# thorstone25/qups

Measured on AMD Instinct MI355X. Metric: beamformed Mpixels/sec (1024^2 px, 256x256 Tx/Rx), higher is better.
Workload: dtype f32; 1 GPU; C3: 256-el FSA (256 Tx x 256 Rx), 1024x1024 ScanCartesian lambda/4, T=2816, complex64, lanczos3; pixels=1048576, pairs_per_frame=68719476736, kernel=tiled, reciprocal_mode=True, reciprocity_fold=True, mirror_mode=True, kernel_name=das_tile_kernel<interp=3,f32,sym,fold,mirror,mb=32,W=128> [jit 56fb2bda29f94d0f], jit=True, fallback_tiles=0, aperture_split=1, parallelism=1 GPU, device=AMD Radeon Graphics (gfx950:sramecc+:xnack-), cu=256

## Files before the change

### include/qdas.h

```cpp
#ifndef QDAS_H
#define QDAS_H

#include <stddef.h>
#include <stdint.h>

#ifdef __cplusplus
extern "C" {
#endif

#define QDAS_VERSION 103

#define QDAS_F64 0
#define QDAS_F32 1
#define QDAS_F16 2

#define QDAS_INTERP_NEAREST  0
#define QDAS_INTERP_LINEAR   1
#define QDAS_INTERP_CUBIC    2
#define QDAS_INTERP_LANCZOS3 3
#define QDAS_INTERP_LINEAR4  4
#define QDAS_INTERP_CUBIC_DEV 5
#define QDAS_FLAG_INTERP_MASK 7
#define QDAS_FLAG_KEEP_RX 8
#define QDAS_FLAG_KEEP_TX 16
#define QDAS_FLAG_TPOSE   32

#define QDAS_MEM_HOST   0
#define QDAS_MEM_DEVICE 1

#define QDAS_KERNEL_AUTO    0
#define QDAS_KERNEL_GENERIC 1
#define QDAS_KERNEL_TILED   2

#define QDAS_RXAPOD_NONE             0
#define QDAS_RXAPOD_ACCEPTANCE       1
#define QDAS_RXAPOD_COSINE           2
#define QDAS_RXAPOD_FNUMBER_PLANAR   3
#define QDAS_RXAPOD_FNUMBER_ORIENTED 4

#define QDAS_PLAN_NO_RECIPROCAL 1
#define QDAS_PLAN_JIT           2

#define QDAS_PLAN_COPY_INPUTS   4

#define QDAS_PLAN_NO_MIRROR     8

#define QDAS_PLAN_MIRROR_SLAB   16

#define QDAS_PLAN_NO_FOLD       32

#define QDAS_PLAN_APPROX_SYMMETRY 64

#define QDAS_PLAN_PREFOLDED     128


#define QDAS_OK            0
#define QDAS_EINVAL        1
#define QDAS_EUNSUPPORTED  2
#define QDAS_EHIP          3
#define QDAS_ENOMEM        4
#define QDAS_ENOCONV       5
#define QDAS_ENOTLDS       6

typedef struct qdas_sizes {
    uint64_t T;
    uint64_t N, M;
    uint64_t I1, I2, I3;
    uint64_t S;
    int32_t  flag;
    int32_t  VS;
    int32_t  DV;
    int32_t  dtype;
} qdas_sizes;

typedef struct qdas_desc {
    qdas_sizes sz;
    double fs, fmod;
    const void *Pi;
    const void *Pr;
    const void *Pv;
    const void *Nv;
    const void *apod;
    const void *cinv;
    const uint64_t *acstride;
    int32_t mem;
    int32_t apod_real;
    int32_t kernel;
    int32_t device;
    uint64_t i_begin;
    uint64_t i_count;
    uint64_t y_ld;
    int32_t  rx_apod_kind;
    int32_t  plan_flags;
    double   rx_apod_p[2];
    const void *rx_normals;
} qdas_desc;

typedef struct qdas_plan qdas_plan;

int  qdas_plan_create(qdas_plan **plan, const qdas_desc *desc);
int  qdas_plan_execute(qdas_plan *plan, const void *x, void *y, void *stream);
int  qdas_plan_execute_frames(qdas_plan *plan, const void *x, void *y, uint64_t F,
                              uint64_t x_stride, uint64_t y_stride, void *stream);
int  qdas_plan_prepare_frames(qdas_plan *plan, uint64_t F);
int  qdas_plan_delays(qdas_plan *plan, void *tau, void *stream);
void qdas_plan_destroy(qdas_plan *plan);
int  qdas_plan_kernel(const qdas_plan *plan);
int  qdas_plan_fallback_tiles(const qdas_plan *plan, uint64_t *ntiles);
int  qdas_plan_tile_shape(const qdas_plan *plan, int *tile_z, int *tile_cols, int *wave_z, int *ksplit);
int  qdas_plan_reciprocal(const qdas_plan *plan);
int  qdas_plan_folded(const qdas_plan *plan);
typedef struct qdas_fold_desc {
    uint64_t T, N;
    uint64_t strN, strM;
    int32_t  dtype;
    int32_t  device;
    const void *wtab;
} qdas_fold_desc;
int  qdas_fold(const qdas_fold_desc *d, const void *x, void *xs, void *stream);
int  qdas_plan_symmetry_bound(const qdas_plan *plan, double *mirror_samples, double *reciprocal_samples);
int  qdas_plan_mirror(const qdas_plan *plan);
int  qdas_plan_kernel_name(const qdas_plan *plan, char *buf, size_t len);
int  qdas_plan_set_timing(qdas_plan *plan, int enable);
int  qdas_plan_last_kernel_ms(const qdas_plan *plan, float *ms);

typedef struct qdas_sharded_plan qdas_sharded_plan;
int  qdas_plan_create_sharded(qdas_sharded_plan **plan, const qdas_desc *desc, int ndev, const int *devices);
int  qdas_plan_execute_sharded(qdas_sharded_plan *plan, const void *x, void *y, void *stream);
int  qdas_plan_sharded_info(const qdas_sharded_plan *plan, int shard, int *device, uint64_t *i_begin, uint64_t *i_count, int *kernel);
int  qdas_plan_sharded_mirror(const qdas_sharded_plan *plan);
void qdas_plan_destroy_sharded(qdas_sharded_plan *plan);

int qdas_DAS (const qdas_sizes *sz, void *y, const double *Pi, const double *Pr, const double *Pv,
              const double *Nv, const void *a, const double *cinv, const uint64_t *acstride_host,
              const void *x, const double tvars[2], void *stream);
int qdas_DASf(const qdas_sizes *sz, void *y, const float *Pi, const float *Pr, const float *Pv,
// ... 217 lines not shown
```

### qups_amd/_lib.py

```python
from __future__ import annotations

import ctypes as C
import os

_HERE = os.path.dirname(os.path.abspath(__file__))
LIB_PATH = os.environ.get("QDAS_LIB") or os.path.join(_HERE, "libqdas.so")

QDAS_F64, QDAS_F32, QDAS_F16 = 0, 1, 2
INTERP_FLAGS = {"nearest": 0, "linear": 1, "cubic": 2, "lanczos3": 3, "cubic_dev": 5}
FLAG_KEEP_RX, FLAG_KEEP_TX, FLAG_TPOSE = 8, 16, 32
MEM_HOST, MEM_DEVICE = 0, 1
KERNEL_AUTO, KERNEL_GENERIC, KERNEL_TILED = 0, 1, 2
KERNEL_NAMES = {KERNEL_GENERIC: "generic", KERNEL_TILED: "tiled"}
MAX_APOD = 6
QDAS_PRE_F32, QDAS_PRE_I16 = 0, 1
QDAS_CONV_FULL, QDAS_CONV_SAME, QDAS_CONV_VALID, QDAS_CONV_CAUSAL = 0, 1, 2, 3
QDAS_CONV_X_ONE_COLUMN, QDAS_CONV_X_ONE_SLICE, QDAS_CONV_Y_ONE_COLUMN, QDAS_CONV_Y_ONE_SLICE = 1, 2, 4, 8
PLAN_NO_RECIPROCAL, PLAN_JIT, PLAN_COPY_INPUTS, PLAN_NO_MIRROR, PLAN_MIRROR_SLAB, PLAN_NO_FOLD, PLAN_APPROX_SYMMETRY, PLAN_PREFOLDED = 1, 2, 4, 8, 16, 32, 64, 128
COH_SLSC_AVERAGE, COH_SLSC_ENSEMBLE, COH_DMAS, COH_COHFAC, COH_PCF = 1, 2, 3, 4, 5
QDAS_ENOCONV = 5
QDAS_ENOTLDS = 6
RXAPOD_NONE, RXAPOD_ACCEPTANCE, RXAPOD_COSINE, RXAPOD_FNUMBER_PLANAR, RXAPOD_FNUMBER_ORIENTED = 0, 1, 2, 3, 4

SYMBOLS = (
    "qdas_plan_create", "qdas_plan_execute", "qdas_plan_execute_frames", "qdas_plan_prepare_frames", "qdas_plan_delays",
    "qdas_plan_destroy", "qdas_plan_kernel", "qdas_plan_fallback_tiles", "qdas_plan_tile_shape", "qdas_plan_reciprocal", "qdas_plan_folded", "qdas_fold", "qdas_plan_symmetry_bound", "qdas_plan_mirror", "qdas_plan_kernel_name", "qdas_plan_set_timing",
    "qdas_plan_last_kernel_ms", "qdas_plan_create_sharded", "qdas_plan_execute_sharded", "qdas_plan_sharded_info", "qdas_plan_sharded_mirror",
    "qdas_plan_destroy_sharded", "qdas_DAS", "qdas_DASf", "qdas_DASh", "qdas_delays", "qdas_delaysf",
    "qdas_das_lut", "qdas_das_lut_last_kernel", "qdas_wsinterpd", "qdas_shift_sum", "qdas_greens", "qdas_convd", "qdas_convd_len", "qdas_permute3", "qdas_pre_plan_create", "qdas_pre_execute", "qdas_pre_plan_destroy", "qdas_pre_plan_one_pass", "qdas_last_error", "qdas_version", "qdas_device_malloc", "qdas_device_free", "qdas_device_trim", "qdas_device_copy", "qdas_iir", "qdas_device_info", "qdas_kernel_variant_build", "qdas_kernel_variant_prebuilt",
    "qdas_coherence", "qdas_eikonal", "qdas_eikonal_tables", "qdas_eikonal_last_passes", "qdas_eikonal_pass_cap", "qdas_adjoint", "qdas_migration",
)


class Sizes(C.Structure):
    _fields_ = [("T", C.c_uint64), ("N", C.c_uint64), ("M", C.c_uint64),
                ("I1", C.c_uint64), ("I2", C.c_uint64), ("I3", C.c_uint64), ("S", C.c_uint64),
                ("flag", C.c_int32), ("VS", C.c_int32), ("DV", C.c_int32), ("dtype", C.c_int32)]


class Desc(C.Structure):
    _fields_ = [("sz", Sizes), ("fs", C.c_double), ("fmod", C.c_double),
                ("Pi", C.c_void_p), ("Pr", C.c_void_p), ("Pv", C.c_void_p), ("Nv", C.c_void_p),
                ("apod", C.c_void_p), ("cinv", C.c_void_p), ("acstride", C.POINTER(C.c_uint64)),
                ("mem", C.c_int32), ("apod_real", C.c_int32), ("kernel", C.c_int32), ("device", C.c_int32),
                ("i_begin", C.c_uint64), ("i_count", C.c_uint64), ("y_ld", C.c_uint64),
                ("rx_apod_kind", C.c_int32), ("plan_flags", C.c_int32), ("rx_apod_p", C.c_double * 2),
                ("rx_normals", C.c_void_p)]


class LutDesc(C.Structure):
    _fields_ = [("T", C.c_uint64), ("N", C.c_uint64), ("M", C.c_uint64), ("I", C.c_uint64),
                ("flag", C.c_int32), ("dtype", C.c_int32), ("omega", C.c_double),
                ("tau_rx", C.c_void_p), ("tau_tx", C.c_void_p), ("w", C.c_void_p),
                ("wstride", C.c_uint64 * 3), ("w_real", C.c_int32), ("reserved", C.c_int32), ("I1", C.c_uint64)]


class WsDesc(C.Structure):
    _fields_ = [("T", C.c_uint64), ("x_tstride", C.c_uint64), ("ndim", C.c_int32), ("flag", C.c_int32), ("dtype", C.c_int32),
                ("w_real", C.c_int32), ("size", C.c_uint64 * 8), ("tstride", C.c_int64 * 8), ("xstride", C.c_int64 * 8),
                ("wstride", C.c_int64 * 8), ("sum", C.c_uint8 * 8), ("omega", C.c_double), ("extrap", C.c_double),
                ("t", C.c_void_p), ("w", C.c_void_p), ("x", C.c_void_p), ("ystride", C.c_int64 * 8), ("lane_dim", C.c_int32), ("reserved", C.c_int32)]


class FoldDesc(C.Structure):
    _fields_ = [("T", C.c_uint64), ("N", C.c_uint64), ("strN", C.c_uint64), ("strM", C.c_uint64), ("dtype", C.c_int32), ("device", C.c_int32), ("wtab", C.c_void_p)]


class IirDesc(C.Structure):
    _fields_ = [("T", C.c_uint64), ("K", C.c_uint64), ("nsec", C.c_int32), ("dtype", C.c_int32), ("cplx", C.c_int32), ("device", C.c_int32),
                ("gain", C.c_double), ("sos", C.POINTER(C.c_double))]


class GreensDesc(C.Structure):
    _fields_ = [("S", C.c_uint64), ("T", C.c_uint64), ("N", C.c_uint64), ("M", C.c_uint64), ("I", C.c_uint64),
                ("En", C.c_int32), ("Em", C.c_int32), ("interp", C.c_int32), ("dtype", C.c_int32),
                ("s0", C.c_double), ("t0", C.c_double), ("fs", C.c_double), ("fsr", C.c_double), ("cinv", C.c_double),
                ("R0", C.c_double), ("Ps", C.c_void_p), ("a", C.c_void_p), ("Pr", C.c_void_p), ("Pv", C.c_void_p),
                ("x", C.c_void_p), ("device", C.c_int32), ("reserved", C.c_int32)]


class PreDesc(C.Structure):
    _fields_ = [("T", C.c_uint64), ("K", C.c_uint64), ("Nfft", C.c_uint64), ("in_type", C.c_int32), ("device", C.c_int32),
                ("fs", C.c_double), ("t0", C.c_double), ("fdown", C.c_double)]


class ShiftDesc(C.Structure):
    _fields_ = [("T", C.c_uint64), ("To", C.c_uint64), ("N", C.c_uint64), ("M", C.c_uint64), ("Mo", C.c_uint64), ("F", C.c_uint64),
                ("flag", C.c_int32), ("dtype", C.c_int32), ("cplx", C.c_int32), ("w_real", C.c_int32), ("device", C.c_int32), ("tpad", C.c_int32),
                ("shift", C.c_void_p), ("w", C.c_void_p)]


class ConvdDesc(C.Structure):
    _fields_ = [("C", C.c_uint64), ("M", C.c_uint64), ("N", C.c_uint64), ("S", C.c_uint64), ("dtype", C.c_int32), ("cplx", C.c_int32),
                ("shape", C.c_int32), ("bcast", C.c_int32), ("device", C.c_int32), ("y_real", C.c_int32)]


class CoherenceDesc(C.Structure):
    _fields_ = [("method", C.c_int32), ("dtype", C.c_int32), ("cplx", C.c_int32), ("device", C.c_int32),
                ("N", C.c_uint64), ("K", C.c_uint64), ("strideN", C.c_int64), ("strideK", C.c_int64),
                ("size", C.c_uint64 * 3), ("stride", C.c_int64 * 3), ("lag_lo", C.c_uint64), ("lag_hi", C.c_uint64),
                ("lags", C.POINTER(C.c_int64)), ("nlags", C.c_uint64), ("gamma", C.c_double)]
# ... 122 lines not shown
```

### qups_amd/csrc/das_tile_impl.h

```cpp
#pragma once
#include "tile_params.h"
#ifndef QDAS_DBG_SYNC
#define QDAS_DBG_SYNC 0
#endif
#ifndef QDAS_ONEACC_PLAIN
#define QDAS_ONEACC_PLAIN 0
#endif
#ifndef QDAS_F16_PIPE
#define QDAS_F16_PIPE 0
#endif
#include "tile_util.h"
#include "tile_taps.h"
#include "tile_hooks.h"
#include "das_tile_cfg.h"

namespace qdas {

typedef __attribute__((address_space(3))) void lds_void;

template <int INTERP_, typename ST_, bool FMOD_, bool WTAB_, bool SYM_, bool FB2_, bool FB4_, int WAVES_, int MB_, int W_, int NBUF_, bool BIG_, bool LUT_, bool BF_ = false, bool MIRQ_ = false, bool FOLD_ = false>
struct TileCfg {
    static constexpr int INTERP = INTERP_, WAVES = WAVES_, MB = MB_, W = W_, NBUF = NBUF_;
    using ST = ST_;
    static constexpr bool FMOD = FMOD_, WTAB = WTAB_, SYM = SYM_, FB2 = FB2_, FB4 = FB4_, BIG = BIG_, LUT = LUT_;
    static constexpr bool BF = BF_;
    static constexpr bool FBX = FB2 || FB4;
    static constexpr bool MIRQ = MIRQ_;
    static constexpr bool FOLD = FOLD_;
    static constexpr bool FOLDQ = FOLD_ && MIRQ_;
    static constexpr bool QUAD = FB4 || (MIRQ && !FOLD) || (FOLDQ && FB2);
    static constexpr bool TWO = (SYM && !FOLD) || FBX || FOLDQ;
    static constexpr bool ONEACC = (FB2 && !SYM && sizeof(ST_) == 8 && MB_ >= 32) || (!TWO && sizeof(ST_) == 8 && FMOD_ && WTAB_ && INTERP_ == 3 && !BF_ && !LUT_ && !BIG_);
    static constexpr int NHP = QUAD ? 2 : 1;
    static constexpr int NFR = FB4 ? 4 : (FB2 ? 2 : 1);
    static constexpr int NW = QUAD ? 4 * MB : (TWO ? 2 * MB : MB);
    static constexpr int K = tapinfo<INTERP>::K;
    static constexpr int THREADS = WAVES * 64;
    static constexpr int WPW = FB4 ? 1 : MB / WAVES;
    static constexpr int SB = (int)sizeof(ST);
    static constexpr bool F32 = (SB == 8);
    static constexpr bool F64 = (SB == 16);
#ifdef QDAS_JIT
    static constexpr bool JITB = true;
#else
    static constexpr bool JITB = false;
#endif
#ifdef QDAS_NO_ACT
    static constexpr bool ACT = false;
#else
    static constexpr bool ACT = !F64 && !SYM && !BIG && !BF_ && !(FB2 && F32 && !JITB) && !FB4;
    static constexpr bool WMIR = ACT && FB2;
    static constexpr bool W64 = F64 && !FMOD_;
#endif
    static constexpr bool WST = WTAB_ && !F64 && !BF_ && !FB4;
    static constexpr int WSTB = WST ? NBUF_ * (2 * MB_ * 8 + 16) : 0;
    static constexpr bool BPIX = F32 && !SYM_ && !FB2_ && !FB4_ && !BF_ && !LUT_ && !BIG_ && !WTAB_ && !FMOD_ && MB_ == 16 && W_ == 384;
    using GT = std::conditional_t<F64, double, float>;
    static constexpr int WB = W * SB;
    static constexpr int PB = 1024;
    static constexpr int PCS = (WB + PB - 1) / PB;
    static constexpr int NDMA = WPW * PCS * (QUAD ? (FB4 ? 2 : 4) : TWO ? 2 : 1);
    static_assert(!(SYM && FBX && !FOLD_) && !(FB2 && FB4) && !(FOLD_ && FB4), "reciprocal mode runs one frame per launch (folded data: one or two)");
    static_assert(!MIRQ || FOLD || (SYM && MB_ == WAVES_ && 4 * MB_ * W_ * (int)sizeof(ST_) <= 65536), "reciprocal + lateral-mirror mode: one window per wave and set, immediate LDS offsets");
    static_assert(!FOLD || (SYM && !WTAB_ && !BIG && !LUT && !BF_ && sizeof(ST_) == 8), "folded data: reciprocal plans, fp32, weights folded into the data");
    static_assert(!FOLDQ || (MB_ % WAVES_ == 0 && (FB2 ? 4 : 2) * MB_ * W_ * (int)sizeof(ST_) <= 65536), "folded data + lateral-mirror mode: two (two frames: four) window sets within the immediate LDS offsets");
    static_assert(!BIG || (!SYM && !FBX), "the re-basing general kernel runs one frame per launch");
    static_assert(!(FOLDQ && FB2) || MB_ == WAVES_, "folded data + mirror mode, two frames: one window per wave and set");
    static_assert(!LUT || (!SYM && !FB4 && !BIG && (!FB2 || JITB)), "table-driven delays: general mode, one frame per launch (hiprtc builds: the lateral-mirror mode's two window sets)");
    static_assert(!BF || (!SYM && !FBX && !BIG && !LUT && sizeof(ST_) == 8), "'BF': general mode, fp32 data, one frame per launch");
    static_assert(!F64 || (!SYM && !FBX && !BIG && !LUT && !BF), "fp64 data: the 'DAS' sum (optionally remodulated / with a weight table), one frame per launch");
    static_assert(FB4 ? (2 * MB == WAVES) : (MB % WAVES == 0 && MB % 2 == 0), "staging split");
    static_assert(WB % 16 == 0, "window must be a whole number of 16-byte lanes");
};

template <class C> struct Tile {
    using ST = typename C::ST;
    const TileParams &P;
    hooks::Timer timer;
    int tid, lane, wave;
    uint32_t M, N;
    int T;
    uint64_t strN, strM;
    int kindB, kindS;
    using GT = typename C::GT;
    struct rec64 { double x, y, z; int b, pad; };
    int *Abase; float *Aext, *Bext; float4 *nrec; rec64 *nrec64; GT *PvL, *NvL; ST *win; float *part; uint32_t win_off;
    unsigned char *wst; uint32_t wst_off;
    uint2 *act;
    uint32_t split, S, tile_id;
    uint32_t Sm, sm;
    double fs, symC; int symCi;
    bool tile_interior;
    int need_b;
    static constexpr uint32_t NOT_MINE = 0xffffffffu;
    uint32_t pofs;
    __device__ __forceinline__ bool in_shard() const { return pofs != NOT_MINE; }
    static __device__ __forceinline__ uint32_t lane_now() {
        uint32_t l;
        asm volatile("v_mbcnt_lo_u32_b32 %0, -1, 0\n\tv_mbcnt_hi_u32_b32 %0, -1, %0" : "=v"(l));
        return l;
    }
    uint64_t ipx;
    uint64_t ipx2;
    GT px, py, pz;
    double cf;
    uint32_t n_lo, n_hi, nstage;
    uint32_t nact; bool use_act;
    v2f acc, acc1, acc2, acc3;
    v2f ra[C::MB / 2];
    v2f bw[C::BPIX ? C::MB / 2 : 1]; bool bp;
    double rad[C::F64 ? C::MB : 1];
    double dacc[4];
    v2f tot[C::NFR];
    double dtot[2], w64[2];
    bool wpix, syn;
    int wb[C::WPW], wb2[C::WPW];
    int qo[C::MIRQ ? (C::FOLD ? 2 * C::WPW : 4) : 1];
    uint32_t soff, soff2;
    __amdgpu_buffer_rsrc_t rsD, rsM;
    uint64_t offD, offM, xbytes;
    int fa, fb;

    __device__ __forceinline__ Tile(const TileParams &p) : P(p) {}

    __device__ __forceinline__ void setup(unsigned char *smem);
    __device__ __forceinline__ uint32_t locate(uint32_t &i1, uint32_t &col, bool first, bool image = false);
    template <bool PROBE> __device__ __forceinline__ bool prologue();
    __device__ __forceinline__ void plan_stages();
    template <bool CHECK> __device__ __forceinline__ void run();
    __device__ __forceinline__ void epilogue();

    __device__ __forceinline__ uint32_t blk(uint32_t r) const {
        if constexpr (C::SYM) return (r * S + ((r & 1u) ? S - 1u - split : split)) * C::MB;
        else if constexpr (C::ACT) return (r * Sm + sm) * C::MB;
        else return r * C::MB;
    }
    __device__ __forceinline__ uint32_t nlim(uint32_t m0) const { return C::SYM ? (m0 + C::MB < N ? m0 + C::MB : N) : n_hi; }

    static __device__ __forceinline__ double dsqrt(double d2) {
        const float s0 = __builtin_amdgcn_sqrtf((float)d2);
        const double sd = (double)s0;
        const double r = __builtin_fma(-sd, sd, d2);
        return __builtin_fma(r, (double)(0.5f * __builtin_amdgcn_rcpf(fmaxf(s0, 1.0e-30f))), sd);
    }
    __device__ __forceinline__ double a_of(uint32_t m, const GT *gPv, const GT *gNv) const;
    __device__ __forceinline__ double b_at(GT ex, GT ey, GT ez) const;
    __device__ __forceinline__ double s_at(uint32_t n, GT ex, GT ey, GT ez) const;
    __device__ __forceinline__ bool on_side(uint32_t n, GT ex, GT ey, GT ez) const;
    __device__ __forceinline__ const GT *geo_Pi() const { return (const GT *)P.Pi; }
    __device__ __forceinline__ const GT *geo_Pr() const { return (const GT *)P.Pr; }
    __device__ __forceinline__ const GT *geo_Pv() const { return (const GT *)P.Pv; }
    __device__ __forceinline__ const GT *geo_Nv() const { return (const GT *)P.Nv; }
    struct wraw { uint32_t a, b; };
    __device__ __forceinline__ wraw wload_raw(uint32_t n, bool image = false) const;
    __device__ __forceinline__ v2f wconv(wraw r) const;
    __device__ __forceinline__ v2f wload(uint32_t n) const { return wconv(wload_raw(n)); }

    __device__ __forceinline__ __amdgpu_buffer_rsrc_t make_rs(uint64_t o, uint64_t extra) const;
    __device__ __forceinline__ int wjr(int r) const;
    __device__ __forceinline__ void dma_block(uint32_t m0);
    __device__ __forceinline__ void stage_dma(int bn, int buf);

    template <bool CHECK, bool TAILV, bool WZ = true> __device__ __forceinline__ void pairs_plain(uint32_t n, uint32_t m0, int bn, float rb, uint32_t cbase, float phB, uint32_t wbase, uint64_t wmask, uint64_t xmask);
    __device__ __forceinline__ void pairs_pipelined(float rb, uint32_t cbase);
    template <bool CHECK, bool TAILV> __device__ __forceinline__ void pairs_f64(uint32_t n, uint32_t m0, int bn, double rb, uint32_t cbase);
    __device__ __forceinline__ void frame_sums(v2f (&Sf)[4]) const {
        if constexpr (C::FOLDQ && C::FB2) { Sf[0] = acc; Sf[1] = acc1; Sf[2] = acc2; Sf[3] = acc3; }
        else if constexpr (C::MIRQ) { Sf[0] = acc + acc1; Sf[1] = acc2 + acc3; }
        else if constexpr (C::FB4) { Sf[0] = acc; Sf[1] = acc1; Sf[2] = acc2; Sf[3] = acc3; }
        else if constexpr (C::FB2) { Sf[0] = acc + acc1; Sf[1] = acc2 + acc3; }
        else Sf[0] = (acc + acc1) + (acc2 + acc3);
    }
};

}

#include "tile_prologue.h"
#include "tile_staging.h"
#include "tile_pairs.h"

namespace qdas {

template <class C> __device__ __forceinline__ uint32_t Tile<C>::locate(uint32_t &i1, uint32_t &col, bool first, bool image) {
    const uint32_t nb = gridDim.x;
    uint32_t bid = blockIdx.x;
    {
        const uint32_t q = nb / 8, r = nb % 8, xcd = bid % 8, k = bid / 8;
        bid = (xcd < r ? xcd * (q + 1) : r * (q + 1) + (xcd - r) * q) + k;
    }
    const uint32_t ntile = P.tiles_x * P.tiles_z;
    const uint32_t sp = bid / ntile;
    bid -= sp * ntile;
#ifdef QDAS_SHALLOW_FIRST
    const uint32_t tz = bid / P.tiles_x, txi = P.tile_x0 + bid % P.tiles_x;
#else
    const uint32_t tz = P.tiles_z - 1u - bid / P.tiles_x, txi = P.tile_x0 + bid % P.tiles_x;
#endif
    if (first) { S = QSPEC(KSPLIT, P.ksplit); split = sp; tile_id = tz + P.tiles_z * txi; }

    const uint64_t I1 = QSPEC(I1, P.I1);
    uint64_t ncols = P.I2 * P.I3;
    asm volatile("" : "+s"(ncols));
    const uint64_t i_end = P.i_begin + P.i_count;
    const int tzl = QSPEC(TZL, P.tz_log2), wzl = QSPEC(WZL, P.wz_log2);
    const uint32_t wave_z = (uint32_t)wave & ((1u << (tzl - wzl)) - 1u), wave_c = (uint32_t)wave >> (tzl - wzl);
    if (first) {
        i1 = (tz << tzl) + (wave_z << wzl) + (uint32_t)(lane & ((1 << wzl) - 1));
        col = txi * ((uint32_t)(C::WAVES * 64) >> tzl) + (wave_c << (6 - wzl)) + (uint32_t)(lane >> wzl);
    } else {
        uint32_t ln = (uint32_t)lane;
        asm volatile("" : "+v"(ln));
        i1 = (tz << tzl) + (wave_z << wzl) + (ln & ((1u << wzl) - 1u));
        col = txi * ((uint32_t)(C::WAVES * 64) >> tzl) + (wave_c << (6 - wzl)) + (ln >> wzl);
    }
    const bool mirror = C::MIRQ || (C::FB2 && QSPEC(MIR, P.mir));
    const uint64_t ncols_mine = mirror ? (ncols + 1) / 2 : ncols;
    uint64_t ig = (uint64_t)i1 + I1 * (uint64_t)col;
    bool inside = ((uint64_t)i1 < I1) && ((uint64_t)col < ncols_mine) && (ig >= P.i_begin) && (ig < i_end);
    if constexpr (C::MIRQ || C::FB2) {
        if (image) {
            const uint64_t col2 = ncols - 1 - (uint64_t)col;
            inside = inside && mirror && col2 != (uint64_t)col;
            ig = (uint64_t)i1 + I1 * col2;
            if (QSPEC(MIR, P.mir) == 2) ig = ig - (I1 * ncols - i_end) + i_end;
        }
    }
    uint32_t po = inside ? (uint32_t)(ig - P.i_begin) : NOT_MINE;
    asm volatile("" : "+v"(po));
    return po;
}

template <class C> __device__ __forceinline__ void Tile<C>::setup(unsigned char *smem) {
    tid = threadIdx.x; lane = tid & 63;
    wave = __builtin_amdgcn_readfirstlane(tid >> 6);
    M = QSPEC(M, (uint32_t)P.M); N = QSPEC(N, (uint32_t)P.N);
    T = QSPEC(T, (int)P.T);
    strN = QSPEC(STRN, P.strN); strM = QSPEC(STRM, P.strM);
    kindB = QSPEC(KINDB, P.kindB); kindS = QSPEC(KINDS, P.kindS);
    fs = P.fs;
    Abase = (int *)smem;
    Aext  = (float *)(Abase + M);
    Bext  = Aext + M;
    nrec = (float4 *)(smem + (((2 * M + N) * 4 + 15) & ~15u));
    nrec64 = (rec64 *)nrec;
    constexpr uint32_t RECB = C::F64 ? 32u : 16u, GB = (uint32_t)sizeof(GT);
    PvL   = (GT *)((unsigned char *)nrec + RECB * N);
    NvL   = PvL + 4 * M;
// ... 354 lines not shown
            if (skip64) {}
            else if (m0 + C::MB <= M) pairs_f64<CHECK, false>(n, m0, bn, rbd, cbase);
            else                      pairs_f64<CHECK, true>(n, m0, bn, rbd, cbase);
        } else if (!skip) {
            const int bn = rec_b;
            const float rb = C::LUT ? tbc - (float)bn : hooks::fake_rx_delay ? (float)(lane * 2 + 3) + 0.37f * (float)(n & 7)
                                                                            : (float)(s_at(n, rec_x, rec_y, rec_z) - (double)bn);
            const uint32_t cbase = win_off + (uint32_t)buf * (C::NW * C::WB) - (MAGIC_BITS * (uint32_t)C::SB);
            if (C::SYM ? (n < m0 && (!C::FOLD || m0 + C::MB <= M)) : (m0 + C::MB <= M)) {
                if constexpr (C::TWO && (C::F32 || C::SYM || QDAS_F16_PIPE) && C::K == 4 && !(CHECK || C::FMOD || C::WTAB) && !hooks::no_pipeline && !((QDAS_ONEACC_PLAIN || C::INTERP == 3) && C::ONEACC))
                    pairs_pipelined(rb, cbase);
                else
                {
                    constexpr uint64_t FULL = C::MB >= 64 ? ~0ull : ((1ull << (C::MB & 63)) - 1ull);
                    bool done = false;
                    if constexpr (C::WST) {
                        if (wmask == FULL && (!C::SYM || xmask == FULL)) {
                            pairs_plain<CHECK, false, false>(n, m0, bn, rb, cbase, phB, wst_off + (uint32_t)buf * WBUF, wmask, xmask);
                            done = true;
                        }
                    }
                    if (!done) pairs_plain<CHECK, false>(n, m0, bn, rb, cbase, phB, wst_off + (uint32_t)buf * WBUF, wmask, xmask);
                }
            } else {
                pairs_plain<CHECK, true>(n, m0, bn, rb, cbase, phB, wst_off + (uint32_t)buf * WBUF, wmask, xmask);
            }
        }
        if constexpr ((QDAS_DBG_SYNC & 8) != 0) __syncthreads();
        if constexpr (!hooks::no_fair_prio) __builtin_amdgcn_s_setprio(3);
        if (!hooks::no_stage_dma && more && dma_late) dma_next((buf + NBUF - 1) % NBUF);
        if (st + 1 < nstage) wst_store((buf + 1) % NBUF);
        timer.mark(3);
        if (!hooks::no_stage_barrier) {
            if (more) asm volatile("s_waitcnt vmcnt(%0) lgkmcnt(0)\n\ts_barrier" ::"n"((NBUF - 2) * NDMA) : "memory");
            else asm volatile("s_waitcnt vmcnt(0) lgkmcnt(0)\n\ts_barrier" ::: "memory");
        }
        timer.mark(4);
        timer.stage_done();
        buf = (buf + 1 == NBUF) ? 0 : buf + 1;
        if (syn) {
            v2f Sf[4];
            frame_sums(Sf);
#pragma unroll
            for (int f = 0; f < C::NFR; ++f) {
                if (wpix) Sf[f] = (v2f){wcur.x * Sf[f].x - wcur.y * Sf[f].y, wcur.x * Sf[f].y + wcur.y * Sf[f].x};
                if (in_shard()) {
                    float2 *plane = (float2 *)P.y + (size_t)f * P.y_fstride + (size_t)n * P.y_ld;
                    asm volatile("" : "+s"(plane));
                    uint32_t po = pofs;
                    asm volatile("" : "+v"(po));
                    float *q = (float *)(plane + po);
                    unsafeAtomicAdd(q, Sf[f].x); unsafeAtomicAdd(q + 1, Sf[f].y);
                }
            }
            if (wpix) { if constexpr (!C::F32) asm volatile("" : "+v"(wnext_r.a)); wcur = wconv(wnext_r); }
            acc = acc1 = acc2 = acc3 = (v2f){0.f, 0.f};
        } else if (C::W64 && wpix) {
            if constexpr (C::W64) {
                const double sr = dacc[0] + dacc[2], si = dacc[1] + dacc[3];
                dtot[0] += w64[0] * sr - w64[1] * si; dtot[1] += w64[0] * si + w64[1] * sr;
                dacc[0] = dacc[1] = dacc[2] = dacc[3] = 0.0;
                w64[0] = w64n[0]; w64[1] = w64n[1];
            }
        } else if (wpix) {
            v2f Sf[4];
            frame_sums(Sf);
#pragma unroll
            for (int f = 0; f < C::NFR; ++f) {
                const v2f wf = (C::WMIR && f == 1) ? wcur2 : wcur;
                tot[f] += (v2f){wf.x * Sf[f].x - wf.y * Sf[f].y, wf.x * Sf[f].y + wf.y * Sf[f].x};
            }
            acc = acc1 = acc2 = acc3 = (v2f){0.f, 0.f};
            if constexpr (!C::F32) asm volatile("" : "+v"(wnext_r.a));
            wcur = wconv(wnext_r);
            wcur2 = wcur;
            if constexpr (C::WMIR) { if (wmir) { asm volatile("" : "+v"(wnext_r2.a)); wcur2 = wconv(wnext_r2); } }
        }
        if constexpr (C::LUT) tbc = tbn;
        if (++k == klim(m0)) { k = 0; m0 = blk(++cr); }
        n = n_next;
    }
}

template <class C> __device__ __forceinline__ void Tile<C>::epilogue() {
    if (syn || C::BF) return;
    if constexpr (C::F64) {
        if (pofs != NOT_MINE) {
            uint32_t po = pofs;
            asm volatile("" : "+v"(po));
            ST *base = S > 1 ? (ST *)P.part + (size_t)split * P.i_count : (ST *)P.y;
            asm volatile("" : "+s"(base));
            if (C::W64 && wpix) st(base, (size_t)po, cplx<double>{dtot[0], dtot[1]});
            else st(base, (size_t)po, cplx<double>{dacc[0] + dacc[2], dacc[1] + dacc[3]});
        }
    } else {
        v2f res[4];
        frame_sums(res);
        uint32_t po = pofs;
        if constexpr (C::SYM) { uint32_t i1, col; po = locate(i1, col, false); }
        if constexpr (C::FOLDQ && C::FB2) {
            uint32_t i1, col;
            const uint32_t po2 = locate(i1, col, false, true);
            const uint32_t pos[2] = {po, po2};
#pragma unroll
            for (int f = 0; f < 2; ++f) {
#pragma unroll
                for (int h = 0; h < 2; ++h) {
                    uint32_t q = pos[h];
                    if (q == NOT_MINE) continue;
                    asm volatile("" : "+v"(q));
                    const v2f r = res[2 * f + h];
                    if (S > 1) { float2 *base = P.part + ((size_t)split * 2 + f) * (P.i_count << (QSPEC(MIR, P.mir) == 2 ? 1 : 0)); asm volatile("" : "+s"(base)); base[q] = make_float2(r.x, r.y); }
                    else { ST *base = (ST *)P.y + (size_t)f * P.y_fstride; asm volatile("" : "+s"(base)); st(base, (size_t)q, cplx<float>{r.x, r.y}); }
                }
            }
            return;
        }
        if constexpr (C::FB2 || C::MIRQ) {
            if (C::MIRQ || QSPEC(MIR, P.mir)) {
                uint32_t i1, col;
                const uint32_t po2 = locate(i1, col, false, true);
                const uint32_t pos[2] = {po, po2};
#pragma unroll
                for (int f = 0; f < 2; ++f) {
                    uint32_t q = pos[f];
                    if (q == NOT_MINE) continue;
                    asm volatile("" : "+v"(q));
                    v2f r = res[f];
                    if constexpr (!C::MIRQ) { if (wpix) r = tot[f]; }
                    if (S > 1) { float2 *base = P.part + (size_t)split * (P.i_count << (QSPEC(MIR, P.mir) == 2 ? 1 : 0)); asm volatile("" : "+s"(base)); base[q] = make_float2(r.x, r.y); }
                    else { ST *base = (ST *)P.y; asm volatile("" : "+s"(base)); st(base, (size_t)q, cplx<float>{r.x, r.y}); }
                }
                return;
            }
        }
        if (po != NOT_MINE) {
            asm volatile("" : "+v"(po));
#pragma unroll
            for (int f = 0; f < C::NFR; ++f) {
                const v2f r = wpix ? tot[f] : res[f];
                if (S > 1) { float2 *base = P.part + ((size_t)split * C::NFR + f) * P.i_count; asm volatile("" : "+s"(base)); base[po] = make_float2(r.x, r.y); }
                else { ST *base = (ST *)P.y + (size_t)f * P.y_fstride; asm volatile("" : "+s"(base)); st(base, (size_t)po, cplx<float>{r.x, r.y}); }
            }
        }
    }
}

template <class C, bool PROBE> __device__ __forceinline__ void das_tile_body(const TileParams &P, unsigned char *smem) {
    Tile<C> t(P);
    t.timer.begin();
    t.setup(smem);
    if (!t.template prologue<PROBE>()) return;
    if constexpr (!PROBE) {
        t.timer.prologue_done();
        t.plan_stages();
        if (P.pro_mask == 2) return;
        if (t.tile_interior) t.template run<false>(); else t.template run<true>();
        t.timer.finish(t.lane, t.wave, C::WAVES);
        t.epilogue();
    }
}

template <int INTERP, typename ST, bool FMOD, bool WTAB, bool SYM, bool FB2, bool FB4, int WAVES, int MB, int W, int NBUF, int PSZ, int BPC, bool PROBE, bool BIG = false, bool LUT = false, bool BFM = false, bool MIRQ = false, bool FOLD = false>
__global__ void __launch_bounds__(WAVES * 64, WAVES * BPC / 4)
das_tile_kernel(const TileParams P) {
    static_assert(PSZ == 16, "16-byte DMA pieces");
    extern __shared__ __attribute__((aligned(16))) unsigned char smem[];
    das_tile_body<TileCfg<INTERP, ST, FMOD, WTAB, SYM, FB2, FB4, WAVES, MB, W, NBUF, BIG, LUT, BFM, MIRQ, FOLD>, PROBE>(P, smem);
}

#ifndef __HIPCC_RTC__
}
#include "jit.h"
namespace qdas {
void tile_census(int ci, int interp, int sample_bytes, bool fm, bool wt, bool probe);
bool tile_prepare_only();
template <int INTERP, typename ST, int CI>
static hipError_t launch_tile_i(const TileParams &P, unsigned ntiles, size_t lds, hipStream_t s) {
    constexpr Cfg G = CFGS[CI];
    constexpr bool FOLD = (CI >= 17 && CI <= 21);
    constexpr bool MIRQ = (CI == 15 || CI == 16 || CI == 17 || CI == 18 || CI == 20);
    constexpr bool SYM = (CI == 1 || CI == 7 || CI == 8 || MIRQ || FOLD), FB2 = (CI == 3 || CI == 4 || CI == 20 || CI == 21), FB4 = (CI == 5 || CI == 6), BIG = (CI == 9), LUT = (CI == 10 || CI == 11), BFM = (CI == 12);
    const bool fm = P.fmod != 0.0, wt = P.wtab != nullptr;
    const dim3 g(ntiles * (P.probe ? 1u : P.ksplit)), b(G.waves * 64);
    tile_census(CI, INTERP, (int)sizeof(ST), fm, wt, P.probe != 0);
#define QDAS_LAUNCH(FM, WT) QDAS_LAUNCH_P(FM, WT, false)
#define QDAS_LAUNCH_P(FM, WT, PR)                                                                        \
    do {                                                                                                 \
        if constexpr (tile_prebuilt(CI, INTERP, FM, WT, PR)) {                                           \
            if (tile_prepare_only()) return hipSuccess;                                                  \
            auto kfn = das_tile_kernel<INTERP, ST, FM, WT, SYM, FB2, FB4, G.waves, G.mb, G.w, G.nbuf, G.psz, G.bpc, PR, BIG && !PR, LUT, BFM && !PR, MIRQ && !PR, FOLD && !PR>; \
            hipError_t e = hipFuncSetAttribute((const void *)kfn, hipFuncAttributeMaxDynamicSharedMemorySize, (int)lds); \
            if (e != hipSuccess) return e;                                                               \
            kfn<<<g, b, lds, s>>>(P);                                                                    \
        } else {                                                                                         \
            return lazy_tile_launch(LazySpec{INTERP, (int)sizeof(ST), FM, WT, CI, PR}, P, g.x, b.x, lds, s, tile_prepare_only()); \
        }                                                                                                \
    } while (0)
    if (P.probe) {
        if constexpr (FB2 || FB4) return hipErrorInvalidValue;
        else { QDAS_LAUNCH_P(false, false, true); return hipGetLastError(); }
    }
    if constexpr (sizeof(ST) == 16) {
        if ((P.apix && fm) || P.gen_kind || P.syn) return hipErrorInvalidValue;
        if (fm && wt) QDAS_LAUNCH(true, true);
        else if (fm)  QDAS_LAUNCH(true, false);
        else if (wt)  QDAS_LAUNCH(false, true);
        else          QDAS_LAUNCH(false, false);
    } else if constexpr (FOLD) {
        if (wt) return hipErrorInvalidValue;
        if (fm) QDAS_LAUNCH(true, false);
        else    QDAS_LAUNCH(false, false);
    } else if constexpr (MIRQ) {
        if (fm && wt) QDAS_LAUNCH(true, true);
        else if (fm)  QDAS_LAUNCH(true, false);
        else if (wt)  QDAS_LAUNCH(false, true);
        else          QDAS_LAUNCH(false, false);
    } else if constexpr (SYM) {
        if (fm && wt) QDAS_LAUNCH(true, true);
        else if (fm)  QDAS_LAUNCH(true, false);
        else if (wt)  QDAS_LAUNCH(false, true);
        else          QDAS_LAUNCH(false, false);
    } else if constexpr (FB4 && sizeof(ST) == 8) {
        if (fm || wt || P.apix || P.gen_kind) return hipErrorInvalidValue;
        QDAS_LAUNCH(false, false);
    } else if constexpr (FB2 && sizeof(ST) == 8) {
        if (P.apix || P.gen_kind) return hipErrorInvalidValue;
        if (fm && wt) QDAS_LAUNCH(true, true);
        else if (fm)  QDAS_LAUNCH(true, false);
        else if (wt)  QDAS_LAUNCH(false, true);
        else          QDAS_LAUNCH(false, false);
    } else {
        if (fm && wt) QDAS_LAUNCH(true, true);
        else if (fm)  QDAS_LAUNCH(true, false);
        else if (wt)  QDAS_LAUNCH(false, true);
        else          QDAS_LAUNCH(false, false);
    }
#undef QDAS_LAUNCH
#undef QDAS_LAUNCH_P
    return hipGetLastError();
// ... 5 lines not shown
```

### qups_amd/csrc/jit.h

```cpp
#pragma once
#include <hip/hip_runtime.h>
#include <stdint.h>
#include <string>
#include <vector>
#include "tile_params.h"
#include "das_tile_cfg.h"

namespace qdas {

struct JitSpec {
    int interp, dtype, fmod, wtab, sym, big;
    int waves, mb, w, nbuf;
    uint64_t N, M, T, I1, strN, strM;
    int kindB, kindS, tzl, wzl;
    unsigned ksplit;
    int gen_kind, has_apix, apix_real, syn, has_st, has_cinv_pix;
    int mir;
    int mirq;
    int mslab;
    int wreal;
    int fold;
    int lut;
    int plain;
};

struct LazySpec { int interp, sample_bytes, fm, wt, ci, probe; };
std::string lazy_tile_source(const LazySpec &k);
hipError_t lazy_tile_launch(const LazySpec &k, const TileParams &P, unsigned grid, unsigned block, size_t lds, hipStream_t s, bool prepare_only);
void lazy_tile_reset();
const std::string &lazy_tile_last();
std::string jit_compile_source(const std::string &src, std::vector<char> *code, std::string *key_out, bool use_disk);

std::string jit_source(const JitSpec &k);
std::string jit_spec_string(const JitSpec &k);
std::string jit_compile(const JitSpec &k, std::vector<char> *code, std::string *key_out, bool use_disk = true);
struct JitKernel { hipFunction_t fn; std::string key, err; };
JitKernel jit_kernel(JitSpec &k, int device);
hipError_t jit_launch(hipFunction_t fn, const TileParams &P, unsigned grid, unsigned block, size_t lds, hipStream_t s);
size_t jit_tile_lds(const JitSpec &k, uint64_t tN, uint64_t tM, uint32_t act_bytes, bool wtab);

}
```

### qups_amd/csrc/jit.hip

```cpp
#include <hip/hip_runtime.h>
#include <hip/hiprtc.h>

#include <dlfcn.h>
#include <fcntl.h>
#include <sys/file.h>
#include <sys/stat.h>
#include <unistd.h>

#include <algorithm>
#include <cstdio>
#include <cstdlib>
#include <cstring>
#include <map>
#include <memory>
#include <mutex>
#include <string>
#include <vector>

#include "../../include/qdas.h"
#include "api_util.h"
#include "jit.h"

namespace qdas {

namespace {
struct Header { const char *name; const char *text; };
#include "jit_sources.inc"

struct Rtc {
    void *h = nullptr;
    decltype(&hiprtcCreateProgram) create = nullptr;
    decltype(&hiprtcCompileProgram) compile = nullptr;
    decltype(&hiprtcGetProgramLogSize) logsize = nullptr;
    decltype(&hiprtcGetProgramLog) log = nullptr;
    decltype(&hiprtcGetCodeSize) codesize = nullptr;
    decltype(&hiprtcGetCode) code = nullptr;
    decltype(&hiprtcDestroyProgram) destroy = nullptr;
    decltype(&hiprtcVersion) version = nullptr;
    bool ok = false;
    std::string why;
};

Rtc &rtc() {
    static Rtc r;
    static std::once_flag once;
    std::call_once(once, [] {
        for (const char *n : {"libhiprtc.so", "libhiprtc.so.7", "/opt/rocm/lib/libhiprtc.so"}) {
            r.h = dlopen(n, RTLD_NOW | RTLD_LOCAL);
            if (r.h) break;
        }
        if (!r.h) {
            const char *e = dlerror();
            r.why = std::string("hiprtc not available: ") + (e ? e : "libhiprtc.so not found");
            return;
        }
#define QDAS_SYM(field, name) r.field = (decltype(r.field))dlsym(r.h, name); if (!r.field) { r.why = "hiprtc: missing symbol " name; return; }
        QDAS_SYM(create, "hiprtcCreateProgram") QDAS_SYM(compile, "hiprtcCompileProgram") QDAS_SYM(logsize, "hiprtcGetProgramLogSize")
        QDAS_SYM(log, "hiprtcGetProgramLog") QDAS_SYM(codesize, "hiprtcGetCodeSize") QDAS_SYM(code, "hiprtcGetCode")
        QDAS_SYM(destroy, "hiprtcDestroyProgram") QDAS_SYM(version, "hiprtcVersion")
#undef QDAS_SYM
        r.ok = true;
    });
    return r;
}

uint64_t fnv1a(const std::string &s, uint64_t h = 1469598103934665603ull) {
    for (unsigned char c : s) { h ^= c; h *= 1099511628211ull; }
    return h;
}

static thread_local bool g_variant_build = false;
std::string cache_dir() {
    if (g_variant_build) { if (const char *v = getenv("QDAS_VARIANT_CACHE_DIR")) if (*v) return std::string(v); }
    if (const char *e = getenv("QDAS_CACHE_DIR")) return *e ? std::string(e) : std::string();
    const char *home = getenv("HOME");
    if (!home || !*home) return std::string();
    return std::string(home) + "/.cache/qdas";
}

void mkdirs(const std::string &p) {
    for (size_t i = 1; i <= p.size(); ++i)
        if (i == p.size() || p[i] == '/') (void)mkdir(p.substr(0, i).c_str(), 0700);
}

bool dir_is_private(const std::string &p) {
    struct stat st;
    if (stat(p.c_str(), &st) != 0 || !S_ISDIR(st.st_mode)) return false;
    return st.st_uid == geteuid() && (st.st_mode & (S_IWGRP | S_IWOTH)) == 0;
}

constexpr char CACHE_MAGIC[8] = {'Q', 'D', 'A', 'S', 'H', 'S', 'A', '1'};

uint64_t fnv_bytes(const char *p, size_t n) {
    uint64_t h = 1469598103934665603ull;
    for (size_t i = 0; i < n; ++i) { h ^= (unsigned char)p[i]; h *= 1099511628211ull; }
    return h;
}

bool read_cache_file(const std::string &p, std::vector<char> *out) {
    FILE *f = fopen(p.c_str(), "rb");
    if (!f) return false;
    fseek(f, 0, SEEK_END);
    const long n = ftell(f);
    fseek(f, 0, SEEK_SET);
    bool ok = n > 28 && n < (1l << 30);
    if (ok) { out->resize((size_t)n); ok = fread(out->data(), 1, (size_t)n, f) == (size_t)n; }
    fclose(f);
    if (ok) {
        const size_t len = (size_t)n - 24;
        uint64_t flen = 0, sum = 0;
        memcpy(&flen, out->data() + len + 8, 8);
        memcpy(&sum, out->data() + len + 16, 8);
        ok = memcmp(out->data() + len, CACHE_MAGIC, 8) == 0 && flen == len && sum == fnv_bytes(out->data(), len) && memcmp(out->data(), "\x7f" "ELF", 4) == 0;
        if (ok) out->resize(len);
    }
    if (!ok) out->clear();
    return ok;
}

void write_cache_file_atomic(const std::string &p, const std::vector<char> &d) {
    const std::string tmp = p + "." + std::to_string((long)getpid()) + ".tmp";
    const int fd = open(tmp.c_str(), O_WRONLY | O_CREAT | O_TRUNC | O_NOFOLLOW, 0600);
    if (fd < 0) return;
    FILE *f = fdopen(fd, "wb");
    if (!f) { close(fd); return; }
    const uint64_t len = d.size(), h = fnv_bytes(d.data(), d.size());
    const bool ok = fwrite(d.data(), 1, d.size(), f) == d.size() && fwrite(CACHE_MAGIC, 1, 8, f) == 8 && fwrite(&len, 8, 1, f) == 1 && fwrite(&h, 8, 1, f) == 1;
    const bool closed = fclose(f) == 0;
    if (ok && closed) (void)rename(tmp.c_str(), p.c_str()); else (void)remove(tmp.c_str());
}

struct BuildLock {
    int fd = -1;
    explicit BuildLock(const std::string &path) {
        fd = open(path.c_str(), O_RDWR | O_CREAT | O_NOFOLLOW, 0600);
        if (fd >= 0 && flock(fd, LOCK_EX) != 0) { close(fd); fd = -1; }
    }
    ~BuildLock() { if (fd >= 0) { (void)flock(fd, LOCK_UN); close(fd); } }
};

std::mutex g_mu;
std::map<std::string, std::vector<char>> g_code;
std::map<std::pair<std::string, int>, hipFunction_t> g_fn;
}

std::string jit_source(const JitSpec &k) {
    char b[4096];
    const char *st = k.dtype == QDAS_F16 ? "uint32_t" : k.dtype == QDAS_F64 ? "double2" : "float2";
    static const char *INTERP_NAMES[8] = {"nearest", "linear", "cubic", "lanczos3", "linear", "cubicdev", "i6", "i7"};
    const std::string sym_name = std::string("qdas_jit_tile__") + INTERP_NAMES[k.interp & 7] + (k.dtype == QDAS_F16 ? "_f16" : k.dtype == QDAS_F64 ? "_f64" : "_f32")
                                 + (k.lut ? "_lut" : "") + (k.fmod ? "_fmod" : "") + (k.wtab ? "_wtab" : "") + (k.sym ? "_sym" : "") + (k.fold ? "_fold" : "") + (k.mirq ? "_mirq" : k.mir ? "_mirror" : "")
                                 + (k.big ? "_big" : "") + "_mb" + std::to_string(k.mb) + "_w" + std::to_string(k.w) + "_n" + std::to_string((unsigned long long)k.N)
                                 + "_m" + std::to_string((unsigned long long)k.M) + "_t" + std::to_string((unsigned long long)k.T);
    snprintf(b, sizeof b,
             "#define QDAS_JIT 1\n%s"
             "#define QDAS_SPEC_M ((uint32_t)%lluu)\n#define QDAS_SPEC_N ((uint32_t)%lluu)\n#define QDAS_SPEC_T ((int)%llu)\n"
             "#define QDAS_SPEC_I1 ((uint64_t)%lluull)\n#define QDAS_SPEC_STRN ((uint64_t)%lluull)\n#define QDAS_SPEC_STRM ((uint64_t)%lluull)\n"
             "#define QDAS_SPEC_KINDB %d\n#define QDAS_SPEC_KINDS %d\n#define QDAS_SPEC_TZL %d\n#define QDAS_SPEC_WZL %d\n#define QDAS_SPEC_KSPLIT ((uint32_t)%uu)\n"
             "#define QDAS_SPEC_GEN_KIND %d\n#define QDAS_SPEC_HAS_APIX %s\n#define QDAS_SPEC_APIX_REAL %d\n#define QDAS_SPEC_SYN %d\n"
             "#define QDAS_SPEC_HAS_ST %s\n#define QDAS_SPEC_HAS_CINV_PIX %s\n#define QDAS_SPEC_MIR %d\n#define QDAS_SPEC_WREAL %d\n"
             "#include \"das_tile_impl.h\"\n"
             "extern \"C\" __global__ void __launch_bounds__(%d, %d) %s(const qdas::TileParams P) {\n"
             "    extern __shared__ __attribute__((aligned(16))) unsigned char smem[];\n"
             "    qdas::das_tile_body<qdas::TileCfg<%d, %s, %s, %s, %s, %s, false, %d, %d, %d, %d, %s, %s, false, %s, %s>, false>(P, smem);\n"
             "}\n",
             k.plain ? "#define QDAS_ONEACC_PLAIN 1\n" : "",
             (unsigned long long)k.M, (unsigned long long)k.N, (unsigned long long)k.T, (unsigned long long)k.I1,
             (unsigned long long)k.strN, (unsigned long long)k.strM, k.kindB, k.kindS, k.tzl, k.wzl, k.ksplit, k.gen_kind,
             k.has_apix ? "true" : "false", k.apix_real, k.syn, k.has_st ? "true" : "false", k.has_cinv_pix ? "true" : "false", k.mslab ? 2 : ((k.mir || k.mirq) ? 1 : 0), k.wreal ? 1 : 0,
             k.waves * 64, k.waves / 4, sym_name.c_str(),
             k.interp, st, k.fmod ? "true" : "false", k.wtab ? "true" : "false", k.sym ? "true" : "false", k.mir ? "true" : "false", k.waves, k.mb, k.w, k.nbuf,
             k.big ? "true" : "false", k.lut ? "true" : "false", k.mirq ? "true" : "false", k.fold ? "true" : "false");
    std::string src = b;
    if (const char *e = getenv("QDAS_JIT_DEFINES")) {
        std::string defs, item;
        for (const char *c = e;; ++c) {
            if (*c == ';' || *c == 0) {
                if (!item.empty()) {
                    const size_t eq = item.find('=');
                    defs += "#define " + (eq == std::string::npos ? item + " 1" : item.substr(0, eq) + " " + item.substr(eq + 1)) + "\n";
                }
                item.clear();
                if (!*c) break;
            } else item += *c;
        }
        src = defs + src;
    }
    return src;
}

static std::string key_of(const std::string &src, int *rtc_major = nullptr) {
    uint64_t h = fnv1a(src);
    if (const char *e = getenv("QDAS_JIT_FLAGS")) h = fnv1a(std::string("flags:") + e, h);
    for (const Header &hd : JIT_HEADERS) h = fnv1a(hd.text, h);
    int maj = 0, min = 0;
    if (rtc().ok) (void)rtc().version(&maj, &min);
    if (rtc_major) *rtc_major = maj;
    h = fnv1a("gfx950;v" + std::to_string(QDAS_VERSION) + ";rtc" + std::to_string(maj) + "." + std::to_string(min), h);
    char hex[32];
    snprintf(hex, sizeof hex, "%016llx", (unsigned long long)h);
    return hex;
}

std::string jit_compile(const JitSpec &k, std::vector<char> *code, std::string *key_out, bool use_disk) {
    return jit_compile_source(jit_source(k), code, key_out, use_disk);
}

std::string jit_compile_source(const std::string &src, std::vector<char> *code, std::string *key_out, bool use_disk) {
    Rtc &R = rtc();
    const std::string key = key_of(src);
    if (key_out) *key_out = key;
    {
        std::lock_guard<std::mutex> lk(g_mu);
        auto it = g_code.find(key);
        if (it != g_code.end()) { *code = it->second; return ""; }
    }
    std::string dir = (use_disk && !getenv("QDAS_JIT_NO_DISK_CACHE")) ? cache_dir() : std::string();
    if (!dir.empty()) { mkdirs(dir); if (!dir_is_private(dir)) dir.clear(); }
    const std::string path = dir + "/" + key + ".hsaco";
    auto from_disk = [&]() {
        if (dir.empty() || !read_cache_file(path, code)) return false;
        std::lock_guard<std::mutex> lk(g_mu);
        g_code[key] = *code;
        return true;
    };
    if (from_disk()) return "";
    if (const char *wd = (use_disk && !getenv("QDAS_JIT_NO_DISK_CACHE")) ? getenv("QDAS_JIT_WARM_DIR") : nullptr) {
        if (*wd && dir_is_private(wd) && read_cache_file(std::string(wd) + "/" + key + ".hsaco", code)) {
            if (!dir.empty()) write_cache_file_atomic(path, *code);
            std::lock_guard<std::mutex> lk(g_mu);
            g_code[key] = *code;
            return "";
        }
    }
    if (!R.ok) return R.why;
    std::unique_ptr<BuildLock> lock;
    if (!dir.empty()) {
        lock.reset(new BuildLock(path + ".lock"));
        if (from_disk()) return "";
    }
    std::vector<const char *> names, texts;
    for (const Header &hd : JIT_HEADERS) { names.push_back(hd.name); texts.push_back(hd.text); }
    hiprtcProgram prog = nullptr;
    if (R.create(&prog, src.c_str(), "qdas_jit_tile.hip", (int)names.size(), texts.data(), names.data()) != HIPRTC_SUCCESS)
        return "hiprtcCreateProgram failed";
    std::vector<std::string> optv = {"--offload-arch=gfx950", "-std=c++17", "-O3", "-ffp-contract=fast"};
    if (const char *e = getenv("QDAS_JIT_FLAGS")) {
        std::string item;
        for (const char *c = e;; ++c) {
            if (*c == ' ' || *c == 0) { if (!item.empty()) optv.push_back(item); item.clear(); if (!*c) break; }
            else item += *c;
        }
    }
    std::vector<const char *> opts;
    for (const std::string &o : optv) opts.push_back(o.c_str());
// ... 21 lines not shown
    if (a == std::string::npos) return "qdas_jit_tile";
    size_t b = a;
    while (b < src.size() && (isalnum((unsigned char)src[b]) || src[b] == '_')) ++b;
    return src.substr(a, b - a);
}

namespace {
struct Entry {
    JitSpec spec{};
    hipFunction_t fn = nullptr;
    std::string key, err;
    int scratch = 0;
    bool transient = false, logged = false;
};
std::mutex g_reg_mu;
std::map<std::string, Entry> g_reg;

std::string scratch_refusal(int scratch, bool variant) {
    if (scratch <= (variant ? 32 : 0) || getenv("QDAS_JIT_ALLOW_SCRATCH")) return "";
    return "hiprtc build uses " + std::to_string(scratch) + " bytes of scratch memory per lane (spilled registers): not used";
}

Entry build(const std::string &src, int device, bool variant) {
    Entry e;
    std::vector<char> code;
    g_variant_build = variant;
    e.err = jit_compile_source(src, &code, &e.key, true);
    g_variant_build = false;
    if (!e.err.empty()) return e;
    {
        std::lock_guard<std::mutex> lk(g_mu);
        auto it = g_fn.find({e.key, device});
        hipModule_t mod = nullptr;
        hipError_t r = hipSuccess;
        if (it != g_fn.end()) e.fn = it->second;
        else if ((r = hipModuleLoadData(&mod, code.data())) != hipSuccess) e.err = std::string("hipModuleLoadData: ") + hipGetErrorString(r);
        else if ((r = hipModuleGetFunction(&e.fn, mod, jit_entry_name(src).c_str())) != hipSuccess) e.err = std::string("hipModuleGetFunction: ") + hipGetErrorString(r);
        else g_fn[{e.key, device}] = e.fn;
        if (r != hipSuccess) { e.fn = nullptr; e.transient = true; return e; }
    }
    if (hipFuncGetAttribute(&e.scratch, HIP_FUNC_ATTRIBUTE_LOCAL_SIZE_BYTES, e.fn) != hipSuccess) { (void)hipGetLastError(); e.scratch = 0; }
    return e;
}

template <class Spec> std::string memo_key(char kind, const Spec &k, int device) {
    std::string m(1, kind);
    m.append((const char *)&k, sizeof k).append((const char *)&device, sizeof device);
    for (const char *v : {"QDAS_JIT_DEFINES", "QDAS_JIT_FLAGS"}) { const char *e = getenv(v); m += e ? std::string("=") + e : std::string(); m += '\0'; }
    return m;
}

template <class Make> Entry resolve(const std::string &mk, bool variant, bool may_build, Make make) {
    std::unique_lock<std::mutex> lk(g_reg_mu);
    auto it = g_reg.find(mk);
    if (it == g_reg.end()) {
        if (!may_build) return Entry{};
        lk.unlock();
        const Entry b = make();
        if (b.transient) return b;
        lk.lock();
        it = g_reg.emplace(mk, b).first;
    }
    Entry &m = it->second;
    const std::string why = m.err.empty() ? scratch_refusal(m.scratch, variant) : m.err;
    if (!why.empty()) { Entry r = m; r.fn = nullptr; r.err = why; return r; }
    if (const char *lf = variant || m.logged ? nullptr : getenv("QDAS_JIT_SPEC_LOG")) {
        if (FILE *f = fopen(lf, "a")) { fprintf(f, "%s\n", jit_spec_string(m.spec).c_str()); fclose(f); }
        m.logged = true;
    }
    return m;
}
}

JitKernel jit_kernel(JitSpec &k, int device) {
    const Entry e = resolve(memo_key('J', k, device), false, true, [&] {
        JitSpec s = k;
        const bool tight = s.mir && !s.sym && s.dtype == QDAS_F32 && s.mb >= 32;
        if (tight && s.has_st) s.plain = 1;
        Entry b = build(jit_source(s), device, false);
        if (b.err.empty() && tight && !s.plain && b.scratch > 0) {
            s.plain = 1;
            Entry b2 = build(jit_source(s), device, false);
            if (b2.err.empty() || b2.transient) b = b2; else s.plain = 0;
        }
        b.spec = s;
        return b;
    });
    k = e.spec;
    return JitKernel{e.fn, e.key, e.err};
}

std::string lazy_tile_source(const LazySpec &k) {
    const Cfg &G = CFGS[k.ci];
    const int CI = k.ci;
    const bool FOLD = (CI >= 17 && CI <= 21), MIRQ = (CI == 15 || CI == 16 || CI == 17 || CI == 18 || CI == 20);
    const bool SYM = (CI == 1 || CI == 7 || CI == 8 || MIRQ || FOLD), FB2 = (CI == 3 || CI == 4 || CI == 20 || CI == 21), FB4 = (CI == 5 || CI == 6), BIG = (CI == 9), LUT = (CI == 10 || CI == 11), BFM = (CI == 12);
    const bool PR = k.probe != 0;
    const char *st = k.sample_bytes == 4 ? "uint32_t" : k.sample_bytes == 16 ? "double2" : "float2";
    auto B = [](bool v) { return v ? "true" : "false"; };
    char b[2048];
    snprintf(b, sizeof b,
             "#include \"das_tile_impl.h\"\n"
             "extern \"C\" __global__ void __launch_bounds__(%d, %d) qdas_jit_tile__cfg%d_i%d_b%d%s%s%s(const qdas::TileParams P) {\n"
             "    extern __shared__ __attribute__((aligned(16))) unsigned char smem[];\n"
             "    qdas::das_tile_body<qdas::TileCfg<%d, %s, %s, %s, %s, %s, %s, %d, %d, %d, %d, %s, %s, %s, %s, %s>, %s>(P, smem);\n"
             "}\n",
             G.waves * 64, G.waves * G.bpc / 4, CI, k.interp, k.sample_bytes, k.fm ? "_fmod" : "", k.wt ? "_wtab" : "", PR ? "_probe" : "",
             k.interp, st, B(k.fm), B(k.wt), B(SYM), B(FB2), B(FB4), G.waves, G.mb, G.w, G.nbuf, B(BIG && !PR), B(LUT), B(BFM && !PR), B(MIRQ && !PR), B(FOLD && !PR), B(PR));
    return b;
}

static thread_local std::string g_lazy_key;
void lazy_tile_reset() { g_lazy_key.clear(); }
const std::string &lazy_tile_last() { return g_lazy_key; }

hipError_t lazy_tile_launch(const LazySpec &k, const TileParams &P, unsigned grid, unsigned block, size_t lds, hipStream_t s, bool prepare_only) {
    int dev = 0;
    if (hipGetDevice(&dev) != hipSuccess) return hipErrorInvalidDevice;
    const bool no_lazy = getenv("QDAS_NO_LAZY") != nullptr;
    const Entry e = no_lazy && prepare_only ? Entry{} : resolve(memo_key('L', k, dev), true, !no_lazy, [&] { return build(lazy_tile_source(k), dev, true); });
    if (!e.fn) {
        ::qdas_internal_set_error(no_lazy ? "this variant of the fused kernel is built on demand (hiprtc), and QDAS_NO_LAZY is set"
                                          : ("this variant of the fused kernel is built on demand: " + e.err).c_str());
        return hipErrorSharedObjectInitFailed;
    }
    g_lazy_key = e.key;
    if (prepare_only) return hipSuccess;
    return jit_launch(e.fn, P, grid, block, lds, s);
}

hipError_t jit_launch(hipFunction_t fn, const TileParams &P, unsigned grid, unsigned block, size_t lds, hipStream_t s) {
    TileParams p = P;
    void *args[] = {&p};
    return hipModuleLaunchKernel(fn, grid, 1, 1, block, 1, 1, (unsigned)lds, s, args, nullptr);
}

size_t jit_tile_lds(const JitSpec &k, uint64_t tN, uint64_t tM, uint32_t act_bytes, bool wtab) {
    const size_t MX = std::min<size_t>(tM > tN ? tM : tN, QDAS_PROLOGUE_CHUNK);
    const size_t off_act = (((((2 * tM + tN) * 4 + 15) & ~(size_t)15) + 16 * tN + 7 * tM * 4) + 15) & ~(size_t)15;
    const size_t off_wst = off_act + (((size_t)act_bytes + 15) & ~(size_t)15);
    const size_t hdr = (off_wst + (wtab ? (size_t)k.nbuf * (2 * (size_t)k.mb * 8 + 16) : 0) + 15) & ~(size_t)15;
    size_t body = (size_t)k.nbuf * k.mb * (k.fold ? (k.mirq ? 2 : 1) : k.mirq ? 4 : (k.sym || k.mir) ? 2 : 1) * k.w * (k.dtype == QDAS_F16 ? 4 : 8);
    const size_t scratch = 2 * (size_t)k.waves * MX * 4 + 1024;
    if (body < scratch) body = scratch;
    return hdr + body;
}

}

namespace qdas {
#define QDAS_JITSPEC_FIELDS(X) X(interp) X(dtype) X(fmod) X(wtab) X(sym) X(big) X(waves) X(mb) X(w) X(nbuf) X(N) X(M) X(T) X(I1) X(strN) X(strM) X(kindB) X(kindS) X(tzl) X(wzl) \
    X(ksplit) X(gen_kind) X(has_apix) X(apix_real) X(syn) X(has_st) X(has_cinv_pix) X(mir) X(mirq) X(mslab) X(wreal) X(fold) X(lut) X(plain)
std::string jit_spec_string(const JitSpec &k) {
    std::string o = "raw:";
#define X(f) o += std::string(#f "=") + std::to_string((unsigned long long)k.f) + ",";
    QDAS_JITSPEC_FIELDS(X)
#undef X
    o.pop_back();
    return o;
}
static bool jit_spec_parse(const char *str, JitSpec *k) {
    if (strncmp(str, "raw:", 4) != 0) return false;
    std::string s(str + 4);
    size_t pos = 0;
    *k = JitSpec{};
    while (pos < s.size()) {
        size_t end = s.find(',', pos);
        if (end == std::string::npos) end = s.size();
        const std::string item = s.substr(pos, end - pos);
        const size_t eq = item.find('=');
        if (eq == std::string::npos) return false;
        const std::string nm = item.substr(0, eq);
        const unsigned long long v = strtoull(item.c_str() + eq + 1, nullptr, 10);
        bool known = false;
#define X(f) if (nm == #f) { k->f = (decltype(k->f))v; known = true; }
        QDAS_JITSPEC_FIELDS(X)
#undef X
        if (!known) return false;
        pos = end + 1;
    }
    return k->waves > 0 && k->mb > 0 && k->w > 0 && k->nbuf >= 2;
}
}

extern "C" int qdas_debug_jit_compile(int interp, int dtype, int sym, int fmod, unsigned long long N, unsigned long long M, unsigned long long T,
                                      char *msg, size_t msg_len, unsigned long long *code_bytes) {
    qdas::JitSpec k{};
    k.interp = interp; k.dtype = dtype; k.sym = sym; k.fmod = fmod;
    const qdas::Cfg &g = qdas::CFGS[qdas::cfg_index(dtype, sym, 1, getenv("QDAS_JIT_NARROW") ? 1 : 0)];
    k.waves = g.waves; k.mb = g.mb; k.w = g.w; k.nbuf = g.nbuf;
    if (const char *e = getenv("QDAS_JIT_MB")) { const int mb = atoi(e); if (mb >= 2 && mb % k.waves == 0) k.mb = mb; }
    k.N = N; k.M = M; k.T = T; k.I1 = 512; k.strN = T; k.strM = T * N; k.kindB = 0; k.kindS = 0; k.tzl = 5; k.wzl = 3; k.ksplit = 1;
    const char *raw = getenv("QDAS_JIT_DEBUG_SPEC");
    if (raw && !strncmp(raw, "raw:", 4)) {
        if (!qdas::jit_spec_parse(raw, &k)) { if (msg && msg_len) snprintf(msg, msg_len, "bad raw spec"); return 1; }
    } else
    if (const char *e = getenv("QDAS_JIT_DEBUG_SPEC")) {
        std::string str(e);
        size_t pos = 0;
        while (pos < str.size()) {
            size_t end = str.find(',', pos);
            if (end == std::string::npos) end = str.size();
            const std::string item = str.substr(pos, end - pos);
            const size_t eq = item.find('=');
            if (eq != std::string::npos) {
                const std::string nm = item.substr(0, eq);
                const long long v = atoll(item.c_str() + eq + 1);
                if (nm == "has_apix") k.has_apix = v != 0; else if (nm == "apix_real") k.apix_real = (int)v; else if (nm == "gen_kind") k.gen_kind = (int)v;
                else if (nm == "syn") k.syn = (int)v; else if (nm == "wtab") k.wtab = v != 0; else if (nm == "kindB") k.kindB = (int)v; else if (nm == "kindS") k.kindS = (int)v;
                else if (nm == "tzl") k.tzl = (int)v; else if (nm == "wzl") k.wzl = (int)v; else if (nm == "ksplit") k.ksplit = (unsigned)v; else if (nm == "I1") k.I1 = (uint64_t)v;
                else if (nm == "has_cinv_pix") k.has_cinv_pix = v != 0; else if (nm == "has_st") k.has_st = v != 0;
                else if (nm == "wreal") k.wreal = v != 0;
                else if (nm == "mb") k.mb = (int)v; else if (nm == "w") k.w = (int)v;
                else if (nm == "fold") { k.fold = v != 0; if (k.fold) { k.sym = 1; const qdas::Cfg &g2 = qdas::CFGS[qdas::cfg_index(dtype, 1, 1, v == 1, k.mirq, 1)]; k.waves = g2.waves; k.mb = g2.mb; k.w = g2.w; k.nbuf = g2.nbuf; } }
                else if (nm == "mirq") { k.mirq = v != 0; if (k.mirq) { const qdas::Cfg &g2 = qdas::CFGS[qdas::cfg_index(dtype, 1, 1, 1, 1)]; k.waves = g2.waves; k.mb = g2.mb; k.w = g2.w; k.nbuf = g2.nbuf; k.sym = 1; } }
                else if (nm == "mir") { k.mir = v != 0; if (k.mir) { const qdas::Cfg &g2 = qdas::CFGS[qdas::cfg_index(dtype, 0, 2, 0)]; k.waves = g2.waves; k.mb = g2.mb; k.w = g2.w; k.nbuf = g2.nbuf; } }
            }
            pos = end + 1;
        }
    }
    std::vector<char> code;
    std::string key;
    const std::string err = qdas::jit_compile(k, &code, &key, getenv("QDAS_CACHE_DIR") != nullptr);
    if (msg && msg_len) snprintf(msg, msg_len, "%s", err.empty() ? key.c_str() : err.c_str());
    if (code_bytes) *code_bytes = code.size();
    return err.empty() ? 0 : 1;
}

extern "C" int qdas_debug_lazy_compile(int ci, int interp, int sample_bytes, int fm, int wt, int probe, char *msg, size_t msg_len, unsigned long long *code_bytes) {
    if (ci < 0 || ci > 21 || interp < 0 || interp > 5 || interp == 4 || (sample_bytes != 4 && sample_bytes != 8 && sample_bytes != 16)) { if (msg && msg_len) snprintf(msg, msg_len, "bad spec"); return 1; }
    const qdas::LazySpec k{interp, sample_bytes, fm, wt, ci, probe};
    std::vector<char> code;
    std::string key;
    const std::string err = qdas::jit_compile_source(qdas::lazy_tile_source(k), &code, &key, getenv("QDAS_CACHE_DIR") != nullptr);
    if (msg && msg_len) snprintf(msg, msg_len, "%s", err.empty() ? key.c_str() : err.c_str());
    if (code_bytes) *code_bytes = code.size();
    return err.empty() ? 0 : 1;
}
extern "C" int qdas_debug_tile_prebuilt(int ci, int interp, int fm, int wt, int probe) { return qdas::tile_prebuilt(ci, interp, fm != 0, wt != 0, probe != 0) ? 1 : 0; }

extern "C" int qdas_kernel_variant_prebuilt(int cfg, int interp, int fmod, int wtab) {
    const bool fm = fmod != 0, wt = wtab != 0;
    const bool known = cfg == 0 || (cfg >= 2 && cfg <= 6) || (cfg >= 8 && cfg <= 14) || (cfg >= 16 && cfg <= 21);
    if (!known || interp < 0 || interp > 5 || interp == 4) return -1;
    if ((cfg >= 17 && wt) || (cfg == 5 && (fm || wt))) return -1;
    return qdas::tile_prebuilt(cfg, interp, fm, wt, false) ? 1 : 0;
}

extern "C" int qdas_kernel_variant_build(int cfg, int interp, int fmod, int wtab) {
    const bool fm = fmod != 0, wt = wtab != 0;
    const int pb = qdas_kernel_variant_prebuilt(cfg, interp, fmod, wtab);
    if (pb < 0) { qdas_internal_set_error("no such variant of the fused kernel"); return 3; }
    if (pb) return 2;
    const int sb = (cfg == 2 || cfg == 4 || cfg == 6 || cfg == 8 || cfg == 11 || cfg == 16) ? 4 : cfg == 13 ? 16 : 8;
    const qdas::LazySpec k{interp, sb, fm, wt, cfg, 0};
    std::vector<char> code;
    std::string key;
    qdas::g_variant_build = true;
    const std::string err = qdas::jit_compile_source(qdas::lazy_tile_source(k), &code, &key, true);
    qdas::g_variant_build = false;
    if (!err.empty()) { qdas_internal_set_error(err.c_str()); return 1; }
    return 0;
}
```

### qups_amd/csrc/plan_modes.h

```cpp
#pragma once
#include <stddef.h>
#include <stdint.h>
#include <algorithm>
#include "../../include/qdas.h"
#include "das_tile_cfg.h"

#ifndef QDAS_MAX_APOD
#define QDAS_MAX_APOD 6
#endif

namespace qdas {

struct TileConfig { int waves; int mb; int window; size_t lds_bytes; int threads; };

inline TileConfig tile_config(int dtype, int sym, int narrow = 0, int fb = 1, int mirq = 0, int fold = 0) {
    const Cfg &g = CFGS[cfg_index(dtype, sym, fb, narrow, mirq, fold)];
    TileConfig c;
    c.waves = g.waves;
    c.mb = g.mb;
    c.window = g.w;
    c.threads = g.waves * 64;
    const int sets = (fold && sym && dtype == 1) ? (mirq ? 2 : 1) * (fb == 2 ? 2 : 1) : (mirq && sym) ? 4 : (sym || fb == 2) ? 2 : 1;
    c.lds_bytes = (size_t)g.nbuf * g.mb * sets * g.w * (dtype == 2 ? 4 : dtype == 0 ? 16 : 8);
    return c;
}

inline size_t tile_lds_bytes(int dtype, int sym, uint64_t N, uint64_t M, int narrow = 0, int pixw = 0, int wtab = 0, int mirq = 0, int fold = 0, int fb = 1) {
    const Cfg &g = CFGS[cfg_index(dtype, sym, fold ? fb : 1, narrow, mirq, fold)];
    const TileConfig c = tile_config(dtype, sym, narrow, fold ? fb : 1, mirq, fold);
    const size_t MX = std::min<size_t>(M > N ? M : N, QDAS_PROLOGUE_CHUNK);
    const size_t off_act = (((((2 * M + N) * 4 + 15) & ~(size_t)15) + (dtype == 0 ? 32 : 16) * N + 7 * M * (dtype == 0 ? 8 : 4)) + 15) & ~(size_t)15;
    const size_t off_wst = off_act + (((pixw ? 8 * (N + 1) : 0) + 15) & ~(size_t)15);
    const size_t hdr = (off_wst + ((wtab && dtype != 0) ? (size_t)g.nbuf * (2 * (size_t)g.mb * 8 + 16) : 0) + 15) & ~(size_t)15;
    size_t body = c.lds_bytes;
    const size_t scratch = 2 * (size_t)g.waves * MX * 4 + 1024;
    if (body < scratch) body = scratch;
    return hdr + body;
}
inline size_t tile_lds_limit(int sym) { return (size_t)(160 * 1024) / CFGS[sym ? 1 : 0].bpc; }

namespace modes {

inline size_t data_size(int dtype) { return dtype == QDAS_F64 ? 16 : (dtype == QDAS_F32 ? 8 : 4); }

struct Switches {
    bool no_sym = false, no_fold = false, no_jit = false, no_mirror = false, no_mirq = false, no_narrow = false, no_role_swap = false, no_bpix = false,
         no_w64 = false, no_mirror_wpix = false, no_mirror_wpix32 = false, no_side_split = false, no_wide = false, no_fb2 = false, no_fb4 = false, no_fold16 = false;
    double sym_tol = -1.0;
    int ksplit = 0;
    int ksplit_m = 0;
};

struct Request {
    bool eligible = true;
    const char *why = "";
    bool mul = false, syn = false, bfm = false, cmap = false;
    int pix_arr = -1;
    bool pix_is_tx = false, pix_only = false, pix_fold = false, bpix_mode = false;
    bool is_pix[QDAS_MAX_APOD] = {};
    uint64_t npix = 0;
    bool dep_rx = false, dep_tx = false;
};

inline Request analyze_request(const qdas_desc &d, const Switches &sw) {
    Request r;
    const qdas_sizes &z = d.sz;
    const int dt = z.dtype;
    const uint64_t *cst = d.acstride, *ast = d.acstride + 6;
    r.mul = (z.flag & QDAS_FLAG_KEEP_TX) && !(z.flag & QDAS_FLAG_KEEP_RX);
    r.syn = ((z.flag & QDAS_FLAG_KEEP_RX) && !(z.flag & QDAS_FLAG_KEEP_TX)) || r.mul;
    r.bfm = (z.flag & QDAS_FLAG_KEEP_TX) && (z.flag & QDAS_FLAG_KEEP_RX);
    r.eligible = (!r.syn && !r.bfm) || dt == QDAS_F32;
    r.why = "tiled kernel needs the 'DAS' mode (or fp32 data and 'SYN' / 'MUL' / 'BF')";
    auto no = [&](const char *w) { r.eligible = false; r.why = w; };
    if (r.eligible && dt == QDAS_F64 && d.rx_apod_kind) no("tiled kernel, fp64 data: a generated receive apodization needs the generic kernel");
    if (r.eligible && (cst[0] || cst[1] || cst[2] || cst[3] || cst[4])) {
        r.cmap = !cst[3] && !cst[4] && (cst[0] == 1 || z.I1 == 1) && (cst[1] == z.I1 || z.I2 == 1) && (cst[2] == z.I1 * z.I2 || z.I3 == 1);
        if (!r.cmap) no("tiled kernel needs a scalar sound speed or a full per-pixel map without aperture dependence");
        else if (dt == QDAS_F64) no("tiled kernel, fp64 data: a sound-speed map needs the generic kernel");
    }
    const uint64_t I = z.I1 * z.I2 * z.I3;
    bool direct = true;
    for (uint64_t s = 0; s < z.S && r.eligible; ++s) {
        const uint64_t *a = &ast[6 * s];
        if (!a[0] && !a[1] && !a[2]) continue;
        const bool dn = a[3] && z.N > 1, dm = a[4] && z.M > 1;
        if (dn && dm) { no("tiled kernel: an apodization array over pixels x receivers x transmits needs the generic kernel"); break; }
        const bool pixstr = (a[0] == 1 || z.I1 == 1) && (a[1] == z.I1 || z.I2 == 1) && (a[2] == z.I1 * z.I2 || z.I3 == 1);
        if (!pixstr || (dn && a[3] != I) || (dm && a[4] != I)) direct = false;
        r.is_pix[s] = true; ++r.npix; r.dep_rx |= dn; r.dep_tx |= dm;
        if (r.pix_arr < 0) r.pix_arr = (int)s;
    }
    if (r.eligible && r.npix) {
        if (r.dep_rx && r.dep_tx) {
            bool ok = dt == QDAS_F32 && d.apod_real && !r.syn && !r.bfm && d.fmod == 0.0 && I < (1ull << 30) && !sw.no_bpix;
            for (uint64_t s = 0; s < z.S && ok; ++s) {
                const uint64_t *a = &ast[6 * s];
                if (!r.is_pix[s] && a[3] && z.N > 1 && a[4] && z.M > 1) ok = false;
            }
            if (ok) { r.bpix_mode = true; r.pix_is_tx = true; for (uint64_t s = 0; s < z.S; ++s) r.is_pix[s] = true; r.npix = z.S; }
            else no("tiled kernel: pixel x receiver and pixel x transmit apodization arrays together run fused for fp32 data, real weights, 'DAS', no remodulation, no N x M array only");
        }
        else if (dt == QDAS_F64 && !(r.npix == 1 && direct && !r.dep_tx && d.fmod == 0.0 && !r.syn && !r.bfm && !r.mul && !sw.no_w64)) {
            no("tiled kernel, fp64 data: only a single pixel x receiver / pixel-only apodization array without remodulation runs fused");
        }
        else if (r.dep_tx) {
            if ((!r.syn || r.mul) && !r.bfm) r.pix_is_tx = true;
            else no("tiled kernel: a pixel x transmit apodization array with 'SYN' / 'BF' needs the generic kernel");
        } else if (!r.dep_rx && z.N > 1) {
            if (!r.bfm && !r.mul) r.pix_only = true;
            else no("tiled kernel: a pixel-only apodization array needs the generic kernel");
        }
        r.pix_fold = r.eligible && (r.npix > 1 || !direct || r.bpix_mode);
    }
    if (r.eligible && d.rx_apod_kind && r.pix_arr >= 0) no("tiled kernel: a generated receive apodization and a pixel-dependent array need the generic kernel");
    if (r.eligible && r.bfm && (r.pix_arr >= 0 || d.rx_apod_kind)) no("tiled kernel: 'BF' with a pixel x receiver apodization needs the generic kernel");
    if (r.eligible && r.mul && ((r.pix_arr >= 0 && !r.pix_is_tx) || d.rx_apod_kind)) no("tiled kernel: 'MUL' with a pixel x receiver apodization needs the generic kernel");
    return r;
}

struct Facts {
    bool recip_known = false, recip_one_t0 = false, recip_exact = false, recip_finite = true;
    double recip_dev = 0.0;
    double cinv0 = 0.0;
    bool fold_buf_known = false, fold_buf_ok = false;
    bool mirror_known = false, mirror_yes = false;
    double mirror_bound = 0.0;
};
enum { NEED_NOTHING = 0, NEED_RECIP = 1, NEED_FOLD_BUF = 2, NEED_MIRROR = 3 };

// ... 119 lines not shown
        if (!t.mir) { t.narrow = 0; t.set_tc(1, 0, 1, 0, 1); fit = run(); if (*err) return false; }
        return fit;
    }
    t.narrow = (t.sym && dt == QDAS_F32 && !sw.no_narrow) ? 1 : 0;
    if (t.sym && t.mir && dt == QDAS_F32 && !t.narrow) t.mir = 0;
    if (t.narrow) t.set_tc(1, 1, 1, t.mir ? 1 : 0);
    else if (t.sym && t.mir) t.set_tc(1, 0, 1, 1);
    if (t.bpix) { t.narrow = 2; t.set_tc(0, 2); }
    fit = run(); if (*err) return false;
    if (t.mir && !fit) {
        t.mir = 0;
        if (t.narrow == 1) t.set_tc(1, 1); else t.set_tc(t.sym);
        fit = run(); if (*err) return false;
    }
    if (t.narrow == 1 && !fit) { t.narrow = 0; t.set_tc(1, 0); fit = run(); if (*err) return false; }
    return fit;
}

inline bool side_split_applicable(const qdas_desc &d, const Request &rq, const Symmetry &s, bool no_fallback, int txkind, bool has_wtab_in_kernel, const Switches &sw) {
    const qdas_sizes &z = d.sz;
    const int dt = z.dtype;
    return !no_fallback && txkind == 1 && !rq.syn && !rq.bfm && !s.sym && !s.big && (rq.pix_arr < 0 || ((rq.pix_is_tx || rq.pix_only) && !(d.fmod != 0.0 && has_wtab_in_kernel)))
           && !d.rx_apod_kind && (dt == QDAS_F32 || dt == QDAS_F16) && z.M < (1u << 15) && tile_lds_bytes(dt, 0, 2 * z.M, z.N, 0, 1, has_wtab_in_kernel ? 1 : 0) <= tile_lds_limit(0) && !sw.no_side_split;
}

inline bool wide_applicable(int dtype, bool no_fallback, bool bfm, int big, int narrow, bool prefolded, uint64_t tN, uint64_t tM, uint64_t strN, uint64_t strM,
                            bool stage_list, bool table_in_kernel, const Switches &sw) {
    return !no_fallback && dtype == QDAS_F32 && !bfm && !big && narrow != 2 && !sw.no_wide && !prefolded
           && tile_lds_bytes(dtype, 0, tN, tM, 2, stage_list ? 1 : 0, table_in_kernel ? 1 : 0) <= tile_lds_limit(0)
           && (tN * strN + (uint64_t)tile_config(dtype, 0, 2).mb * strM) * data_size(dtype) + 65536 < (1ull << 31);
}

inline unsigned choose_ksplit(unsigned ntiles, unsigned cus, uint64_t M, int mb, bool sym, uint64_t kN_eff, bool stage_list, bool syn, const Switches &sw) {
    const uint64_t nmb = (M + (uint64_t)mb - 1) / (uint64_t)mb;
    const unsigned cap = (unsigned)std::min<uint64_t>(8, sym ? nmb : kN_eff);
    unsigned ks = 1;
    while (ks * 2 <= cap && (uint64_t)ntiles * ks < (uint64_t)cus) ks *= 2;
    if (stage_list && !syn)
        while (ks * 2 <= cap && (uint64_t)ntiles * ks < 8ull * cus && kN_eff / (ks * 2) >= 16) ks *= 2;
    if (sw.ksplit >= 1 && sw.ksplit <= 8 && (unsigned)sw.ksplit <= cap) ks = (unsigned)sw.ksplit;
    return ks;
}

inline unsigned choose_ksplit_m(uint32_t *ksplit, uint64_t tM, int mb, bool sym, bool stage_list, bool syn, int dtype, const Switches &sw) {
    if (!stage_list || syn || sym || dtype == QDAS_F64 || *ksplit <= 1) return 1;
    const unsigned nblk = (unsigned)((tM + (uint64_t)mb - 1) / (uint64_t)mb);
    if (sw.ksplit_m >= 1) {
        const unsigned f = (unsigned)sw.ksplit_m;
        return (f <= nblk && *ksplit % f == 0) ? f : 1;
    }
    if (sw.ksplit >= 1 || nblk < 2) return 1;
    const unsigned sm = nblk < 8u ? nblk : 8u;
    unsigned sn = *ksplit / sm;
    if (sn < 1) sn = 1;
    *ksplit = sm * sn;
    return sm;
}

struct StreamModes { bool fb2_ok, fold2_ok, fb4_off; };
struct PlanShape {
    int dtype = QDAS_F32;
    bool tiled = false;
    int sym = 0, fold = 0, mir = 0, narrow = 0, big = 0, bf = 0, syn = 0, stage_shift = 0;
    bool has_apix = false, has_wtab = false, has_bpix = false;
    int gen_kind = 0;
    double fmod = 0.0;
    uint64_t N = 0, M = 0;
    bool mem_device = true;
};
inline StreamModes stream_modes(const PlanShape &p, uint64_t zN, uint64_t zM, const Switches &sw) {
    StreamModes m;
    const int dt = p.dtype;
    m.fb2_ok = p.tiled && dt != QDAS_F64 && !p.mir && !p.stage_shift && p.narrow != 2 && !(dt == QDAS_F32 && (p.has_apix || p.gen_kind)) && !p.bf && !p.sym && !p.big && p.mem_device && !sw.no_fb2;
    m.fold2_ok = p.tiled && p.fold && (!p.mir || p.narrow) && !p.syn && p.mem_device && !sw.no_fb2
                 && tile_lds_bytes(dt, 1, zN, zM, p.narrow, 0, 0, p.mir ? 1 : 0, 1, 2) <= tile_lds_limit(1);
    m.fb4_off = sw.no_fb4 || (dt == QDAS_F32 && p.tiled && (p.fmod != 0.0 || p.has_wtab || p.has_apix || p.gen_kind));
    return m;
}

struct LaunchShape {
    int dtype = QDAS_F32;
    int sym = 0, fold = 0, mir = 0, narrow_raw = 0, big = 0, bf = 0, syn = 0, stage_shift = 0, probe = 0, nfr = 1;
    bool lut = false, has_wtab = false, has_apix = false, has_bpix = false, has_part = false, jit = false;
    int gen_kind = 0;
    double fmod = 0.0;
    uint32_t act_bytes = 0, ksplit = 1;
    uint64_t N = 0, M = 0;
};
struct LaunchChoice { int narrow = 0, fold = 0, mirq = 0, nf = 1, nfr = 1; bool probe_f32sym = false; size_t lds = 0; int cfg = 0; };

inline const char *launch_legal(const LaunchShape &P, LaunchChoice *c) {
    const int dtype = P.dtype, sym = P.sym ? 1 : 0;
    LaunchChoice ch;
    if (sym && dtype != 1 && dtype != 2) return "reciprocal mode: fp32 / fp16 data only";
    if (dtype == 0) {
        if (P.lut || P.bf || P.syn || P.big || P.nfr > 1 || (P.jit && P.probe) || (!P.probe && (P.ksplit < 1 || (P.ksplit > 1 && !P.has_part)))) return "fp64 data: plain 'DAS', one frame per launch";
        ch.lds = tile_lds_bytes(0, 0, P.N, P.M, 0);
        if (ch.lds > tile_lds_limit(0)) return "fp64 data: LDS image too large";
        ch.cfg = 13;
        if (c) *c = ch;
        return nullptr;
    }
    const int narrow = (sym && dtype == 1 && P.narrow_raw) ? 1 : (!sym && dtype == 1 && P.narrow_raw == 2) ? 2 : 0;
    if (narrow == 2 && (P.lut || P.bf || P.big || (!P.probe && P.nfr > 1))) return "384-sample windows: one frame, no table-driven delays / 'BF' / re-basing";
    if (P.has_bpix && (narrow != 2 || P.has_wtab || P.fmod != 0.0 || P.syn || sym)) return "per-pair pixel weights: the 384-sample configuration without table / remodulation only";
    if (P.act_bytes != 0 && P.act_bytes != 8 * (P.N + 1)) return "stage list: 8 (N + 1) bytes";
    const int fold = (sym && P.fold && dtype == 1) ? 1 : 0;
    if (P.fold && (!fold || P.has_wtab)) return "folded data: reciprocal fp32 plans, the table belongs to the fold pass";
    const bool probe_f32sym = P.probe && sym && dtype == 1;
    if (sym && dtype == 1 && !fold && !P.jit && !P.probe) return "unfolded fp32 reciprocal mode: hiprtc builds only";
    const int mirq = (sym && P.mir && !P.probe) ? 1 : 0;
    const size_t lds = probe_f32sym ? tile_lds_bytes(dtype, 1, P.N, P.M, narrow, 0, 0, narrow ? 1 : 0, 1)
                                    : tile_lds_bytes(dtype, sym, P.N, P.M, narrow, P.act_bytes ? 1 : 0, P.has_wtab ? 1 : 0, mirq, fold, (fold && P.nfr == 2) ? 2 : 1);
    if (lds > tile_lds_limit(sym)) return "LDS image too large";
    if (!P.probe && (P.ksplit < 1 || (P.ksplit > 1 && !P.has_part && !P.bf))) return "split aperture without partial images";
    const int nfr = P.probe ? 1 : (P.nfr > 1 ? P.nfr : 1);
    if (P.mir && !P.probe && ((nfr != 1 && !(fold && nfr == 2)) || P.big || P.bf || (P.lut && !P.jit) || P.syn || ((P.has_apix || P.gen_kind) && ((dtype != 2 && !P.jit) || sym || P.stage_shift || P.has_bpix))
                              || (!sym && narrow) || (sym && dtype == 1 && !narrow && !fold)))
        return "lateral-mirror mode: one frame (folded data: two), no re-basing / 'BF' / 'SYN' / tables of delays, pixel weights for fp16 data or hiprtc builds, narrow windows when reciprocal";
    const int nf = (P.mir && !P.probe && !sym) ? 2 : nfr;
    if ((nf != 1 && nf != 2 && nf != 4) || (nf > 1 && ((sym && !(fold && nf == 2)) || P.big))) return "frames per launch: 1, 2 or 4; reciprocal plans one (folded: two); no re-basing";
    if (P.lut && (sym || (nf != 1 && !(P.mir && P.jit && nf == 2 && dtype == 1 && !P.syn)) || (dtype != 1 && dtype != 2) || (P.syn && dtype != 1))) return "table-driven delays: general mode, one frame";
    if (P.jit && (P.probe || nfr != 1 || (P.lut && !P.mir) || P.bf)) return "hiprtc builds: one frame, no probe / 'BF'; table-driven delays in lateral-mirror mode only";
    if (P.bf && (sym || nf != 1 || dtype != 1 || P.lut || P.big || P.has_apix || P.gen_kind)) return "'BF': fp32 general mode without pixel weights";
    ch.narrow = narrow; ch.fold = fold; ch.mirq = mirq; ch.nf = nf; ch.nfr = nfr; ch.probe_f32sym = probe_f32sym; ch.lds = lds;
    ch.cfg = cfg_index(dtype, sym, 1, narrow, mirq, fold);
    if (c) *c = ch;
    return nullptr;
}

struct BuildOutcome {
    int mir = 0, narrow = 0;
    bool side_split = false, wide = false;
    unsigned ksplit = 1;
};
inline LaunchShape derive_launch_shape(const qdas_desc &d, const Request &rq, const Symmetry &sy, const BuildOutcome &o) {
    LaunchShape L;
    const qdas_sizes &z = d.sz;
    const int dt = z.dtype;
    L.dtype = dt; L.sym = sy.sym; L.fold = sy.rfold; L.big = sy.big; L.mir = o.mir; L.narrow_raw = o.narrow;
    L.bf = rq.bfm ? 1 : 0; L.syn = rq.syn ? 1 : 0;
    uint64_t tN = sy.swap ? z.M : z.N, tM = sy.swap ? z.N : z.M;
    const bool apix = rq.bpix_mode || rq.pix_fold || rq.pix_arr >= 0;
    const bool table = z.S > rq.npix;
    L.has_apix = apix; L.has_bpix = rq.bpix_mode; L.gen_kind = d.rx_apod_kind;
    L.has_wtab = table && !L.fold;
    if (o.side_split) { tN = 2 * z.M; tM = z.N; L.stage_shift = 1; L.gen_kind = apix ? 6 : 5; }
    L.act_bytes = ((apix || L.gen_kind) && dt != QDAS_F64) ? (uint32_t)(8 * (tN + 1)) : 0u;
    if (o.wide) { L.narrow_raw = 2; L.sym = 0; if (L.fold) { L.fold = 0; L.has_wtab = table; } }
    L.N = tN; L.M = tM; L.ksplit = o.ksplit; L.has_part = o.ksplit > 1 && !L.bf;
    L.fmod = dt == QDAS_F64 ? d.fmod : (double)(float)d.fmod;
    return L;
}
inline const char *shape_mismatch(const LaunchShape &a, const LaunchShape &b) {
#define QDAS_CMP(f) if (a.f != b.f) return #f;
    QDAS_CMP(dtype) QDAS_CMP(sym) QDAS_CMP(fold) QDAS_CMP(mir) QDAS_CMP(narrow_raw) QDAS_CMP(big) QDAS_CMP(bf) QDAS_CMP(syn) QDAS_CMP(stage_shift) QDAS_CMP(lut)
    QDAS_CMP(has_wtab) QDAS_CMP(has_apix) QDAS_CMP(has_bpix) QDAS_CMP(has_part) QDAS_CMP(gen_kind) QDAS_CMP(fmod) QDAS_CMP(act_bytes) QDAS_CMP(ksplit) QDAS_CMP(N) QDAS_CMP(M)
#undef QDAS_CMP
    return nullptr;
}

}
}
```

### qups_amd/csrc/qdas_api.hip

```cpp
#include <hip/hip_runtime.h>
#include <hip/hip_fp16.h>

#include <algorithm>
#include <cmath>
#include <cstdarg>
#include <cstdio>
#include <cstdlib>
#include <cstring>
#include <string>
#include <vector>

#include "../../include/qdas.h"
#include "api_util.h"
#include "qdas_kernels.h"
#include "jit.h"

using namespace qdas;

static thread_local std::string g_err;

int qdas::fail(int code, const char *fmt, ...) {
    char buf[512];
    va_list ap;
    va_start(ap, fmt);
// ... 291 lines not shown
}
static int mirror_symmetric_map(const float *dmap, uint64_t I1, uint64_t I2, bool *yes) {
    *yes = false;
    uint32_t *flag = nullptr, res = 1;
    HIPCHK(hipMalloc((void **)&flag, sizeof(uint32_t)));
    hipError_t e = hipMemset(flag, 0, sizeof(uint32_t));
    if (e == hipSuccess) {
        const uint64_t n = I1 * (I2 / 2);
        mirror_map_check_kernel<<<(unsigned)std::min<uint64_t>((n + 255) / 256 + 1, 4096), 256, 0, 0>>>((const uint32_t *)dmap, I1, I2, flag);
        e = hipGetLastError();
        if (e == hipSuccess) e = hipMemcpy(&res, flag, sizeof(uint32_t), hipMemcpyDeviceToHost);
    }
    (void)hipFree(flag);
    HIPCHK(e);
    *yes = res == 0;
    return QDAS_OK;
}
static int mirror_symmetric(const qdas_desc *desc, const float *dPi, bool *yes, double tol = -1.0, double cinv_fs = 0.0, double *bound = nullptr) {
    const qdas_sizes &z = desc->sz;
    *yes = false;
    if (bound) *bound = 0.0;
    std::vector<float> hr(3 * z.N), hv(4 * z.M), hn(3 * z.M);
    int rc;
    if ((rc = fetch_host(desc->Pr, hr.size() * 4, desc->mem, hr.data()))) return rc;
    if ((rc = fetch_host(desc->Pv, hv.size() * 4, desc->mem, hv.data()))) return rc;
    if ((rc = fetch_host(desc->Nv, hn.size() * 4, desc->mem, hn.data()))) return rc;
    double dr = 0.0, dv = 0.0;
    auto dist3 = [](const float *a, const float *b) { const double dx = (double)a[0] + (double)b[0], dy = (double)a[1] - (double)b[1], dz = (double)a[2] - (double)b[2]; return sqrt(dx * dx + dy * dy + dz * dz); };
    for (uint64_t n = 0; n < z.N; ++n) {
        const float *a = &hr[3 * n], *b = &hr[3 * (z.N - 1 - n)];
        if (!(a[0] == -b[0] && a[1] == b[1] && a[2] == b[2])) {
            if (tol < 0) return QDAS_OK;
            const double d = dist3(a, b);
            if (!(d == d)) return QDAS_OK;
            dr = std::max(dr, d);
        }
    }
    for (uint64_t m = 0; m < z.M; ++m) {
        const float *a = &hv[4 * m], *b = &hv[4 * (z.M - 1 - m)], *c = &hn[3 * m], *d = &hn[3 * (z.M - 1 - m)];
        if (!(a[3] == b[3] && c[0] == -d[0] && c[1] == d[1] && c[2] == d[2])) return QDAS_OK;
        if (!(a[0] == -b[0] && a[1] == b[1] && a[2] == b[2])) {
            if (tol < 0) return QDAS_OK;
            const double e = dist3(a, b);
            if (!(e == e)) return QDAS_OK;
            dv = std::max(dv, e);
        }
    }
    if (desc->rx_apod_kind && desc->rx_normals) {
        std::vector<float> hx(3 * z.N);
        if ((rc = fetch_host(desc->rx_normals, hx.size() * 4, desc->mem, hx.data()))) return rc;
        for (uint64_t n = 0; n < z.N; ++n) {
            const float *a = &hx[3 * n], *b = &hx[3 * (z.N - 1 - n)];
            if (!(a[0] == -b[0] && a[1] == b[1] && a[2] == b[2])) return QDAS_OK;
        }
    }
    uint32_t *flag = nullptr;
    HIPCHK(hipMalloc(&flag, 2 * sizeof(uint32_t)));
    hipError_t e = hipMemset(flag, 0, 2 * sizeof(uint32_t));
    uint32_t res[2] = {1u, 0x7f800000u};
    if (e == hipSuccess) {
        const uint64_t n = z.I1 * ((z.I2 + 1) / 2);
        mirror_check_kernel<<<(unsigned)std::min<uint64_t>((n + 255) / 256, 4096), 256, 0, 0>>>(dPi, z.I1, z.I2, flag, flag + 1);
        e = hipGetLastError();
        if (e == hipSuccess) e = hipMemcpy(res, flag, 2 * sizeof(uint32_t), hipMemcpyDeviceToHost);
    }
    (void)hipFree(flag);
    HIPCHK(e);
    float dpf;
    memcpy(&dpf, &res[1], 4);
    const double dp = res[0] ? (double)dpf : 0.0;
    if (tol < 0) { *yes = res[0] == 0; return QDAS_OK; }
    const double b = cinv_fs * (2.0 * dp + dr + dv);
    if (bound) *bound = b;
    *yes = b == b && b <= tol;
    return QDAS_OK;
}

static modes::Switches read_switches() {
    modes::Switches sw;
    auto on = [](const char *n) { return getenv(n) != nullptr; };
    sw.no_sym = on("QDAS_NO_SYM"); sw.no_fold = on("QDAS_NO_FOLD"); sw.no_jit = on("QDAS_NO_JIT"); sw.no_mirror = on("QDAS_NO_MIRROR"); sw.no_mirq = on("QDAS_NO_MIRQ");
    sw.no_narrow = on("QDAS_NO_NARROW"); sw.no_role_swap = on("QDAS_NO_ROLE_SWAP"); sw.no_bpix = on("QDAS_NO_BPIX"); sw.no_w64 = on("QDAS_NO_W64");
    sw.no_mirror_wpix = on("QDAS_NO_MIRROR_WPIX"); sw.no_mirror_wpix32 = on("QDAS_NO_MIRROR_WPIX32"); sw.no_side_split = on("QDAS_NO_SIDE_SPLIT"); sw.no_wide = on("QDAS_NO_WIDE");
    sw.no_fb2 = on("QDAS_NO_FB2"); sw.no_fb4 = on("QDAS_NO_FB4"); sw.no_fold16 = on("QDAS_NO_FOLD16");
    if (const char *e = getenv("QDAS_SYM_TOL")) { const double v = atof(e); if (v >= 0.0 && v <= 0.5) sw.sym_tol = v; }
    if (const char *e = getenv("QDAS_KSPLIT")) { const int v = atoi(e); if (v >= 1 && v <= 8) sw.ksplit = v; }
    if (const char *e = getenv("QDAS_KSPLIT_M")) { const int v = atoi(e); if (v >= 1 && v <= 8) sw.ksplit_m = v; }
    return sw;
}

struct PlanBuild {
    const qdas_desc *desc = nullptr;
    modes::Switches sw;
    modes::Request rq;
    modes::Symmetry sy;
    size_t ael = 0;
    int txkind = 0;
    std::vector<float> host_tab;
    uint64_t kN_eff = 0;
    modes::BuildOutcome outcome;
};

static int plan_init(qdas_plan *pl, const qdas_desc *desc) {
    pl->d = *desc;
    const qdas_sizes &z = pl->d.sz;
    pl->I = z.I1 * z.I2 * z.I3;
    pl->i_count = desc->i_count ? desc->i_count : pl->I - desc->i_begin;
    pl->y_ld = desc->y_ld ? desc->y_ld : pl->i_count;
    pl->oN = (z.flag & QDAS_FLAG_KEEP_RX) ? z.N : 1;
    pl->oM = (z.flag & QDAS_FLAG_KEEP_TX) ? z.M : 1;
    if (pl->y_ld < pl->i_count) return fail(QDAS_EINVAL, "y_ld smaller than the pixel count");
    if (desc->plan_flags & QDAS_PLAN_MIRROR_SLAB) {
        const bool ok = z.I3 == 1 && z.I2 % 2 == 0 && z.I1 && desc->i_begin % z.I1 == 0 && pl->i_count % z.I1 == 0 && pl->i_count
                        && desc->i_begin + pl->i_count <= pl->I / 2 && !(z.flag & (QDAS_FLAG_KEEP_RX | QDAS_FLAG_KEEP_TX)) && desc->kernel != QDAS_KERNEL_GENERIC;
        if (!ok) return fail(QDAS_EINVAL, "QDAS_PLAN_MIRROR_SLAB: the slab must be whole columns of the first half of an even number of columns (I3 == 1, 'DAS')");
        if (!desc->y_ld) pl->y_ld = 2 * pl->i_count;
        else if (desc->y_ld < 2 * pl->i_count) return fail(QDAS_EINVAL, "QDAS_PLAN_MIRROR_SLAB: y_ld smaller than 2 * i_count (y holds slab A and its mirror image)");
    }
    return QDAS_OK;
}

static int plan_import_inputs(qdas_plan *pl, const qdas_desc *desc, PlanBuild &b) {
    const qdas_sizes &z = pl->d.sz;
    const int dt = z.dtype;
    GenericParams &g = pl->gp;
    int rc;
    memcpy(g.cst, desc->acstride, sizeof g.cst);
    memset(g.ast, 0, sizeof g.ast);
    memcpy(g.ast, desc->acstride + 6, sizeof(uint64_t) * 6 * z.S);
    const size_t rs = real_size(dt);
    uint64_t apod_elems = 0;
    for (uint64_t s = 0; s < z.S; ++s) {
        const uint64_t end = g.ast[6 * s + 5] + bcast_numel(&g.ast[6 * s], z);
        if (end > apod_elems) apod_elems = end;
    }
    b.ael = desc->apod_real ? apod_real_size(dt) : data_size(dt);
    const uint64_t cinv_elems = bcast_numel(g.cst, z);
    if ((rc = import_array(pl, desc->Pi, 3 * pl->I * rs, desc->mem, &g.Pi))) return rc;
    if ((rc = import_array(pl, desc->Pr, 3 * z.N * rs, desc->mem, &g.Pr))) return rc;
    if ((rc = import_array(pl, desc->Pv, 4 * z.M * rs, desc->mem, &g.Pv))) return rc;
    if ((rc = import_array(pl, desc->Nv, 3 * z.M * rs, desc->mem, &g.Nv))) return rc;
    if ((rc = import_array(pl, desc->cinv, cinv_elems * rs, desc->mem, &g.cinv))) return rc;
    if ((rc = import_array(pl, desc->apod, apod_elems * b.ael, desc->mem, &g.apod))) return rc;
    g.T = z.T; g.N = z.N; g.M = z.M; g.I1 = z.I1; g.I2 = z.I2; g.I3 = z.I3;
    g.i_begin = desc->i_begin; g.i_count = pl->i_count; g.y_ld = pl->y_ld;
    g.fs = dt == QDAS_F64 ? desc->fs : (double)(float)desc->fs;
    g.fmod = dt == QDAS_F64 ? desc->fmod : (double)(float)desc->fmod;
    g.S = (int32_t)z.S; g.flag = z.flag; g.VS = z.VS; g.DV = z.DV; g.apod_real = desc->apod_real;
    g.gen_kind = desc->rx_apod_kind; g.gen_p0 = desc->rx_apod_p[0]; g.gen_p1 = desc->rx_apod_p[1]; g.rxn = nullptr;
    if (g.gen_kind && desc->rx_normals && (rc = import_array(pl, desc->rx_normals, 3 * z.N * rs, desc->mem, &g.rxn))) return rc;
    g.tile_list = nullptr; g.blocks_per_tile = 0; g.tile_cols = 0; g.tiles_z = 0;
    if (dt == QDAS_F64) { if ((rc = fetch_host(desc->cinv, sizeof(double), desc->mem, &pl->cinv0))) return rc; }
    else { float c32; if ((rc = fetch_host(desc->cinv, sizeof(float), desc->mem, &c32))) return rc; pl->cinv0 = (double)c32; }
    return QDAS_OK;
}

static int gather_recip_facts(const qdas_desc *desc, modes::Facts *f) {
    const qdas_sizes &z = desc->sz;
    std::vector<float> hr(3 * z.N), hv(4 * z.M);
    int rc;
    if ((rc = fetch_host(desc->Pr, hr.size() * 4, desc->mem, hr.data()))) return rc;
    if ((rc = fetch_host(desc->Pv, hv.size() * 4, desc->mem, hv.data()))) return rc;
    f->recip_known = true; f->recip_one_t0 = true; f->recip_exact = true; f->recip_finite = true; f->recip_dev = 0.0;
    for (uint64_t m = 0; m < z.M; ++m) {
        if (memcmp(&hv[4 * m + 3], &hv[3], 4) != 0) { f->recip_one_t0 = false; break; }
        if (memcmp(&hv[4 * m], &hr[3 * m], 12) != 0) {
            f->recip_exact = false;
// ... 311 lines not shown
        pl->misfit_frac = keep_frac; pl->no_fallback = keep_frac == 0.0; pl->ntiles = keep_ntiles; pl->tile_cols = keep_cols;
        HIPCHK(hipMemset(pl->fallback, 0, sizeof(uint32_t)));
    }
    return QDAS_OK;
}

static int plan_wide_windows(qdas_plan *pl, const qdas_desc *desc, PlanBuild &b) {
    const qdas_sizes &z = pl->d.sz;
    TileParams &t = pl->tp;
    if (!modes::wide_applicable(z.dtype, pl->no_fallback, b.rq.bfm, t.big, t.narrow, pl->prefolded, t.N, t.M, t.strN, t.strM, t.act_bytes != 0,
                                t.wtab || (t.fold && pl->fold_wtab), b.sw)) return QDAS_OK;
    int rc;
    const TileParams keep = t;
    const TileConfig keep_tc = pl->tc;
    const double keep_frac = pl->misfit_frac;
    const unsigned keep_ntiles = pl->ntiles, keep_cols = pl->tile_cols;
    t.narrow = 2; t.sym = 0;
    if (t.fold) { t.fold = 0; t.wtab = pl->fold_wtab; }
    pl->tc = tile_config(z.dtype, 0, 2);
    auto set_grid = [&](int tzl) { plan_set_grid(pl, tzl); };
    if ((rc = choose_tile_shape(pl, desc, set_grid))) return rc;
    b.outcome.wide = pl->misfit_frac < keep_frac;
    if (!b.outcome.wide) {
        t = keep; pl->tc = keep_tc;
        pl->misfit_frac = keep_frac; pl->no_fallback = keep_frac == 0.0; pl->ntiles = keep_ntiles; pl->tile_cols = keep_cols;
        HIPCHK(hipMemset(pl->fallback, 0, sizeof(uint32_t)));
    }
    return QDAS_OK;
}

static int plan_stage_shape(qdas_plan *pl, const qdas_desc *desc, PlanBuild &b) {
    const qdas_sizes &z = pl->d.sz;
    TileParams &t = pl->tp;
    const bool jit_on = (desc->plan_flags & QDAS_PLAN_JIT) && !b.sw.no_jit;
    const bool f16 = z.dtype == QDAS_F16;
    if (!(jit_on && (z.dtype == QDAS_F32 || f16) && !t.big && !t.bf && !t.syn && !t.bpix && t.narrow == 0 && !t.stage_shift && !t.cinv_pix
          && !(f16 && (t.sym || !t.mir)) && pl->no_fallback && !getenv("QDAS_NO_STAGE_SHAPE") && !getenv("QDAS_JIT_MB") && !getenv("QDAS_JIT_W"))) return QDAS_OK;
    int mb = 0, sets = 1;
    if (t.mir && !t.sym) { mb = 32; sets = 2; }
    else if (!t.mir && (!t.sym || t.fold)) { mb = 64; sets = 1; }
    if (!mb || t.M < (uint64_t)mb) return QDAS_OK;
    const int w1k = f16 ? 256 : 128;
    const int pixw = t.act_bytes ? 1 : 0;
    const size_t hdr = tile_lds_bytes(z.dtype, t.sym, t.N, t.M, 0, pixw, t.wtab ? 1 : 0, 0, t.fold) - tile_config(z.dtype, t.sym, 0, t.mir ? 2 : 1, 0, t.fold).lds_bytes;
    if (hdr + (t.wtab ? (size_t)2 * 2 * (size_t)mb * 8 : 0) + (size_t)2 * sets * mb * 1024 > (size_t)158 * 1024) return QDAS_OK;
    int rc;
    const TileParams keep = t;
    const double keep_frac = pl->misfit_frac;
    const unsigned keep_ntiles = pl->ntiles, keep_cols = pl->tile_cols;
    const bool keep_nf = pl->no_fallback;
    t.probe_w = w1k;
    auto set_grid = [&](int tzl) { plan_set_grid(pl, tzl); };
    if ((rc = choose_tile_shape(pl, desc, set_grid))) return rc;
    const bool fits = pl->no_fallback;
    t.probe_w = 0;
    if (fits) { pl->hint_mb = mb; pl->hint_w = w1k; }
    else {
        t = keep;
        pl->misfit_frac = keep_frac; pl->no_fallback = keep_nf; pl->ntiles = keep_ntiles; pl->tile_cols = keep_cols;
        HIPCHK(hipMemset(pl->fallback, 0, sizeof(uint32_t)));
    }
    return QDAS_OK;
}

static int plan_split_aperture(qdas_plan *pl, PlanBuild &b) {
    const qdas_sizes &z = pl->d.sz;
    TileParams &t = pl->tp;
    int ncu = 0, rc;
    HIPCHK(hipDeviceGetAttribute(&ncu, hipDeviceAttributeMultiprocessorCount, pl->device));
    const unsigned cus = ncu > 0 ? (unsigned)ncu : 256u;
    int mb_eff = pl->hint_mb ? pl->hint_mb : pl->tc.mb;
    int mb_grp = pl->hint_mb ? pl->hint_mb : pl->tc.mb;
    if (const char *e = getenv("QDAS_JIT_MB")) { const int mb = atoi(e); if (mb >= 2 && mb % pl->tc.waves == 0 && (b.desc->plan_flags & QDAS_PLAN_JIT) && !b.sw.no_jit) { mb_eff = mb; mb_grp = mb; } }
    t.ksplit = modes::choose_ksplit(pl->ntiles, cus, z.M, mb_eff, t.sym != 0, b.kN_eff, t.act_bytes != 0, t.syn != 0, b.sw);
    t.ksplit_m = modes::choose_ksplit_m(&t.ksplit, t.M, mb_grp, t.sym != 0, t.act_bytes != 0, t.syn != 0, z.dtype, b.sw);
    if (t.ksplit > 1 && !t.bf) {
        void *pb;
        if ((rc = dev_alloc(pl, &pb, sizeof(float) * 2 * (size_t)t.ksplit * 4 * pl->i_count * (t.mir == 2 ? 2 : 1)))) return rc;
        t.part = (float2 *)pb;
    }
    return QDAS_OK;
}

static int plan_jit(qdas_plan *pl, const qdas_desc *desc, int *remake) {
    const qdas_sizes &z = pl->d.sz;
    const int dt = z.dtype;
    *remake = 0;
    g_err.clear();
    if (!((desc->plan_flags & QDAS_PLAN_JIT) && pl->kernel == QDAS_KERNEL_TILED && !pl->tp.bf && !getenv("QDAS_NO_JIT"))) return QDAS_OK;
    const TileParams &t = pl->tp;
    JitSpec k{};
    k.interp = (z.flag & 7) == 4 ? 1 : (z.flag & 7); k.dtype = dt; k.fmod = t.fmod != 0.0; k.wtab = t.wtab != nullptr; k.sym = t.sym; k.big = t.big;
    const int narrow = (t.sym && dt == QDAS_F32 && t.narrow) ? 1 : (!t.sym && dt == QDAS_F32 && t.narrow == 2) ? 2 : 0;
    const int mirq = (t.sym && t.mir) ? 1 : 0;
    const Cfg &cg = CFGS[cfg_index(dt, t.sym, t.fold ? 1 : (t.mir ? 2 : 1), narrow, mirq, t.fold)];
    k.mir = t.sym ? 0 : t.mir; k.mirq = mirq; k.mslab = t.mir == 2; k.fold = t.fold;
    k.waves = cg.waves; k.mb = cg.mb; k.w = cg.w; k.nbuf = cg.nbuf;
    k.N = t.N; k.M = t.M; k.T = t.T; k.I1 = t.I1; k.strN = t.strN; k.strM = t.strM;
    k.kindB = t.kindB; k.kindS = t.kindS; k.tzl = t.tz_log2; k.wzl = t.wz_log2; k.ksplit = t.ksplit;
    k.gen_kind = t.gen_kind; k.has_apix = t.apix != nullptr; k.apix_real = t.apix_real; k.syn = t.syn;
    k.has_st = t.St != nullptr; k.has_cinv_pix = t.cinv_pix != nullptr;
    k.wreal = (t.wtab && pl->wtab_real && !getenv("QDAS_NO_WREAL")) ? 1 : 0;
    if (t.sym && !mirq && !t.fold && z.M % 32 == 0 && 2 * 32 * k.w * (dt == QDAS_F16 ? 4 : 8) <= 65536 && !getenv("QDAS_JIT_NO_MB32")) k.mb = 32;
    if (pl->hint_mb && pl->hint_w) { k.mb = pl->hint_mb; k.w = pl->hint_w; }
    if (const char *e = getenv("QDAS_JIT_MB")) {
        const int mb = atoi(e);
        if (mb >= 2 && mb % k.waves == 0 && (!t.sym || t.fold || z.M % (uint64_t)mb == 0) && (!mirq || t.fold)) k.mb = mb;
    }
    if (const char *e = getenv("QDAS_JIT_NBUF")) { const int nb = atoi(e); if (nb >= 2 && nb <= 4) k.nbuf = nb; }
    if (const char *e = getenv("QDAS_JIT_W")) { const int wv = atoi(e); if (wv >= 64 && wv <= 1024 && wv % 64 == 0) k.w = wv; }
    pl->jit_lds = dt == QDAS_F64 ? 0 : jit_tile_lds(k, t.N, t.M, t.act_bytes, t.wtab != nullptr);
    const JitKernel jk = pl->jit_lds > (size_t)160 * 1024 ? JitKernel{nullptr, "", "LDS image too large for the requested configuration"} : jit_kernel(k, pl->device);
    pl->jit_fn = jk.fn;
    if (jk.fn) { pl->jit_tag = "jit " + jk.key; pl->jit_mb = k.mb; pl->jit_w = k.w; return QDAS_OK; }
    g_err = "QDAS_PLAN_JIT: " + jk.err + " -- using the prebuilt kernel";
    const bool unfolded = dt == QDAS_F32 && t.sym && !t.fold;
    if ((dt == QDAS_F32 && t.mir && !t.sym && (t.apix || t.gen_kind)) || unfolded)
        *remake = unfolded ? QDAS_PLAN_NO_RECIPROCAL : QDAS_PLAN_NO_MIRROR;
    return QDAS_OK;
}

static void plan_f16_child(qdas_plan *pl, const qdas_desc *desc) {
    const qdas_sizes &z = pl->d.sz;
    if (!(pl->kernel == QDAS_KERNEL_TILED && z.dtype == QDAS_F16 && pl->tp.sym && !pl->tp.syn && !pl->tp.bf && !(desc->plan_flags & QDAS_PLAN_NO_FOLD) && !getenv("QDAS_NO_FOLD")
          && !getenv("QDAS_NO_FOLD16") && z.N >= 2 && z.N <= 65535)) return;
    qdas_desc d = *desc;
    const GenericParams &gg = pl->gp;
    uint64_t acs[6] = {gg.cst[0], gg.cst[1], gg.cst[2], gg.cst[3], gg.cst[4], gg.cst[5]};
    d.sz.dtype = QDAS_F32; d.sz.S = 0;
    d.Pi = gg.Pi; d.Pr = gg.Pr; d.Pv = gg.Pv; d.Nv = gg.Nv; d.cinv = gg.cinv; d.apod = nullptr; d.rx_normals = nullptr; d.rx_apod_kind = 0; d.acstride = acs;
    d.mem = QDAS_MEM_DEVICE; d.device = pl->device; d.y_ld = 0;
    d.plan_flags = (d.plan_flags | QDAS_PLAN_PREFOLDED) & ~(QDAS_PLAN_COPY_INPUTS | QDAS_PLAN_NO_FOLD);
    const std::string keep = g_err;
    qdas_plan *child = nullptr;
    void *fb = nullptr, *yb = nullptr;
    if (qdas_plan_create(&child, &d) == QDAS_OK && child && child->kernel == QDAS_KERNEL_TILED && child->prefolded
        && hipMalloc(&fb, (size_t)z.T * z.N * z.M * 8) == hipSuccess && hipMalloc(&yb, (size_t)child->y_ld * 8 + 16) == hipSuccess
        && hipMemset(fb, 0, (size_t)z.T * z.N * z.M * 8) == hipSuccess) {
        pl->owned.push_back(fb); pl->owned.push_back(yb);
        pl->fold_buf = fb; pl->y32 = yb; pl->f16_child = child;
        pl->fold_wtab = pl->tp.wtab;
    } else {
        (void)hipGetLastError();
        if (fb) (void)hipFree(fb);
        if (yb) (void)hipFree(yb);
        if (child) qdas_plan_destroy(child);
    }
    g_err = keep;
}

static void plan_resolve_kernel(qdas_plan *pl, bool *no_compiler) {
    *no_compiler = false;
    if (!(pl->kernel == QDAS_KERNEL_TILED && !pl->jit_fn && !pl->f16_child)) return;
    std::string built;
    TileParams t1 = pl->tp;
    t1.nfr = 1;
    const hipError_t pe = prepare_tile(t1, pl->d.sz.dtype, pl->ntiles, &built);
    if (pe == hipErrorSharedObjectInitFailed) { *no_compiler = true; return; }
    if (pe != hipSuccess) (void)hipGetLastError();
    if (!built.empty()) pl->jit_tag = "built on demand " + built;
}

static int plan_finish(qdas_plan *pl, const qdas_desc *desc, const PlanBuild &b) {
    const qdas_sizes &z = pl->d.sz;
    const int dt = z.dtype;
    int rc;
    modes::PlanShape ps;
    ps.dtype = dt; ps.tiled = pl->kernel == QDAS_KERNEL_TILED; ps.sym = pl->tp.sym; ps.fold = pl->tp.fold; ps.mir = pl->tp.mir; ps.narrow = pl->tp.narrow; ps.big = pl->tp.big;
    ps.bf = pl->tp.bf; ps.syn = pl->tp.syn; ps.stage_shift = pl->tp.stage_shift; ps.has_apix = pl->tp.apix != nullptr; ps.has_wtab = pl->tp.wtab != nullptr;
    ps.has_bpix = pl->tp.bpix != nullptr; ps.gen_kind = pl->tp.gen_kind; ps.fmod = pl->tp.fmod; ps.N = pl->tp.N; ps.M = pl->tp.M; ps.mem_device = desc->mem == QDAS_MEM_DEVICE;
    const modes::StreamModes sm = modes::stream_modes(ps, z.N, z.M, b.sw);
    pl->fb2_ok = sm.fb2_ok; pl->fold2_ok = sm.fold2_ok; pl->fb4_off = sm.fb4_off;
    if (desc->mem == QDAS_MEM_HOST) {
        pl->x_bytes = (size_t)z.T * z.N * z.M * data_size(dt);
        pl->y_bytes = (size_t)pl->y_ld * pl->oN * pl->oM * data_size(dt);
        if ((rc = dev_alloc(pl, &pl->dx, pl->x_bytes))) return rc;
        if ((rc = dev_alloc(pl, &pl->dy, pl->y_bytes))) return rc;
    }
    pl->mirror_bound = b.sy.mirror_bound; pl->recip_bound = b.sy.recip_bound;
    if (pl->fold_buf && !pl->f16_child && !(pl->kernel == QDAS_KERNEL_TILED && pl->tp.fold)) {
        for (size_t k = 0; k < pl->owned.size(); ++k) if (pl->owned[k] == pl->fold_buf) { pl->owned.erase(pl->owned.begin() + (long)k); break; }
        (void)hipFree(pl->fold_buf);
        pl->fold_buf = nullptr;
    }
    pl->d.Pi = pl->d.Pr = pl->d.Pv = pl->d.Nv = pl->d.apod = pl->d.cinv = pl->d.rx_normals = nullptr;
    pl->d.acstride = nullptr;
    return QDAS_OK;
}

namespace qdas { modes::LaunchShape launch_shape(const TileParams &P, int dtype, bool jit); }

static int plan_cache_prologue(qdas_plan *pl) {
    TileParams &t = pl->tp;
    t.pro_tab = nullptr; t.pro_out = nullptr;
    if (getenv("QDAS_NO_PRO_TAB") || !pl->ntiles) return QDAS_OK;
    t.pro_mask = 0;
    const bool with_mask = t.act_bytes != 0 && !getenv("QDAS_NO_PRO_MASK");
// ... 501 lines not shown
```

### qups_amd/csrc/tile_pairs.h

```cpp
#pragma once

#ifndef QDAS_PAIR_PRIO
#define QDAS_PAIR_PRIO(q) (q)
#endif

namespace qdas {

template <class C> template <bool CHECK, bool TAILV, bool WZ>
__device__ __forceinline__ void Tile<C>::pairs_plain(uint32_t n, uint32_t m0, int bn, float rb, uint32_t cbase, float phB, uint32_t wbase, uint64_t wmask, uint64_t xmask) {
    constexpr int K = C::K, MB = C::MB, WB = C::WB, INTERP = C::INTERP, NHP = C::NHP;
    constexpr bool SYM = C::SYM, FB4 = C::QUAD, FBX = C::FBX, TWO = C::TWO, F32 = C::F32, FMOD = C::FMOD, WTAB = C::WTAB, BF = C::BF;
    constexpr bool TAIL = (!SYM || C::FOLD) && TAILV, DIAG = SYM && TAILV;
    const bool wmixed = C::WST && WZ && ((((wmask ^ (wmask >> 1)) & 0x5555555555555555ull) != 0ull) || (SYM && C::WTAB && (((xmask ^ (xmask >> 1)) & 0x5555555555555555ull) != 0ull)));
    unroll<MB / 2>([&](auto pc) {
        constexpr int p = decltype(pc)::value;
        if constexpr (!hooks::no_fair_prio && (p * 4) % (MB / 2) == 0) __builtin_amdgcn_s_setprio(QDAS_PAIR_PRIO(3 - (p * 4) / (MB / 2)));
        const uint32_t m = m0 + 2 * p;
        if constexpr (TAIL) { if (m >= M) return; }
        if constexpr (DIAG) { if (m + 1 < n) return; }
        const bool upper = !TAIL || (m + 1 < M);
        float wr0 = 1.f, wi0 = 0.f, wr1 = 1.f, wi1 = 0.f;
        float xr0 = 1.f, xi0 = 0.f, xr1 = 1.f, xi1 = 0.f;
        constexpr bool SW = SYM && WTAB;
        constexpr bool SEP = FBX || SW || C::FOLDQ;
        constexpr bool RECIP = SYM && !SW && !C::FOLD;
        v4f wv = {1.f, 0.f, 1.f, 0.f}, xv = {1.f, 0.f, 1.f, 0.f};
        if constexpr (C::WST) {
            if constexpr (WZ) { if (((wmask >> (2 * p)) & 3ull) == 0ull && (!SW || ((xmask >> (2 * p)) & 3ull) == 0ull)) return; }
            asm volatile("ds_read_b128 %0, %1 offset:%2" : "=&v"(wv) : "v"(wbase), "n"(2 * p * 8));
            if constexpr (SW) asm volatile("ds_read_b128 %0, %1 offset:%2" : "=&v"(xv) : "v"(wbase), "n"(MB * 8 + 2 * p * 8));
        } else if constexpr (WTAB) {
            const float2 wa = ((const float2 *)P.wtab)[n + (size_t)N * m];
            const float2 wb_ = upper ? ((const float2 *)P.wtab)[n + (size_t)N * (m + 1)] : make_float2(0.f, 0.f);
            wr0 = wa.x; wi0 = wa.y; wr1 = wb_.x; wi1 = wb_.y;
            if constexpr (!BF) { if (wr0 == 0.f && wi0 == 0.f && wr1 == 0.f && wi1 == 0.f) return; }
        }
        const v2f t = ra[p] + rb;
        const v2f tm = t + MAGIC;
        const v2f s = t - (tm - MAGIC);
        const uint32_t ad0 = (hooks::linear_taps ? (MAGIC_BITS + (uint32_t)lane + (__float_as_uint(tm.x) & 1u)) : __float_as_uint(tm.x)) * (uint32_t)C::SB + cbase;
        const uint32_t ad1 = (hooks::linear_taps ? (MAGIC_BITS + (uint32_t)lane + (__float_as_uint(tm.y) & 1u)) : __float_as_uint(tm.y)) * (uint32_t)C::SB + cbase;
        constexpr bool SPLIT = CHECK || FMOD || WTAB || BF || C::BPIX;
        v2f w[4] = {{0.f, 0.f}, {0.f, 0.f}, {0.f, 0.f}, {0.f, 0.f}};
        unroll<NHP>([&](auto hpc) {
            constexpr int hp = decltype(hpc)::value;
            constexpr int GSET = FB4 ? 2 * hp : 0, HSET = FB4 ? 2 * hp + 1 : 1;
            v2f &A0 = *(FB4 ? (hp ? &acc2 : &acc) : &acc), &A1 = *(FB4 ? (hp ? &acc2 : &acc) : ((C::FOLDQ || C::ONEACC) ? &acc : &acc1));
            v2f &B0 = *((C::MIRQ && !C::FOLD) ? (hp ? &acc2 : &acc) : FB4 ? (hp ? &acc3 : &acc1) : &acc2), &B1 = *((C::MIRQ && !C::FOLD) ? (hp ? &acc2 : &acc) : FB4 ? (hp ? &acc3 : &acc1) : ((SYM || C::ONEACC) ? &acc2 : &acc3));
            v2f v0 = {0.f, 0.f}, v1 = {0.f, 0.f};
            v2f u0 = {0.f, 0.f}, u1 = {0.f, 0.f};
            if constexpr (F32) {
                taps_f32 g0, g1, h0, h1;
                if constexpr (hooks::no_tap_reads) { for (int k = 0; k < 4; ++k) { g0.s[k] = h0.s[k] = (v2f){s.x, t.x}; g1.s[k] = h1.s[k] = (v2f){t.y, s.y}; } }
                else {
                    lds_issue<K, (GSET * MB + 2 * p) * WB>(g0, ad0); lds_issue<K, (GSET * MB + 2 * p + 1) * WB>(g1, ad1);
                    if constexpr (TWO) { lds_issue<K, (HSET * MB + 2 * p) * WB>(h0, ad0); lds_issue<K, (HSET * MB + 2 * p + 1) * WB>(h1, ad1); }
                }
                if constexpr (hp == 0) {
                    if constexpr (hooks::trivial_weights) { w[0] = s; w[1] = t; w[2] = tm; w[3] = s + t; }
                    else if constexpr (K > 1) weights2<INTERP>(s, w);
                }
                if constexpr (TWO) lds_fence2<K>(g0, g1, h0, h1, w); else lds_fence<K>(g0, g1, w);
                if constexpr (DIAG) {
                    const v2f z = {0.f, 0.f};
                    if (m < n)      { for (int k = 0; k < K; ++k) g0.s[k] = z; }
                    if constexpr (C::FOLD) {
                        if constexpr (TWO) { if (m < n) { for (int k = 0; k < K; ++k) h0.s[k] = z; } }
                    } else {
                        if (m <= n)     { for (int k = 0; k < K; ++k) h0.s[k] = z; }
                        if (m + 1 <= n) { for (int k = 0; k < K; ++k) h1.s[k] = z; }
                    }
                }
                if constexpr (TAIL) {
                    if (!upper) {
#pragma unroll
                        for (int k = 0; k < K; ++k) { g1.s[k] = (v2f){0.f, 0.f}; if constexpr (FBX || C::FOLDQ) h1.s[k] = (v2f){0.f, 0.f}; }
                    }
                }
                if constexpr (K == 1) { v0 = g0.s[0]; v1 = g1.s[0]; if constexpr (SEP) { u0 = h0.s[0]; u1 = h1.s[0]; } }
                else if constexpr (SPLIT) {
#pragma unroll
                    for (int k = 0; k < K; ++k) { v0 = w[k].x * g0.s[k] + v0; v1 = w[k].y * g1.s[k] + v1; }
                    if constexpr (RECIP) {
#pragma unroll
                        for (int k = 0; k < K; ++k) { v0 = w[k].x * h0.s[k] + v0; v1 = w[k].y * h1.s[k] + v1; }
                    }
                    if constexpr (SEP) {
#pragma unroll
                        for (int k = 0; k < K; ++k) { u0 = w[k].x * h0.s[k] + u0; u1 = w[k].y * h1.s[k] + u1; }
                    }
                } else {
#pragma unroll
                    for (int k = 0; k < K; ++k) { A0 = w[k].x * g0.s[k] + A0; A1 = w[k].y * g1.s[k] + A1; }
                    if constexpr (TWO) {
#pragma unroll
                        for (int k = 0; k < K; ++k) { B0 = w[k].x * h0.s[k] + B0; B1 = w[k].y * h1.s[k] + B1; }
                    }
                }
                if constexpr (RECIP && K == 1) { v0 += h0.s[0]; v1 += h1.s[0]; }
            } else {
                taps_f16 g0, g1, h0, h1;
                lds_issue<K, (GSET * MB + 2 * p) * WB>(g0, ad0); lds_issue<K, (GSET * MB + 2 * p + 1) * WB>(g1, ad1);
                if constexpr (TWO) { lds_issue<K, (HSET * MB + 2 * p) * WB>(h0, ad0); lds_issue<K, (HSET * MB + 2 * p + 1) * WB>(h1, ad1); }
                if constexpr (hp == 0 && K > 1) weights2<INTERP>(s, w);
                if constexpr (TWO) lds_fence2<K>(g0, g1, h0, h1, w); else lds_fence<K>(g0, g1, w);
                if constexpr (DIAG) {
                    if (m < n)      { for (int k = 0; k < K; ++k) g0.r[k] = 0u; }
                    if constexpr (C::FOLD) {
                        if constexpr (TWO) { if (m < n) { for (int k = 0; k < K; ++k) h0.r[k] = 0u; } }
                    } else {
                        if (m <= n)     { for (int k = 0; k < K; ++k) h0.r[k] = 0u; }
                        if (m + 1 <= n) { for (int k = 0; k < K; ++k) h1.r[k] = 0u; }
                    }
                }
                if constexpr (TAIL) {
                    if (!upper) {
#pragma unroll
                        for (int k = 0; k < K; ++k) { g1.r[k] = 0u; if constexpr (FBX || C::FOLDQ) h1.r[k] = 0u; }
                    }
                }
                if constexpr (K == 1) {
                    v0 = half2_to_v2f(g0.r[0]); v1 = half2_to_v2f(g1.r[0]);
                    if constexpr (SEP) { u0 = half2_to_v2f(h0.r[0]); u1 = half2_to_v2f(h1.r[0]); }
                    if constexpr (RECIP) { v0 += half2_to_v2f(h0.r[0]); v1 += half2_to_v2f(h1.r[0]); }
                } else if constexpr (SPLIT) {
#pragma unroll
                    for (int k = 0; k < K; ++k) { mix_mac(v0, g0.r[k], w[k].x); mix_mac(v1, g1.r[k], w[k].y); }
                    if constexpr (RECIP) {
#pragma unroll
                        for (int k = 0; k < K; ++k) { mix_mac(v0, h0.r[k], w[k].x); mix_mac(v1, h1.r[k], w[k].y); }
                    }
                    if constexpr (SEP) {
#pragma unroll
                        for (int k = 0; k < K; ++k) { mix_mac(u0, h0.r[k], w[k].x); mix_mac(u1, h1.r[k], w[k].y); }
                    }
                } else {
#pragma unroll
                    for (int k = 0; k < K; ++k) { mix_mac(A0, g0.r[k], w[k].x); mix_mac(A1, g1.r[k], w[k].y); }
                    if constexpr (TWO) {
#pragma unroll
                        for (int k = 0; k < K; ++k) { mix_mac(B0, h0.r[k], w[k].x); mix_mac(B1, h1.r[k], w[k].y); }
                    }
                }
            }
            if constexpr (C::WST && hp == 0) {
                asm volatile("" : "+v"(wv), "+v"(xv));
                wr0 = wv.x; wi0 = wv.y; wr1 = wv.z; wi1 = wv.w;
                xr0 = xv.x; xi0 = xv.y; xr1 = xv.z; xi1 = xv.w;
            }
            if constexpr (CHECK) {
                const uint32_t mb = upper ? m + 1 : m;
                const int ws0 = Abase[m] + bn, ws1 = Abase[mb] + bn;
                const float lo0 = tapinfo<INTERP>::LO - 0.5f - (float)ws0, hi0 = (float)(T - K + 1 - ws0) - 0.5f;
                const float lo1 = tapinfo<INTERP>::LO - 0.5f - (float)ws1, hi1 = (float)(T - K + 1 - ws1) - 0.5f;
                const bool k0 = (t.x >= lo0) && (t.x < hi0), k1 = (t.y >= lo1) && (t.y < hi1) && upper;
                v0 = k0 ? v0 : (v2f){0.f, 0.f}; v1 = k1 ? v1 : (v2f){0.f, 0.f};
                if constexpr (SEP) { u0 = k0 ? u0 : (v2f){0.f, 0.f}; u1 = k1 ? u1 : (v2f){0.f, 0.f}; }
            }
            if constexpr (C::BPIX) {
                {
                    const v2f b2 = bw[p];
                    v0 = b2.x != 0.f ? v0 * b2.x : (v2f){0.f, 0.f};
                    v1 = b2.y != 0.f ? v1 * b2.y : (v2f){0.f, 0.f};
                }
            }
            if constexpr (FMOD) {
                const uint32_t mb = upper ? m + 1 : m;
                const float f = (float)(P.fmod / fs);
                const v2f ph = t * f + ((v2f){Aext[m], Aext[mb]} + phB);
                const float c0 = __builtin_amdgcn_cosf(ph.x), s0 = __builtin_amdgcn_sinf(ph.x);
                const float c1 = __builtin_amdgcn_cosf(ph.y), s1 = __builtin_amdgcn_sinf(ph.y);
                if constexpr (!BF && !WTAB) {
                    rot_acc(A0, v0, c0, s0); rot_acc(A1, v1, c1, s1);
                    if constexpr (FBX || C::FOLDQ) { rot_acc(B0, u0, c0, s0); rot_acc(B1, u1, c1, s1); }
                } else {
                    v0 = (v2f){v0.x * c0 - v0.y * s0, v0.x * s0 + v0.y * c0};
                    v1 = (v2f){v1.x * c1 - v1.y * s1, v1.x * s1 + v1.y * c1};
                    if constexpr (SEP) {
                        u0 = (v2f){u0.x * c0 - u0.y * s0, u0.x * s0 + u0.y * c0};
                        u1 = (v2f){u1.x * c1 - u1.y * s1, u1.x * s1 + u1.y * c1};
                    }
                }
            }
            if constexpr (BF) {
                if constexpr (WTAB) {
                    v0 = (v2f){wr0 * v0.x - wi0 * v0.y, wr0 * v0.y + wi0 * v0.x};
// ... 3 lines not shown
                    float2 *pl0 = (float2 *)P.y + ((size_t)n * P.bf_pn + (size_t)m * P.bf_pm) * P.y_ld;
                    asm volatile("" : "+s"(pl0));
                    uint32_t po = pofs;
                    asm volatile("" : "+v"(po));
                    pl0[po] = make_float2(v0.x, v0.y);
                    if (upper) { float2 *pl1 = pl0 + P.bf_pm * P.y_ld; asm volatile("" : "+s"(pl1)); pl1[po] = make_float2(v1.x, v1.y); }
                }
            } else if constexpr (WTAB) {
                if constexpr (C::WST && WZ) {
                  if (wmixed) {
                    const v2f z = {0.f, 0.f};
                    if (!((wmask >> (2 * p)) & 1ull)) { v0 = z; if constexpr (FBX) u0 = z; }
                    if (!((wmask >> (2 * p + 1)) & 1ull)) { v1 = z; if constexpr (FBX) u1 = z; }
                    if constexpr (SW) { if (!((xmask >> (2 * p)) & 1ull)) { u0 = z; } if (!((xmask >> (2 * p + 1)) & 1ull)) { u1 = z; } }
                  }
                }
                wgt_acc(A0, v0, wr0, wi0); wgt_acc(A1, v1, wr1, wi1);
                if constexpr (FBX) { wgt_acc(B0, u0, wr0, wi0); wgt_acc(B1, u1, wr1, wi1); }
                if constexpr (SW) { wgt_acc(B0, u0, xr0, xi0); wgt_acc(B1, u1, xr1, xi1); }
            } else if constexpr (FMOD) {
            } else if constexpr (SPLIT || K == 1) { A0 += v0; A0 += v1; if constexpr (FBX || C::FOLDQ) { B0 += u0; B0 += u1; } }
        });
    });
}

template <class C> template <bool CHECK, bool TAILV>
__device__ __forceinline__ void Tile<C>::pairs_f64(uint32_t n, uint32_t m0, int bn, double rb, uint32_t cbase) {
    constexpr int K = C::K, MB = C::MB, WB = C::WB, INTERP = C::INTERP;
    double lead[4];
    weights1_lead<INTERP, !C::FMOD>(lead);
    const double fq = C::FMOD ? P.fmod / fs : 0.0;
    unroll<MB>([&](auto pc) {
        constexpr int p = decltype(pc)::value;
        if constexpr (!hooks::no_fair_prio && (p * 4) % MB == 0) __builtin_amdgcn_s_setprio(QDAS_PAIR_PRIO(3 - (p * 4) / MB));
        const uint32_t m = m0 + p;
        if constexpr (TAILV) { if (m >= M) return; }
        if constexpr (C::FMOD) __builtin_amdgcn_sched_barrier(0);
        double wr = 1.0, wi = 0.0;
        if constexpr (C::WTAB) {
            const double2 wv = ((const double2 *)P.wtab)[n + (size_t)N * m];
            wr = wv.x; wi = wv.y;
            if (wr == 0.0 && wi == 0.0) return;
        }
        const double t = rad[p] + rb;
        const double tm = t + MAGIC64;
        const double s = t - (tm - MAGIC64);
        const uint32_t ad = (uint32_t)__double2loint(tm) * 16u + cbase;
        taps_f64 g;
        lds_issue<K, p * WB>(g, ad);
        double w[4] = {0.0, 0.0, 0.0, 0.0};
        if constexpr (K > 1) weights1<INTERP>(s, w, lead);
        lds_fence<K>(g, w);
        double &ar = dacc[2 * (p & 1)], &ai = dacc[2 * (p & 1) + 1];
        if constexpr (K > 1 && !CHECK && !C::WTAB && !C::FMOD) {
#pragma unroll
            for (int k = 0; k < K; ++k) { ar = __builtin_fma(w[k], g.s[k].x, ar); ai = __builtin_fma(w[k], g.s[k].y, ai); }
        } else {
            double vr = g.s[0].x, vi = g.s[0].y;
            if constexpr (K > 1) {
                vr *= w[0]; vi *= w[0];
#pragma unroll
                for (int k = 1; k < K; ++k) { vr = __builtin_fma(w[k], g.s[k].x, vr); vi = __builtin_fma(w[k], g.s[k].y, vi); }
            }
            if constexpr (CHECK) {
                const int ws = Abase[m] + bn;
                const double lo = (double)tapinfo<INTERP>::LO - 0.5 - (double)ws, hi = (double)(T - K + 1 - ws) - 0.5;
                const bool keep = (t >= lo) && (t < hi);
                vr = keep ? vr : 0.0; vi = keep ? vi : 0.0;
            }
            if constexpr (C::FMOD) {
                __builtin_amdgcn_sched_barrier(0);
                const double ph = (t + ((double)(Abase[m] + bn) + (0.5 - (double)tapinfo<INTERP>::OFF))) * fq;
                double c, sn;
                sincos2pi_f64(ph - __builtin_rint(ph), c, sn);
                const double xr = vr * c - vi * sn, xi = vr * sn + vi * c;
                vr = xr; vi = xi;
            }
            if constexpr (C::WTAB) { ar += wr * vr - wi * vi; ai += wr * vi + wi * vr; }
            else { ar += vr; ai += vi; }
        }
    });
}

template <class C> __device__ __forceinline__ void Tile<C>::pairs_pipelined(float rb, uint32_t cbase) {
    constexpr int K = C::K, MB = C::MB, WB = C::WB, INTERP = C::INTERP, NHP = C::NHP;
    constexpr bool FB4 = C::QUAD, F32 = C::F32;
    constexpr int NP = MB / 2, NU = NP * NHP;
    using taps_t = std::conditional_t<F32, taps_f32, taps_f16>;
    taps_t gd0[2], gd1[2];
    v2f sv[2];
    uint32_t a0v[2], a1v[2];
    v2f w[4];
    auto index = [&](auto uc) {
        constexpr int u = decltype(uc)::value, p = u / NHP, hp = u % NHP, GSET = FB4 ? 2 * hp : 0;
        if constexpr (hp == 0) {
            const v2f t = ra[p] + rb;
            const v2f tm = t + MAGIC;
            sv[p & 1] = t - (tm - MAGIC);
            a0v[p & 1] = __float_as_uint(tm.x) * (uint32_t)C::SB + cbase;
            a1v[p & 1] = __float_as_uint(tm.y) * (uint32_t)C::SB + cbase;
        }
        if constexpr (F32 && hooks::no_tap_reads) { for (int k = 0; k < 4; ++k) { gd0[u & 1].s[k] = (v2f){sv[p & 1].x, rb}; gd1[u & 1].s[k] = (v2f){rb, sv[p & 1].y}; } }
        else { lds_issue<K, (GSET * MB + 2 * p) * WB>(gd0[u & 1], a0v[p & 1]); lds_issue<K, (GSET * MB + 2 * p + 1) * WB>(gd1[u & 1], a1v[p & 1]); }
    };
    index(std::integral_constant<int, 0>{});
    unroll<NU>([&](auto uc) {
        constexpr int u = decltype(uc)::value, p = u / NHP, hp = u % NHP, HSET = FB4 ? 2 * hp + 1 : 1;
        if constexpr (!hooks::no_fair_prio && (u * 4) % NU == 0) __builtin_amdgcn_s_setprio(QDAS_PAIR_PRIO(3 - (u * 4) / NU));
        taps_t h0, h1;
        if constexpr (F32 && hooks::no_tap_reads) { for (int k = 0; k < 4; ++k) { h0.s[k] = sv[p & 1]; h1.s[k] = (v2f){sv[p & 1].y, sv[p & 1].x}; } }
        else { lds_issue<K, (HSET * MB + 2 * p) * WB>(h0, a0v[p & 1]); lds_issue<K, (HSET * MB + 2 * p + 1) * WB>(h1, a1v[p & 1]); }
        if constexpr (u + 1 < NU) index(std::integral_constant<int, u + 1>{});
        if constexpr (hp == 0) {
            if constexpr (hooks::trivial_weights) { w[0] = sv[p & 1]; w[1] = sv[p & 1] + 1.f; w[2] = sv[p & 1] * 2.f; w[3] = 1.f - sv[p & 1]; }
            else weights2<INTERP>(sv[p & 1], w);
        }
        if constexpr (u + 1 < NU) lds_fence2_keep<8>(gd0[u & 1], gd1[u & 1], h0, h1, w);
        else                      lds_fence2_keep<0>(gd0[u & 1], gd1[u & 1], h0, h1, w);
        v2f &A0 = *(FB4 ? (hp ? &acc2 : &acc) : &acc), &A1 = *(FB4 ? (hp ? &acc2 : &acc) : ((C::FOLDQ || C::ONEACC) ? &acc : &acc1));
        v2f &B0 = *((C::MIRQ && !C::FOLD) ? (hp ? &acc2 : &acc) : FB4 ? (hp ? &acc3 : &acc1) : &acc2), &B1 = *((C::MIRQ && !C::FOLD) ? (hp ? &acc2 : &acc) : FB4 ? (hp ? &acc3 : &acc1) : ((C::SYM || C::ONEACC) ? &acc2 : &acc3));
#pragma unroll
        for (int k = 0; k < K; ++k) {
            tap_mac(A0, gd0[u & 1], k, w[k].x); tap_mac(A1, gd1[u & 1], k, w[k].y);
            tap_mac(B0, h0, k, w[k].x);         tap_mac(B1, h1, k, w[k].y);
        }
    });
}

}
```

### qups_amd/csrc/tile_staging.h

```cpp
#pragma once

namespace qdas {

constexpr uint32_t DMA_REBASE = 1u << 30;

template <class C> __device__ __forceinline__ __amdgpu_buffer_rsrc_t Tile<C>::make_rs(uint64_t o, uint64_t extra) const {
    const uint64_t rem = xbytes > o ? xbytes - o : 0;
    return __builtin_amdgcn_make_buffer_rsrc((void *)((const char *)P.x + (rem ? o + extra : 0)), 0, rem > 0xfffffff0ull ? 0xfffffff0u : (uint32_t)rem, 0x00020000);
}

template <class C> __device__ __forceinline__ int Tile<C>::wjr(int r) const {
    return C::FB4 ? __builtin_amdgcn_readfirstlane(wave % C::MB) : __builtin_amdgcn_readfirstlane(wave + C::WAVES * r);
}

template <class C> __device__ __forceinline__ void Tile<C>::dma_block(uint32_t m0) {
    constexpr int SB = C::SB;
    if constexpr (C::MIRQ) {
        rsD = make_rs(0, 0);
        if constexpr (C::FOLD && C::FB2) rsM = make_rs(0, P.x_fstride);
        if constexpr (C::FOLD) {
#pragma unroll
            for (int r = 0; r < C::WPW; ++r) {
                const uint32_t m = m0 + (uint32_t)wjr(r);
                const uint32_t mc = m < M ? m : M - 1;
// ... 61 lines not shown
#pragma unroll
                for (int k = 0; k < 2; ++k) {
#pragma unroll
                    for (int q = 0; q < PCS; ++q) {
                        lds_void *dst = (lds_void *)((unsigned char *)win + ((buf * NW + (2 * f + k) * MB + j) * WB + q * PB));
#ifdef QDAS_DMA_SAME_SRC
                        if (l16 < need_b - q * PB)
                            __builtin_amdgcn_raw_ptr_buffer_load_lds(f ? rsM : rsD, dst, 16, l16, (j & 1) * PB + q * PB, 0, 0);
#else
                        if (l16 < need_b - q * PB)
                            __builtin_amdgcn_raw_ptr_buffer_load_lds(f ? rsM : rsD, dst, 16, l16, qo[2 * r + k] + bs + q * PB, 0, 0);
#endif
                    }
                }
            }
            qo[2 * r] += (int)((uint32_t)strN * SB); qo[2 * r + 1] -= (int)((uint32_t)strM * SB);
        }
        return;
    } else if constexpr (C::MIRQ) {
        const int j = wjr(0);
#pragma unroll
        for (int k = 0; k < 4; ++k) {
#pragma unroll
            for (int q = 0; q < PCS; ++q) {
                lds_void *dst = (lds_void *)((unsigned char *)win + ((buf * NW + k * MB + j) * WB + q * PB));
                if (l16 < need_b - q * PB)
                    __builtin_amdgcn_raw_ptr_buffer_load_lds(rsD, dst, 16, l16, qo[k] + bs + q * PB, 0, 0);
            }
        }
        qo[0] += (int)((uint32_t)strN * SB); qo[1] += (int)((uint32_t)strM * SB);
        qo[2] -= (int)((uint32_t)strN * SB); qo[3] -= (int)((uint32_t)strM * SB);
        return;
    }
#pragma unroll
    for (int r = 0; r < C::WPW; ++r) {
        const int j = wjr(r);
        const int so = (int)soff + wb[r] + bs;
#pragma unroll
        for (int q = 0; q < (hooks::one_dma_piece ? 1 : PCS); ++q) {
            lds_void *dst = (lds_void *)((unsigned char *)win + ((buf * NW + fa * MB + j) * WB + q * PB));
            if (l16 < need_b - q * PB)
                __builtin_amdgcn_raw_ptr_buffer_load_lds(rsD, dst, 16, l16, so + q * PB, 0, 0);
        }
    }
    if constexpr (C::FBX) {
        const bool mirror = C::FB2 && QSPEC(MIR, P.mir);
#pragma unroll
        for (int r = 0; r < C::WPW; ++r) {
            const int j = wjr(r);
            const int so = mirror ? (int)soff2 + wb2[r] + bs : (int)soff + wb[r] + bs;
#pragma unroll
            for (int q = 0; q < PCS; ++q) {
                lds_void *dst = (lds_void *)((unsigned char *)win + ((buf * NW + fb * MB + j) * WB + q * PB));
                if (l16 < need_b - q * PB)
                    __builtin_amdgcn_raw_ptr_buffer_load_lds(rsM, dst, 16, l16, so + q * PB, 0, 0);
            }
        }
    }
    soff += (uint32_t)strN * SB;
    if constexpr (C::FB2) { if (QSPEC(MIR, P.mir)) soff2 -= (uint32_t)strN * SB; }
    if constexpr (C::SYM || C::BIG) {
        if (soff >= DMA_REBASE) {
            offD += soff; soff = 0; rsD = make_rs(offD, (uint64_t)fa * P.x_fstride);
            if constexpr (C::FBX) { if (!(C::FB2 && QSPEC(MIR, P.mir))) rsM = make_rs(offD, (uint64_t)fb * P.x_fstride); }
        }
    }
    if constexpr (C::SYM && !C::FOLD) {
#pragma unroll
        for (int r = 0; r < C::WPW; ++r) {
            const int j = __builtin_amdgcn_readfirstlane(wave + C::WAVES * r);
            const int so = (int)soff2 + wb2[r] + bs;
#pragma unroll
            for (int q = 0; q < PCS; ++q) {
                lds_void *dst = (lds_void *)((unsigned char *)win + ((buf * NW + MB + j) * WB + q * PB));
                if (l16 < need_b - q * PB)
                    __builtin_amdgcn_raw_ptr_buffer_load_lds(rsM, dst, 16, l16, so + q * PB, 0, 0);
            }
        }
        soff2 += (uint32_t)strM * SB;
        if (soff2 >= DMA_REBASE) { offM += soff2; soff2 = 0; rsM = make_rs(offM, 0); }
    }
}

}
```

### qups_amd/das_spec.py

```python
from __future__ import annotations

import collections
import ctypes as C
import os
import threading
from dataclasses import dataclass, field
from typing import Any, Sequence

import numpy as np

from . import _lib

_FUNS = ("DAS", "SYN", "MUL", "BF", "delays")
_PREC = {"double": _lib.QDAS_F64, "single": _lib.QDAS_F32, "halfT": _lib.QDAS_F16}
_REAL_NP = {"double": np.float64, "single": np.float32, "halfT": np.float32}


class DasError(ValueError):

    def __init__(self, msg, identifier=None):
        super().__init__(msg)
        self.identifier = identifier


# ... 272 lines not shown
        if prec == "halfT":
            adt = np.float16 if apod_real else None
        if adt is None:
            flat = np.concatenate([np.stack([a.real, a.imag], 0).reshape(2, -1, order="F").T.reshape(-1)
                                   for a in apods]).astype(np.float16)
        else:
            parts = [_flat_cached(a, adt) for a in apods]
            flat = parts[0] if len(parts) == 1 else np.concatenate(parts)
    else:
        flat = None

    t0v = _to_numpy(t0, np.float64).reshape(-1) if fun != "delays" else np.zeros(1)
    if t0v.size not in (1, M):
        raise DasError("t0 must be a scalar or have one value per transmit.")
    Pv4 = np.concatenate([Pv, np.broadcast_to(t0v.reshape(1, -1), (1, M))], 0)

    keep_rx, keep_tx = fun in ("SYN", "BF"), fun in ("MUL", "BF")
    flag = _lib.INTERP_FLAGS[interp] + 8 * keep_rx + 16 * keep_tx + 32 * tpose
    osize = {"DAS": (1, 1), "SYN": (N, 1), "MUL": (1, M), "BF": (M, N) if tpose else (N, M), "delays": (N, M)}[fun]
    col = lambda A: _col_cached(A, rt)
    rxa = opts.get("rx_apod")
    if rxa is not None:
        if not isinstance(rxa, dict) or "kind" not in rxa:
            raise DasError("'rx-apod' expects the dict returned by qups_amd.apodization.rx_apod_spec")
        nrm = rxa.get("normals")
        if nrm is not None:
            nrm = np.asarray(nrm, dtype=np.float64).reshape(3, -1)
            if nrm.shape[1] != N:
                raise DasError(f"'rx-apod': expected 3 x {N} element normals, got {nrm.shape}")
            nrm = col(nrm)
        rxa = dict(kind=int(rxa["kind"]), p=tuple(float(v) for v in rxa.get("p", (0.0, 0.0))), normals=nrm)
    return DasProblem(fun=fun, prec=prec, flag=int(flag), VS=bool(opts["VS"]), DV=bool(opts["DV"]), Isz=Isz,
                      T=T, N=N, M=M, fsz=tuple(fsz), fs=fs, fmod=float(opts["fmod"]),
                      Pi=col(Pi), Pr=col(Pr), Pv=col(Pv4), Nv=col(Nv), cinv=col(cinv),
                      apod=flat, apod_real=apod_real, acstride=np.asarray(table, dtype=np.uint64),
                      S=len(apods), tpose=tpose, interp=interp, osize=osize, rx_apod=rxa)


def _torch():
    import torch
    return torch


def _colmajor(t):
    if t.ndim <= 1:
        return t.contiguous()
    if t.is_cuda and 2 <= t.ndim <= 3 and t.is_contiguous() and t.element_size() in (2, 4, 8, 16) and t.numel():
        sh = tuple(t.shape) if t.ndim == 3 else (t.shape[0], 1, t.shape[1])
        if sh[1] <= 65535 and (sh[0] + 63) // 64 <= 65535:
            torch = _torch()
            out = torch.empty(tuple(reversed(t.shape)), dtype=t.dtype, device=t.device)
            with torch.cuda.device(t.device):
                _lib.check(_lib.lib().qdas_permute3(C.c_void_p(t.data_ptr()), C.c_void_p(out.data_ptr()), sh[0], sh[1], sh[2],
                                                    t.element_size(), C.c_void_p(torch.cuda.current_stream().cuda_stream)))
            return out
    return t.permute(*reversed(range(t.ndim))).contiguous()


def _data_dtype(prec):
    torch = _torch()
    return {"double": torch.complex128, "single": torch.complex64, "halfT": torch.complex32}[prec]


def _cast_data(x, prec, device):
    torch = _torch()
    if not _is_torch(x):
        x = torch.from_numpy(np.asarray(x))
    x = x.to(device)
    want = _data_dtype(prec)
    if x.dtype == want:
        return x
    if not x.is_complex():
        x = torch.complex(x.to(torch.float32 if prec != "double" else torch.float64),
                          torch.zeros((), device=device, dtype=torch.float32 if prec != "double" else torch.float64).expand_as(x))
    if prec == "halfT":
        return torch.view_as_complex(torch.view_as_real(x.to(torch.complex64)).to(torch.float16).contiguous())
    return x.to(want)


class DasPlan:

    def __init__(self, prob: DasProblem, device=None, kernel: int = _lib.KERNEL_AUTO,
                 i_begin: int = 0, i_count: int = 0, reciprocal: bool = True, jit: bool = False, mirror: bool = True, mirror_slab: bool = False,
                 fold: bool = True, approx_symmetry: bool = False, prefolded: bool = False):
        torch = _torch()
        self.lib = _lib.lib()
        if not torch.cuda.is_available():
            raise RuntimeError("qups_amd: no HIP device visible -- the DAS path has no CPU fallback")
        self.device = torch.device(device if device is not None else f"cuda:{torch.cuda.current_device()}")
        self.prob = prob
        self.i_begin = int(i_begin)
        self.i_count = int(i_count) if i_count else prob.I - int(i_begin)
        self.out_count = 2 * self.i_count if mirror_slab else self.i_count
        dev = self.device
        up = lambda a: torch.from_numpy(a).to(dev) if a is not None else None
        self._bufs = [up(prob.Pi), up(prob.Pr), up(prob.Pv), up(prob.Nv), up(prob.cinv),
                      up(prob.apod.view(np.uint16) if (prob.apod is not None and prob.apod.dtype == np.float16) else prob.apod)]
        self._acs = (C.c_uint64 * len(prob.acstride))(*[int(v) for v in prob.acstride])
        d = _lib.Desc()
        d.sz = _lib.Sizes(prob.T, prob.N, prob.M, prob.Isz[0], prob.Isz[1], prob.Isz[2], prob.S, prob.flag,
                          int(prob.VS), int(prob.DV), _PREC[prob.prec])
        d.fs, d.fmod = prob.fs, prob.fmod
        ptr = lambda t: C.c_void_p(t.data_ptr()) if t is not None else C.c_void_p(0)
        d.Pi, d.Pr, d.Pv, d.Nv, d.cinv, d.apod = (ptr(self._bufs[0]), ptr(self._bufs[1]), ptr(self._bufs[2]),
                                                   ptr(self._bufs[3]), ptr(self._bufs[4]), ptr(self._bufs[5]))
        d.acstride = self._acs
        d.mem, d.apod_real, d.kernel = _lib.MEM_DEVICE, int(prob.apod_real), int(kernel)
        d.device = dev.index if dev.index is not None else torch.cuda.current_device()
        d.i_begin, d.i_count, d.y_ld = self.i_begin, self.i_count, 0
        d.plan_flags = ((0 if reciprocal else _lib.PLAN_NO_RECIPROCAL) | (_lib.PLAN_JIT if jit else 0) | (0 if mirror else _lib.PLAN_NO_MIRROR)
                        | (_lib.PLAN_MIRROR_SLAB if mirror_slab else 0) | (0 if fold else _lib.PLAN_NO_FOLD)
                        | (_lib.PLAN_APPROX_SYMMETRY if approx_symmetry else 0) | (_lib.PLAN_PREFOLDED if prefolded else 0))
        if prob.rx_apod is not None:
            d.rx_apod_kind = prob.rx_apod["kind"]
            d.rx_apod_p[0], d.rx_apod_p[1] = prob.rx_apod["p"]
            self._bufs.append(up(prob.rx_apod["normals"]))
            d.rx_normals = ptr(self._bufs[-1])
        self._desc = d
        self._h = C.c_void_p()
        self._lock = threading.RLock()
        with torch.cuda.device(dev):
            _lib.check(self.lib.qdas_plan_create(C.byref(self._h), C.byref(d)))
            self._jit_note = (self.lib.qdas_last_error() or b"").decode(errors="replace") if jit else ""

    def jit_note(self) -> str:
        return self._jit_note if "QDAS_PLAN_JIT" in self._jit_note else ""

    @property
    def kernel(self) -> str:
        return _lib.KERNEL_NAMES.get(self.lib.qdas_plan_kernel(self._h), "?")

    def tile_shape(self) -> tuple:
        tz, tc = C.c_int(0), C.c_int(0)
        _lib.check(self.lib.qdas_plan_tile_shape(self._h, C.byref(tz), C.byref(tc), None, None))
        return int(tz.value), int(tc.value)

    def wave_shape(self) -> tuple:
        tz, tc, wz = C.c_int(0), C.c_int(0), C.c_int(0)
        _lib.check(self.lib.qdas_plan_tile_shape(self._h, C.byref(tz), C.byref(tc), C.byref(wz), None))
        return (int(wz.value), 64 // int(wz.value)) if wz.value else (0, 0)

    def aperture_split(self) -> int:
        tz, tc, ks = C.c_int(0), C.c_int(0), C.c_int(0)
        _lib.check(self.lib.qdas_plan_tile_shape(self._h, C.byref(tz), C.byref(tc), None, C.byref(ks)))
        return int(ks.value)

    @property
    def reciprocal(self) -> bool:
        return bool(self.lib.qdas_plan_reciprocal(self._h))

    def symmetry_bound(self) -> tuple:
        a, b = C.c_double(), C.c_double()
        _lib.check(self.lib.qdas_plan_symmetry_bound(self._h, C.byref(a), C.byref(b)))
        return float(a.value), float(b.value)

    @property
    def folded(self) -> bool:
        return bool(self.lib.qdas_plan_folded(self._h))

    @property
    def mirror(self) -> bool:
        return bool(self.lib.qdas_plan_mirror(self._h))

    def kernel_name(self) -> str:
        buf = C.create_string_buffer(256)
        _lib.check(self.lib.qdas_plan_kernel_name(self._h, buf, 256))
        return buf.value.decode()

    def fallback_tiles(self) -> int:
        n = C.c_uint64()
        _lib.check(self.lib.qdas_plan_fallback_tiles(self._h, C.byref(n)))
        return int(n.value)

    def set_timing(self, on: bool = True):
        _lib.check(self.lib.qdas_plan_set_timing(self._h, int(on)))

    def last_kernel_ms(self) -> float:
        ms = C.c_float()
        _lib.check(self.lib.qdas_plan_last_kernel_ms(self._h, C.byref(ms)))
        return float(ms.value)

    def _stream(self):
        return C.c_void_p(_torch().cuda.current_stream(self.device).cuda_stream)

    def execute_colmajor(self, xc, F: int = 1):
        p = self.prob
        oN, oM = p.osize
        y = _torch().empty((F, oM, oN, self.out_count), dtype=_data_dtype(p.prec), device=self.device)
        return self.execute_into(xc, y, F)

    def execute_into(self, xc, y, F: int = 1):
        p = self.prob
        oN, oM = p.osize
        per = p.T * p.N * p.M
        want = _data_dtype(p.prec)
# ... 373 lines not shown
```

Before: 67.24 Mpixel/s.

## Add half-stage LDS ring for folded mirror tile kernel

Adds a half-stage ring pipeline for the folded, lateral-mirror, one-frame tile kernel. Each 32-transmit stage is split into two 16-transmit halves held in four LDS slots, with DMA of the next half issued and published per half instead of per full stage. The aim is finer-grained overlap of global-to-LDS staging with the interpolation math, and a smaller LDS footprint per slot. It adds barriers per half, more complex cursor bookkeeping, and a JIT fallback to the full-stage kernel if the build fails or spills to scratch.

After: 63.05 Mpixel/s. 6.2% lower.

```diff
diff --git a/include/qdas.h b/include/qdas.h
--- a/include/qdas.h
+++ b/include/qdas.h
@@ -52,6 +52,8 @@
 #define QDAS_PLAN_APPROX_SYMMETRY 64
 
 #define QDAS_PLAN_PREFOLDED     128
+
+#define QDAS_PLAN_NO_HALFRING   256
 
 
 #define QDAS_OK            0
diff --git a/qups_amd/_lib.py b/qups_amd/_lib.py
--- a/qups_amd/_lib.py
+++ b/qups_amd/_lib.py
@@ -17,6 +17,7 @@
 QDAS_CONV_FULL, QDAS_CONV_SAME, QDAS_CONV_VALID, QDAS_CONV_CAUSAL = 0, 1, 2, 3
 QDAS_CONV_X_ONE_COLUMN, QDAS_CONV_X_ONE_SLICE, QDAS_CONV_Y_ONE_COLUMN, QDAS_CONV_Y_ONE_SLICE = 1, 2, 4, 8
 PLAN_NO_RECIPROCAL, PLAN_JIT, PLAN_COPY_INPUTS, PLAN_NO_MIRROR, PLAN_MIRROR_SLAB, PLAN_NO_FOLD, PLAN_APPROX_SYMMETRY, PLAN_PREFOLDED = 1, 2, 4, 8, 16, 32, 64, 128
+PLAN_NO_HALFRING = 256
 COH_SLSC_AVERAGE, COH_SLSC_ENSEMBLE, COH_DMAS, COH_COHFAC, COH_PCF = 1, 2, 3, 4, 5
 QDAS_ENOCONV = 5
 QDAS_ENOTLDS = 6
diff --git a/qups_amd/csrc/das_tile_impl.h b/qups_amd/csrc/das_tile_impl.h
--- a/qups_amd/csrc/das_tile_impl.h
+++ b/qups_amd/csrc/das_tile_impl.h
@@ -13,12 +13,13 @@
 #include "tile_taps.h"
 #include "tile_hooks.h"
 #include "das_tile_cfg.h"
+#include "tile_halfring.h"
 
 namespace qdas {
 
 typedef __attribute__((address_space(3))) void lds_void;
 
-template <int INTERP_, typename ST_, bool FMOD_, bool WTAB_, bool SYM_, bool FB2_, bool FB4_, int WAVES_, int MB_, int W_, int NBUF_, bool BIG_, bool LUT_, bool BF_ = false, bool MIRQ_ = false, bool FOLD_ = false>
+template <int INTERP_, typename ST_, bool FMOD_, bool WTAB_, bool SYM_, bool FB2_, bool FB4_, int WAVES_, int MB_, int W_, int NBUF_, bool BIG_, bool LUT_, bool BF_ = false, bool MIRQ_ = false, bool FOLD_ = false, bool HALFRING_ = false>
 struct TileCfg {
     static constexpr int INTERP = INTERP_, WAVES = WAVES_, MB = MB_, W = W_, NBUF = NBUF_;
     using ST = ST_;
@@ -28,6 +29,7 @@
     static constexpr bool MIRQ = MIRQ_;
     static constexpr bool FOLD = FOLD_;
     static constexpr bool FOLDQ = FOLD_ && MIRQ_;
+    static constexpr bool HALFRING = HALFRING_;
     static constexpr bool QUAD = FB4 || (MIRQ && !FOLD) || (FOLDQ && FB2);
     static constexpr bool TWO = (SYM && !FOLD) || FBX || FOLDQ;
     static constexpr bool ONEACC = (FB2 && !SYM && sizeof(ST_) == 8 && MB_ >= 32) || (!TWO && sizeof(ST_) == 8 && FMOD_ && WTAB_ && INTERP_ == 3 && !BF_ && !LUT_ && !BIG_);
@@ -64,6 +66,7 @@
     static_assert(!MIRQ || FOLD || (SYM && MB_ == WAVES_ && 4 * MB_ * W_ * (int)sizeof(ST_) <= 65536), "reciprocal + lateral-mirror mode: one window per wave and set, immediate LDS offsets");
     static_assert(!FOLD || (SYM && !WTAB_ && !BIG && !LUT && !BF_ && sizeof(ST_) == 8), "folded data: reciprocal plans, fp32, weights folded into the data");
     static_assert(!FOLDQ || (MB_ % WAVES_ == 0 && (FB2 ? 4 : 2) * MB_ * W_ * (int)sizeof(ST_) <= 65536), "folded data + lateral-mirror mode: two (two frames: four) window sets within the immediate LDS offsets");
+    static_assert(!HALFRING_ || (FOLDQ && !FB2_ && !FMOD_ && MB_ == 32 && WAVES_ == 16 && NBUF_ == 2), "half-stage ring: folded data + lateral-mirror mode, one frame, 32-transmit stages in two buffers");
     static_assert(!BIG || (!SYM && !FBX), "the re-basing general kernel runs one frame per launch");
     static_assert(!(FOLDQ && FB2) || MB_ == WAVES_, "folded data + mirror mode, two frames: one window per wave and set");
     static_assert(!LUT || (!SYM && !FB4 && !BIG && (!FB2 || JITB)), "table-driven delays: general mode, one frame per launch (hiprtc builds: the lateral-mirror mode's two window sets)");
@@ -128,6 +131,7 @@
     template <bool PROBE> __device__ __forceinline__ bool prologue();
     __device__ __forceinline__ void plan_stages();
     template <bool CHECK> __device__ __forceinline__ void run();
+    template <bool CHECK> __device__ __forceinline__ void run_halfring();
     __device__ __forceinline__ void epilogue();
 
     __device__ __forceinline__ uint32_t blk(uint32_t r) const {
@@ -160,9 +164,10 @@
     __device__ __forceinline__ int wjr(int r) const;
     __device__ __forceinline__ void dma_block(uint32_t m0);
     __device__ __forceinline__ void stage_dma(int bn, int buf);
-
-    template <bool CHECK, bool TAILV, bool WZ = true> __device__ __forceinline__ void pairs_plain(uint32_t n, uint32_t m0, int bn, float rb, uint32_t cbase, float phB, uint32_t wbase, uint64_t wmask, uint64_t xmask);
-    __device__ __forceinline__ void pairs_pipelined(float rb, uint32_t cbase);
+    __device__ __forceinline__ void stage_dma_half(int bn, uint32_t slot, uint32_t h);
+
+    template <bool CHECK, bool TAILV, bool WZ = true, int HALFSEL = -1> __device__ __forceinline__ void pairs_plain(uint32_t n, uint32_t m0, int bn, float rb, uint32_t cbase, float phB, uint32_t wbase, uint64_t wmask, uint64_t xmask);
+    template <int HALFSEL = -1> __device__ __forceinline__ void pairs_pipelined(float rb, uint32_t cbase);
     template <bool CHECK, bool TAILV> __device__ __forceinline__ void pairs_f64(uint32_t n, uint32_t m0, int bn, double rb, uint32_t cbase);
     __device__ __forceinline__ void frame_sums(v2f (&Sf)[4]) const {
         if constexpr (C::FOLDQ && C::FB2) { Sf[0] = acc; Sf[1] = acc1; Sf[2] = acc2; Sf[3] = acc3; }
@@ -683,6 +688,96 @@
     }
 }
 
+template <class C> template <bool CHECK> __device__ __forceinline__ void Tile<C>::run_halfring() {
+    namespace hr = halfring;
+    static_assert(C::MB == (int)hr::MB && C::MB / 2 == (int)hr::HALF && C::NBUF * 2 == (int)hr::SLOTS && C::NDMA % 2 == 0 && C::WPW == 2, "half-stage ring: two halves of one window per wave and set");
+    constexpr int GRP = C::NDMA / 2;
+    constexpr uint32_t SLOTB = (uint32_t)(C::NW / 2) * (uint32_t)C::WB;
+    const hr::Walk wk = {N, n_lo, N, S, split};
+    hr::Cursor fc = hr::first(wk);
+    if (hr::done(wk, fc)) return;
+    uint32_t fq = 0;
+    const uint32_t rec_off = (uint32_t)(uintptr_t)((__attribute__((address_space(3))) unsigned char *)(unsigned char *)nrec);
+    float vbn;
+    auto front_req = [&]() {
+        const uint32_t a = rec_off + 16u * (fc.n < N ? fc.n : N - 1u);
+        asm volatile("ds_read_b32 %0, %1" : "=v"(vbn) : "v"(a));
+    };
+    auto front_go = [&]() {
+        const int bn = __builtin_amdgcn_readfirstlane(__float_as_int(vbn));
+        const uint32_t slot = hr::slot_of(fq);
+        stage_dma_half(bn, slot, fc.h);
+        ++fq;
+        const uint32_t r0 = fc.r;
+        hr::next(wk, fc);
+        if (fc.r != r0 && !hr::done(wk, fc)) dma_block(fc.m0);
+        front_req();
+    };
+    auto publish = [&](uint32_t g) {
+        if (g >= 2u)      asm volatile("s_waitcnt vmcnt(%1) lgkmcnt(0)\n\ts_barrier" : "+v"(vbn) : "n"(2 * GRP) : "memory");
+        else if (g == 1u) asm volatile("s_waitcnt vmcnt(%1) lgkmcnt(0)\n\ts_barrier" : "+v"(vbn) : "n"(GRP) : "memory");
+        else              asm volatile("s_waitcnt vmcnt(0) lgkmcnt(0)\n\ts_barrier" : "+v"(vbn) :: "memory");
+    };
+    dma_block(fc.m0);
+    front_req();
+#pragma unroll
+    for (uint32_t b = 0; b < hr::AHEAD; ++b) {
+        if (hr::done(wk, fc)) break;
+        asm volatile("s_waitcnt lgkmcnt(0)" : "+v"(vbn));
+        front_go();
+    }
+    publish(hr::groups_in_flight(0u, fq));
+    uint32_t cq = 0;
+    uint32_t cr = 0, n = n_lo, m0 = blk(0);
+    bool fresh = true;
+    const bool dma_late = !hooks::no_late_dma && wave < C::WAVES / 2;
+    while (m0 < M) {
+        timer.mark(0);
+        float4 rec;
+        {
+            const uint32_t a = rec_off + 16u * n;
+            asm volatile("ds_read_b128 %0, %1\n\ts_waitcnt lgkmcnt(0)" : "=&v"(rec) : "v"(a));
+        }
+        timer.mark(1);
+        if (fresh) {
+#pragma unroll
+            for (int p = 0; p < C::MB / 2; ++p) {
+                const uint32_t ma = m0 + 2 * p < M ? m0 + 2 * p : M - 1, mb = m0 + 2 * p + 1 < M ? m0 + 2 * p + 1 : M - 1;
+                const float4 ea = nrec[ma], eb = nrec[mb];
+                const double fc0 = symC - (double)symCi - 0.5;
+                ra[p] = (v2f){(float)(b_at(ea.y, ea.z, ea.w) - (double)__float_as_int(ea.x) + fc0),
+                              (float)(b_at(eb.y, eb.z, eb.w) - (double)__float_as_int(eb.x) + fc0)};
+                __builtin_amdgcn_sched_barrier(0);
+            }
+            fresh = false;
+        }
+        timer.mark(2);
+        const int bn = __float_as_int(rec.x);
+        const float rb = hooks::fake_rx_delay ? (float)(lane * 2 + 3) + 0.37f * (float)(n & 7) : (float)(s_at(n, rec.y, rec.z, rec.w) - (double)bn);
+        unroll<2>([&](auto hc) {
+            constexpr int h = decltype(hc)::value;
+            if (!hr::half_exists(N, n, m0, (uint32_t)h)) return;
+            const bool more = !hr::done(wk, fc);
+            if (!hooks::no_stage_dma && more && !dma_late) front_go();
+            const uint32_t cbase = win_off + hr::slot_of(cq) * SLOTB - (MAGIC_BITS * (uint32_t)C::SB);
+            const uint32_t mh = m0 + (uint32_t)h * hr::HALF;
+            if (n < mh && mh + hr::HALF <= M) {
+                if constexpr (C::K == 4 && !CHECK && !hooks::no_pipeline) pairs_pipelined<h>(rb, cbase);
+                else pairs_plain<CHECK, false, true, h>(n, m0, bn, rb, cbase, 0.f, 0u, ~0ull, ~0ull);
+            }
+            else                              pairs_plain<CHECK, true, true, h>(n, m0, bn, rb, cbase, 0.f, 0u, ~0ull, ~0ull);
+            if constexpr (!hooks::no_fair_prio) __builtin_amdgcn_s_setprio(3);
+            if (!hooks::no_stage_dma && more && dma_late) front_go();
+            ++cq;
+            if (!hooks::no_stage_barrier) publish(fq > cq ? hr::groups_in_flight(cq, fq) : 0u);
+        });
+        timer.mark(3);
+        timer.mark(4);
+        timer.stage_done();
+        if (++n == nlim(m0)) { n = n_lo; m0 = blk(++cr); fresh = true; }
+    }
+}
+
 template <class C> __device__ __forceinline__ void Tile<C>::epilogue() {
     if (syn || C::BF) return;
     if constexpr (C::F64) {
@@ -756,7 +851,8 @@
         t.timer.prologue_done();
         t.plan_stages();
         if (P.pro_mask == 2) return;
-        if (t.tile_interior) t.template run<false>(); else t.template run<true>();
+        if constexpr (C::HALFRING) { if (t.tile_interior) t.template run_halfring<false>(); else t.template run_halfring<true>(); }
+        else if (t.tile_interior) t.template run<false>(); else t.template run<true>();
         t.timer.finish(t.lane, t.wave, C::WAVES);
         t.epilogue();
     }
diff --git a/qups_amd/csrc/jit.h b/qups_amd/csrc/jit.h
--- a/qups_amd/csrc/jit.h
+++ b/qups_amd/csrc/jit.h
@@ -21,6 +21,7 @@
     int wreal;
     int fold;
     int lut;
+    int halfring;
     int plain;
 };
 
diff --git a/qups_amd/csrc/jit.hip b/qups_amd/csrc/jit.hip
--- a/qups_amd/csrc/jit.hip
+++ b/qups_amd/csrc/jit.hip
@@ -20,6 +20,7 @@
 #include "../../include/qdas.h"
 #include "api_util.h"
 #include "jit.h"
+#include "plan_modes.h"
 
 namespace qdas {
 
@@ -149,7 +150,7 @@
     const char *st = k.dtype == QDAS_F16 ? "uint32_t" : k.dtype == QDAS_F64 ? "double2" : "float2";
     static const char *INTERP_NAMES[8] = {"nearest", "linear", "cubic", "lanczos3", "linear", "cubicdev", "i6", "i7"};
     const std::string sym_name = std::string("qdas_jit_tile__") + INTERP_NAMES[k.interp & 7] + (k.dtype == QDAS_F16 ? "_f16" : k.dtype == QDAS_F64 ? "_f64" : "_f32")
-                                 + (k.lut ? "_lut" : "") + (k.fmod ? "_fmod" : "") + (k.wtab ? "_wtab" : "") + (k.sym ? "_sym" : "") + (k.fold ? "_fold" : "") + (k.mirq ? "_mirq" : k.mir ? "_mirror" : "")
+                                 + (k.lut ? "_lut" : "") + (k.fmod ? "_fmod" : "") + (k.wtab ? "_wtab" : "") + (k.sym ? "_sym" : "") + (k.fold ? "_fold" : "") + (k.mirq ? "_mirq" : k.mir ? "_mirror" : "") + (k.halfring ? "_halfring" : "")
                                  + (k.big ? "_big" : "") + "_mb" + std::to_string(k.mb) + "_w" + std::to_string(k.w) + "_n" + std::to_string((unsigned long long)k.N)
                                  + "_m" + std::to_string((unsigned long long)k.M) + "_t" + std::to_string((unsigned long long)k.T);
     snprintf(b, sizeof b,
@@ -162,7 +163,7 @@
              "#include \"das_tile_impl.h\"\n"
              "extern \"C\" __global__ void __launch_bounds__(%d, %d) %s(const qdas::TileParams P) {\n"
              "    extern __shared__ __attribute__((aligned(16))) unsigned char smem[];\n"
-             "    qdas::das_tile_body<qdas::TileCfg<%d, %s, %s, %s, %s, %s, false, %d, %d, %d, %d, %s, %s, false, %s, %s>, false>(P, smem);\n"
+             "    qdas::das_tile_body<qdas::TileCfg<%d, %s, %s, %s, %s, %s, false, %d, %d, %d, %d, %s, %s, false, %s, %s, %s>, false>(P, smem);\n"
              "}\n",
              k.plain ? "#define QDAS_ONEACC_PLAIN 1\n" : "",
              (unsigned long long)k.M, (unsigned long long)k.N, (unsigned long long)k.T, (unsigned long long)k.I1,
@@ -170,7 +171,7 @@
              k.has_apix ? "true" : "false", k.apix_real, k.syn, k.has_st ? "true" : "false", k.has_cinv_pix ? "true" : "false", k.mslab ? 2 : ((k.mir || k.mirq) ? 1 : 0), k.wreal ? 1 : 0,
              k.waves * 64, k.waves / 4, sym_name.c_str(),
              k.interp, st, k.fmod ? "true" : "false", k.wtab ? "true" : "false", k.sym ? "true" : "false", k.mir ? "true" : "false", k.waves, k.mb, k.w, k.nbuf,
-             k.big ? "true" : "false", k.lut ? "true" : "false", k.mirq ? "true" : "false", k.fold ? "true" : "false");
+             k.big ? "true" : "false", k.lut ? "true" : "false", k.mirq ? "true" : "false", k.fold ? "true" : "false", k.halfring ? "true" : "false");
     std::string src = b;
     if (const char *e = getenv("QDAS_JIT_DEFINES")) {
         std::string defs, item;
@@ -358,6 +359,10 @@
             s.plain = 1;
             Entry b2 = build(jit_source(s), device, false);
             if (b2.err.empty() || b2.transient) b = b2; else s.plain = 0;
+        }
+        if (s.halfring && !b.transient && (!b.err.empty() || b.scratch > 0)) {
+            s.halfring = 0;
+            b = build(jit_source(s), device, false);
         }
         b.spec = s;
         return b;
@@ -426,7 +431,7 @@
 
 namespace qdas {
 #define QDAS_JITSPEC_FIELDS(X) X(interp) X(dtype) X(fmod) X(wtab) X(sym) X(big) X(waves) X(mb) X(w) X(nbuf) X(N) X(M) X(T) X(I1) X(strN) X(strM) X(kindB) X(kindS) X(tzl) X(wzl) \
-    X(ksplit) X(gen_kind) X(has_apix) X(apix_real) X(syn) X(has_st) X(has_cinv_pix) X(mir) X(mirq) X(mslab) X(wreal) X(fold) X(lut) X(plain)
+    X(ksplit) X(gen_kind) X(has_apix) X(apix_real) X(syn) X(has_st) X(has_cinv_pix) X(mir) X(mirq) X(mslab) X(wreal) X(fold) X(lut) X(plain) X(halfring)
 std::string jit_spec_string(const JitSpec &k) {
     std::string o = "raw:";
 #define X(f) o += std::string(#f "=") + std::to_string((unsigned long long)k.f) + ",";
@@ -486,7 +491,7 @@
                 else if (nm == "syn") k.syn = (int)v; else if (nm == "wtab") k.wtab = v != 0; else if (nm == "kindB") k.kindB = (int)v; else if (nm == "kindS") k.kindS = (int)v;
                 else if (nm == "tzl") k.tzl = (int)v; else if (nm == "wzl") k.wzl = (int)v; else if (nm == "ksplit") k.ksplit = (unsigned)v; else if (nm == "I1") k.I1 = (uint64_t)v;
                 else if (nm == "has_cinv_pix") k.has_cinv_pix = v != 0; else if (nm == "has_st") k.has_st = v != 0;
-                else if (nm == "wreal") k.wreal = v != 0;
+                else if (nm == "wreal") k.wreal = v != 0; else if (nm == "halfring") k.halfring = v != 0;
                 else if (nm == "mb") k.mb = (int)v; else if (nm == "w") k.w = (int)v;
                 else if (nm == "fold") { k.fold = v != 0; if (k.fold) { k.sym = 1; const qdas::Cfg &g2 = qdas::CFGS[qdas::cfg_index(dtype, 1, 1, v == 1, k.mirq, 1)]; k.waves = g2.waves; k.mb = g2.mb; k.w = g2.w; k.nbuf = g2.nbuf; } }
                 else if (nm == "mirq") { k.mirq = v != 0; if (k.mirq) { const qdas::Cfg &g2 = qdas::CFGS[qdas::cfg_index(dtype, 1, 1, 1, 1)]; k.waves = g2.waves; k.mb = g2.mb; k.w = g2.w; k.nbuf = g2.nbuf; k.sym = 1; } }
@@ -501,6 +506,10 @@
     if (msg && msg_len) snprintf(msg, msg_len, "%s", err.empty() ? key.c_str() : err.c_str());
     if (code_bytes) *code_bytes = code.size();
     return err.empty() ? 0 : 1;
+}
+
+extern "C" int qdas_debug_halfring_mode(int dtype, int fold, int mirq, int narrow, int nfr, int jit, double fmod, int plan_flags) {
+    return qdas::modes::halfring_applies(dtype, fold, mirq, narrow, nfr, jit != 0, false, fmod, qdas::modes::halfring_declined(plan_flags, getenv("QDAS_NO_HALFRING") != nullptr, getenv("QDAS_HALFRING") != nullptr)) ? 1 : 0;
 }
 
 extern "C" int qdas_debug_lazy_compile(int ci, int interp, int sample_bytes, int fm, int wt, int probe, char *msg, size_t msg_len, unsigned long long *code_bytes) {
diff --git a/qups_amd/csrc/plan_modes.h b/qups_amd/csrc/plan_modes.h
--- a/qups_amd/csrc/plan_modes.h
+++ b/qups_amd/csrc/plan_modes.h
@@ -45,7 +45,7 @@
 
 struct Switches {
     bool no_sym = false, no_fold = false, no_jit = false, no_mirror = false, no_mirq = false, no_narrow = false, no_role_swap = false, no_bpix = false,
-         no_w64 = false, no_mirror_wpix = false, no_mirror_wpix32 = false, no_side_split = false, no_wide = false, no_fb2 = false, no_fb4 = false, no_fold16 = false;
+         no_w64 = false, no_mirror_wpix = false, no_mirror_wpix32 = false, no_side_split = false, no_wide = false, no_fb2 = false, no_fb4 = false, no_fold16 = false, no_halfring = false;
     double sym_tol = -1.0;
     int ksplit = 0;
     int ksplit_m = 0;
@@ -331,12 +331,21 @@
     int dtype = QDAS_F32;
     int sym = 0, fold = 0, mir = 0, narrow_raw = 0, big = 0, bf = 0, syn = 0, stage_shift = 0, probe = 0, nfr = 1;
     bool lut = false, has_wtab = false, has_apix = false, has_bpix = false, has_part = false, jit = false;
+    bool no_halfring = false;
     int gen_kind = 0;
     double fmod = 0.0;
     uint32_t act_bytes = 0, ksplit = 1;
     uint64_t N = 0, M = 0;
 };
-struct LaunchChoice { int narrow = 0, fold = 0, mirq = 0, nf = 1, nfr = 1; bool probe_f32sym = false; size_t lds = 0; int cfg = 0; };
+struct LaunchChoice { int narrow = 0, fold = 0, mirq = 0, nf = 1, nfr = 1; bool probe_f32sym = false; size_t lds = 0; int cfg = 0; bool halfring = false; };
+
+constexpr bool HALFRING_DEFAULT = true;
+inline bool halfring_declined(int plan_flags, bool env_no, bool env_yes) { return (plan_flags & QDAS_PLAN_NO_HALFRING) != 0 || env_no || !(HALFRING_DEFAULT || env_yes); }
+inline bool halfring_applies(int dtype, int fold, int mirq, int narrow, int nfr, bool jit, bool probe, double fmod, bool no_halfring) {
+    if (!(dtype == 1 && fold && mirq && narrow == 1 && nfr == 1 && jit && !probe && fmod == 0.0 && !no_halfring)) return false;
+    const Cfg &g = CFGS[cfg_index(dtype, 1, 1, narrow, mirq, fold)];
+    return g.mb == 32 && g.nbuf == 2 && g.waves == 16 && g.w == 128;
+}
 
 inline const char *launch_legal(const LaunchShape &P, LaunchChoice *c) {
     const int dtype = P.dtype, sym = P.sym ? 1 : 0;
@@ -374,6 +383,7 @@
     if (P.bf && (sym || nf != 1 || dtype != 1 || P.lut || P.big || P.has_apix || P.gen_kind)) return "'BF': fp32 general mode without pixel weights";
     ch.narrow = narrow; ch.fold = fold; ch.mirq = mirq; ch.nf = nf; ch.nfr = nfr; ch.probe_f32sym = probe_f32sym; ch.lds = lds;
     ch.cfg = cfg_index(dtype, sym, 1, narrow, mirq, fold);
+    ch.halfring = halfring_applies(dtype, fold, mirq, narrow, nfr, P.jit, P.probe != 0, P.fmod, P.no_halfring);
     if (c) *c = ch;
     return nullptr;
 }
@@ -399,6 +409,7 @@
     if (o.wide) { L.narrow_raw = 2; L.sym = 0; if (L.fold) { L.fold = 0; L.has_wtab = table; } }
     L.N = tN; L.M = tM; L.ksplit = o.ksplit; L.has_part = o.ksplit > 1 && !L.bf;
     L.fmod = dt == QDAS_F64 ? d.fmod : (double)(float)d.fmod;
+    L.no_halfring = halfring_declined(d.plan_flags, false, false);
     return L;
 }
 inline const char *shape_mismatch(const LaunchShape &a, const LaunchShape &b) {
diff --git a/qups_amd/csrc/qdas_api.hip b/qups_amd/csrc/qdas_api.hip
--- a/qups_amd/csrc/qdas_api.hip
+++ b/qups_amd/csrc/qdas_api.hip
@@ -397,7 +397,7 @@
     sw.no_sym = on("QDAS_NO_SYM"); sw.no_fold = on("QDAS_NO_FOLD"); sw.no_jit = on("QDAS_NO_JIT"); sw.no_mirror = on("QDAS_NO_MIRROR"); sw.no_mirq = on("QDAS_NO_MIRQ");
     sw.no_narrow = on("QDAS_NO_NARROW"); sw.no_role_swap = on("QDAS_NO_ROLE_SWAP"); sw.no_bpix = on("QDAS_NO_BPIX"); sw.no_w64 = on("QDAS_NO_W64");
     sw.no_mirror_wpix = on("QDAS_NO_MIRROR_WPIX"); sw.no_mirror_wpix32 = on("QDAS_NO_MIRROR_WPIX32"); sw.no_side_split = on("QDAS_NO_SIDE_SPLIT"); sw.no_wide = on("QDAS_NO_WIDE");
-    sw.no_fb2 = on("QDAS_NO_FB2"); sw.no_fb4 = on("QDAS_NO_FB4"); sw.no_fold16 = on("QDAS_NO_FOLD16");
+    sw.no_fb2 = on("QDAS_NO_FB2"); sw.no_fb4 = on("QDAS_NO_FB4"); sw.no_fold16 = on("QDAS_NO_FOLD16"); sw.no_halfring = on("QDAS_NO_HALFRING");
     if (const char *e = getenv("QDAS_SYM_TOL")) { const double v = atof(e); if (v >= 0.0 && v <= 0.5) sw.sym_tol = v; }
     if (const char *e = getenv("QDAS_KSPLIT")) { const int v = atoi(e); if (v >= 1 && v <= 8) sw.ksplit = v; }
     if (const char *e = getenv("QDAS_KSPLIT_M")) { const int v = atoi(e); if (v >= 1 && v <= 8) sw.ksplit_m = v; }
@@ -875,6 +875,8 @@
     return QDAS_OK;
 }
 
+namespace qdas { modes::LaunchShape launch_shape(const TileParams &P, int dtype, bool jit); }
+
 static int plan_jit(qdas_plan *pl, const qdas_desc *desc, int *remake) {
     const qdas_sizes &z = pl->d.sz;
     const int dt = z.dtype;
@@ -902,10 +904,17 @@
     }
     if (const char *e = getenv("QDAS_JIT_NBUF")) { const int nb = atoi(e); if (nb >= 2 && nb <= 4) k.nbuf = nb; }
     if (const char *e = getenv("QDAS_JIT_W")) { const int wv = atoi(e); if (wv >= 64 && wv <= 1024 && wv % 64 == 0) k.w = wv; }
+    {
+        modes::LaunchShape ls = launch_shape(t, dt, true);
+        ls.nfr = 1; ls.probe = 0;
+        ls.no_halfring = modes::halfring_declined(desc->plan_flags, getenv("QDAS_NO_HALFRING") != nullptr, getenv("QDAS_HALFRING") != nullptr);
+        modes::LaunchChoice lc;
+        k.halfring = (!modes::launch_legal(ls, &lc) && lc.halfring && k.fold && k.mirq && !k.fmod && !k.wtab && k.mb == 32 && k.nbuf == 2 && k.waves == 16 && k.w == 128) ? 1 : 0;
+    }
     pl->jit_lds = dt == QDAS_F64 ? 0 : jit_tile_lds(k, t.N, t.M, t.act_bytes, t.wtab != nullptr);
     const JitKernel jk = pl->jit_lds > (size_t)160 * 1024 ? JitKernel{nullptr, "", "LDS image too large for the requested configuration"} : jit_kernel(k, pl->device);
     pl->jit_fn = jk.fn;
-    if (jk.fn) { pl->jit_tag = "jit " + jk.key; pl->jit_mb = k.mb; pl->jit_w = k.w; return QDAS_OK; }
+    if (jk.fn) { pl->jit_tag = "jit " + jk.key + (k.halfring ? ", half-stage ring" : ""); pl->jit_mb = k.mb; pl->jit_w = k.w; return QDAS_OK; }
     g_err = "QDAS_PLAN_JIT: " + jk.err + " -- using the prebuilt kernel";
     const bool unfolded = dt == QDAS_F32 && t.sym && !t.fold;
     if ((dt == QDAS_F32 && t.mir && !t.sym && (t.apix || t.gen_kind)) || unfolded)
diff --git a/qups_amd/csrc/tile_halfring.h b/qups_amd/csrc/tile_halfring.h
--- /dev/null
+++ b/qups_amd/csrc/tile_halfring.h
@@ -0,0 +1,38 @@
+#pragma once
+#ifndef __HIPCC_RTC__
+#include <stdint.h>
+#endif
+
+#if defined(__HIPCC__) || defined(__HIPCC_RTC__)
+#define QDAS_HR_FN __host__ __device__ __forceinline__
+#else
+#define QDAS_HR_FN inline
+#endif
+
+namespace qdas {
+namespace halfring {
+
+constexpr uint32_t MB = 32, HALF = 16, SLOTS = 4, AHEAD = SLOTS - 1;
+
+struct Walk { uint32_t N, n_lo, n_hi, S, split; };
+struct Cursor { uint32_t r, m0, n, h; };
+
+QDAS_HR_FN uint32_t block_first(const Walk &w, uint32_t r) { return (r * w.S + ((r & 1u) ? w.S - 1u - w.split : w.split)) * MB; }
+QDAS_HR_FN uint32_t block_nlim(const Walk &w, uint32_t m0) { const uint32_t e = m0 + MB < w.N ? m0 + MB : w.N; return e < w.n_hi ? e : w.n_hi; }
+QDAS_HR_FN bool half_exists(uint32_t N, uint32_t n, uint32_t m0, uint32_t h) { const uint32_t mh = m0 + HALF * h; return mh < N && n <= mh + (HALF - 1u); }
+QDAS_HR_FN bool done(const Walk &w, const Cursor &c) { return c.m0 >= w.N; }
+QDAS_HR_FN void settle(const Walk &w, Cursor &c) {
+    while (c.m0 < w.N) {
+        if (c.n >= block_nlim(w, c.m0)) { ++c.r; c.m0 = block_first(w, c.r); c.n = w.n_lo; c.h = 0; }
+        else if (c.h > 1u) { ++c.n; c.h = 0; }
+        else if (half_exists(w.N, c.n, c.m0, c.h)) return;
+        else ++c.h;
+    }
+}
+QDAS_HR_FN Cursor first(const Walk &w) { Cursor c = {0u, block_first(w, 0u), w.n_lo, 0u}; settle(w, c); return c; }
+QDAS_HR_FN void next(const Walk &w, Cursor &c) { ++c.h; settle(w, c); }
+QDAS_HR_FN uint32_t slot_of(uint32_t q) { return q & (SLOTS - 1u); }
+QDAS_HR_FN uint32_t groups_in_flight(uint32_t q, uint32_t issued) { const uint32_t g = issued - q - 1u; return g < AHEAD - 1u ? g : AHEAD - 1u; }
+
+}
+}
diff --git a/qups_amd/csrc/tile_pairs.h b/qups_amd/csrc/tile_pairs.h
--- a/qups_amd/csrc/tile_pairs.h
+++ b/qups_amd/csrc/tile_pairs.h
@@ -6,15 +6,19 @@
 
 namespace qdas {
 
-template <class C> template <bool CHECK, bool TAILV, bool WZ>
+template <class C> template <bool CHECK, bool TAILV, bool WZ, int HALFSEL>
 __device__ __forceinline__ void Tile<C>::pairs_plain(uint32_t n, uint32_t m0, int bn, float rb, uint32_t cbase, float phB, uint32_t wbase, uint64_t wmask, uint64_t xmask) {
     constexpr int K = C::K, MB = C::MB, WB = C::WB, INTERP = C::INTERP, NHP = C::NHP;
     constexpr bool SYM = C::SYM, FB4 = C::QUAD, FBX = C::FBX, TWO = C::TWO, F32 = C::F32, FMOD = C::FMOD, WTAB = C::WTAB, BF = C::BF;
     constexpr bool TAIL = (!SYM || C::FOLD) && TAILV, DIAG = SYM && TAILV;
     const bool wmixed = C::WST && WZ && ((((wmask ^ (wmask >> 1)) & 0x5555555555555555ull) != 0ull) || (SYM && C::WTAB && (((xmask ^ (xmask >> 1)) & 0x5555555555555555ull) != 0ull)));
+    static_assert(HALFSEL < 0 || C::HALFRING, "half stages: the half-stage ring only");
+    constexpr int WS = C::HALFRING ? MB / 2 : MB;
     unroll<MB / 2>([&](auto pc) {
         constexpr int p = decltype(pc)::value;
-        if constexpr (!hooks::no_fair_prio && (p * 4) % (MB / 2) == 0) __builtin_amdgcn_s_setprio(QDAS_PAIR_PRIO(3 - (p * 4) / (MB / 2)));
+        if constexpr (HALFSEL >= 0 && p / (MB / 4) != HALFSEL) return;
+        constexpr int PN = HALFSEL >= 0 ? MB / 4 : MB / 2, pp = HALFSEL >= 0 ? p - HALFSEL * (MB / 4) : p;
+        if constexpr (!hooks::no_fair_prio && (pp * 4) % PN == 0) __builtin_amdgcn_s_setprio(QDAS_PAIR_PRIO(3 - (pp * 4) / PN));
         const uint32_t m = m0 + 2 * p;
         if constexpr (TAIL) { if (m >= M) return; }
         if constexpr (DIAG) { if (m + 1 < n) return; }
@@ -53,8 +57,8 @@
                 taps_f32 g0, g1, h0, h1;
                 if constexpr (hooks::no_tap_reads) { for (int k = 0; k < 4; ++k) { g0.s[k] = h0.s[k] = (v2f){s.x, t.x}; g1.s[k] = h1.s[k] = (v2f){t.y, s.y}; } }
                 else {
-                    lds_issue<K, (GSET * MB + 2 * p) * WB>(g0, ad0); lds_issue<K, (GSET * MB + 2 * p + 1) * WB>(g1, ad1);
-                    if constexpr (TWO) { lds_issue<K, (HSET * MB + 2 * p) * WB>(h0, ad0); lds_issue<K, (HSET * MB + 2 * p + 1) * WB>(h1, ad1); }
+                    lds_issue<K, (GSET * WS + (2 * p) % WS) * WB>(g0, ad0); lds_issue<K, (GSET * WS + (2 * p + 1) % WS) * WB>(g1, ad1);
+                    if constexpr (TWO) { lds_issue<K, (HSET * WS + (2 * p) % WS) * WB>(h0, ad0); lds_issue<K, (HSET * WS + (2 * p + 1) % WS) * WB>(h1, ad1); }
                 }
                 if constexpr (hp == 0) {
                     if constexpr (hooks::trivial_weights) { w[0] = s; w[1] = t; w[2] = tm; w[3] = s + t; }
@@ -100,8 +104,8 @@
                 if constexpr (RECIP && K == 1) { v0 += h0.s[0]; v1 += h1.s[0]; }
             } else {
                 taps_f16 g0, g1, h0, h1;
-                lds_issue<K, (GSET * MB + 2 * p) * WB>(g0, ad0); lds_issue<K, (GSET * MB + 2 * p + 1) * WB>(g1, ad1);
-                if constexpr (TWO) { lds_issue<K, (HSET * MB + 2 * p) * WB>(h0, ad0); lds_issue<K, (HSET * MB + 2 * p + 1) * WB>(h1, ad1); }
+                lds_issue<K, (GSET * WS + (2 * p) % WS) * WB>(g0, ad0); lds_issue<K, (GSET * WS + (2 * p + 1) % WS) * WB>(g1, ad1);
+                if constexpr (TWO) { lds_issue<K, (HSET * WS + (2 * p) % WS) * WB>(h0, ad0); lds_issue<K, (HSET * WS + (2 * p + 1) % WS) * WB>(h1, ad1); }
                 if constexpr (hp == 0 && K > 1) weights2<INTERP>(s, w);
                 if constexpr (TWO) lds_fence2<K>(g0, g1, h0, h1, w); else lds_fence<K>(g0, g1, w);
                 if constexpr (DIAG) {
@@ -271,10 +275,12 @@
     });
 }
 
-template <class C> __device__ __forceinline__ void Tile<C>::pairs_pipelined(float rb, uint32_t cbase) {
+template <class C> template <int HALFSEL> __device__ __forceinline__ void Tile<C>::pairs_pipelined(float rb, uint32_t cbase) {
     constexpr int K = C::K, MB = C::MB, WB = C::WB, INTERP = C::INTERP, NHP = C::NHP;
     constexpr bool FB4 = C::QUAD, F32 = C::F32;
-    constexpr int NP = MB / 2, NU = NP * NHP;
+    static_assert(HALFSEL < 0 || C::HALFRING, "half stages: the half-stage ring only");
+    constexpr int WS = C::HALFRING ? MB / 2 : MB;
+    constexpr int NP = MB / 2, NALL = NP * NHP, U0 = HALFSEL >= 0 ? HALFSEL * (NALL / 2) : 0, NU = HALFSEL >= 0 ? NALL / 2 : NALL;
     using taps_t = std::conditional_t<F32, taps_f32, taps_f16>;
     taps_t gd0[2], gd1[2];
     v2f sv[2];
@@ -290,21 +296,21 @@
             a1v[p & 1] = __float_as_uint(tm.y) * (uint32_t)C::SB + cbase;
         }
         if constexpr (F32 && hooks::no_tap_reads) { for (int k = 0; k < 4; ++k) { gd0[u & 1].s[k] = (v2f){sv[p & 1].x, rb}; gd1[u & 1].s[k] = (v2f){rb, sv[p & 1].y}; } }
-        else { lds_issue<K, (GSET * MB + 2 * p) * WB>(gd0[u & 1], a0v[p & 1]); lds_issue<K, (GSET * MB + 2 * p + 1) * WB>(gd1[u & 1], a1v[p & 1]); }
+        else { lds_issue<K, (GSET * WS + (2 * p) % WS) * WB>(gd0[u & 1], a0v[p & 1]); lds_issue<K, (GSET * WS + (2 * p + 1) % WS) * WB>(gd1[u & 1], a1v[p & 1]); }
     };
-    index(std::integral_constant<int, 0>{});
+    index(std::integral_constant<int, U0>{});
     unroll<NU>([&](auto uc) {
-        constexpr int u = decltype(uc)::value, p = u / NHP, hp = u % NHP, HSET = FB4 ? 2 * hp + 1 : 1;
-        if constexpr (!hooks::no_fair_prio && (u * 4) % NU == 0) __builtin_amdgcn_s_setprio(QDAS_PAIR_PRIO(3 - (u * 4) / NU));
+        constexpr int uu = decltype(uc)::value, u = U0 + uu, p = u / NHP, hp = u % NHP, HSET = FB4 ? 2 * hp + 1 : 1;
+        if constexpr (!hooks::no_fair_prio && (uu * 4) % NU == 0) __builtin_amdgcn_s_setprio(QDAS_PAIR_PRIO(3 - (uu * 4) / NU));
         taps_t h0, h1;
         if constexpr (F32 && hooks::no_tap_reads) { for (int k = 0; k < 4; ++k) { h0.s[k] = sv[p & 1]; h1.s[k] = (v2f){sv[p & 1].y, sv[p & 1].x}; } }
-        else { lds_issue<K, (HSET * MB + 2 * p) * WB>(h0, a0v[p & 1]); lds_issue<K, (HSET * MB + 2 * p + 1) * WB>(h1, a1v[p & 1]); }
-        if constexpr (u + 1 < NU) index(std::integral_constant<int, u + 1>{});
+        else { lds_issue<K, (HSET * WS + (2 * p) % WS) * WB>(h0, a0v[p & 1]); lds_issue<K, (HSET * WS + (2 * p + 1) % WS) * WB>(h1, a1v[p & 1]); }
+        if constexpr (uu + 1 < NU) index(std::integral_constant<int, u + 1>{});
         if constexpr (hp == 0) {
             if constexpr (hooks::trivial_weights) { w[0] = sv[p & 1]; w[1] = sv[p & 1] + 1.f; w[2] = sv[p & 1] * 2.f; w[3] = 1.f - sv[p & 1]; }
             else weights2<INTERP>(sv[p & 1], w);
         }
-        if constexpr (u + 1 < NU) lds_fence2_keep<8>(gd0[u & 1], gd1[u & 1], h0, h1, w);
+        if constexpr (uu + 1 < NU) lds_fence2_keep<8>(gd0[u & 1], gd1[u & 1], h0, h1, w);
         else                      lds_fence2_keep<0>(gd0[u & 1], gd1[u & 1], h0, h1, w);
         v2f &A0 = *(FB4 ? (hp ? &acc2 : &acc) : &acc), &A1 = *(FB4 ? (hp ? &acc2 : &acc) : ((C::FOLDQ || C::ONEACC) ? &acc : &acc1));
         v2f &B0 = *((C::MIRQ && !C::FOLD) ? (hp ? &acc2 : &acc) : FB4 ? (hp ? &acc3 : &acc1) : &acc2), &B1 = *((C::MIRQ && !C::FOLD) ? (hp ? &acc2 : &acc) : FB4 ? (hp ? &acc3 : &acc1) : ((C::SYM || C::ONEACC) ? &acc2 : &acc3));
diff --git a/qups_amd/csrc/tile_staging.h b/qups_amd/csrc/tile_staging.h
--- a/qups_amd/csrc/tile_staging.h
+++ b/qups_amd/csrc/tile_staging.h
@@ -167,4 +167,24 @@
     }
 }
 
+template <class C> __device__ __forceinline__ void Tile<C>::stage_dma_half(int bn, uint32_t slot, uint32_t h) {
+    constexpr int SB = C::SB, WB = C::WB, PB = C::PB, PCS = C::PCS, HW = C::MB / 2;
+    const int bs = bn * SB;
+    const int l16 = (int)(lane_now() * 16u);
+    const int j = wjr(0);
+    const int off[2] = {h ? qo[2] : qo[0], h ? qo[3] : qo[1]};
+#pragma unroll
+    for (int k = 0; k < 2; ++k) {
+#pragma unroll
+        for (int q = 0; q < PCS; ++q) {
+            lds_void *dst = (lds_void *)((unsigned char *)win + (((int)slot * 2 * HW + k * HW + j) * WB + q * PB));
+            if (l16 < need_b - q * PB)
+                __builtin_amdgcn_raw_ptr_buffer_load_lds(rsD, dst, 16, l16, off[k] + bs + q * PB, 0, 0);
+        }
+    }
+    const int dn = (int)((uint32_t)strN * SB), dm = (int)((uint32_t)strM * SB);
+    qo[0] += h ? 0 : dn; qo[1] -= h ? 0 : dm;
+    qo[2] += h ? dn : 0; qo[3] -= h ? dm : 0;
 }
+
+}
diff --git a/qups_amd/das_spec.py b/qups_amd/das_spec.py
--- a/qups_amd/das_spec.py
+++ b/qups_amd/das_spec.py
@@ -378,7 +378,7 @@
 
     def __init__(self, prob: DasProblem, device=None, kernel: int = _lib.KERNEL_AUTO,
                  i_begin: int = 0, i_count: int = 0, reciprocal: bool = True, jit: bool = False, mirror: bool = True, mirror_slab: bool = False,
-                 fold: bool = True, approx_symmetry: bool = False, prefolded: bool = False):
+                 fold: bool = True, approx_symmetry: bool = False, prefolded: bool = False, halfring: bool = True):
         torch = _torch()
         self.lib = _lib.lib()
         if not torch.cuda.is_available():
@@ -406,7 +406,8 @@
         d.i_begin, d.i_count, d.y_ld = self.i_begin, self.i_count, 0
         d.plan_flags = ((0 if reciprocal else _lib.PLAN_NO_RECIPROCAL) | (_lib.PLAN_JIT if jit else 0) | (0 if mirror else _lib.PLAN_NO_MIRROR)
                         | (_lib.PLAN_MIRROR_SLAB if mirror_slab else 0) | (0 if fold else _lib.PLAN_NO_FOLD)
-                        | (_lib.PLAN_APPROX_SYMMETRY if approx_symmetry else 0) | (_lib.PLAN_PREFOLDED if prefolded else 0))
+                        | (_lib.PLAN_APPROX_SYMMETRY if approx_symmetry else 0) | (_lib.PLAN_PREFOLDED if prefolded else 0)
+                        | (0 if halfring else _lib.PLAN_NO_HALFRING))
         if prob.rx_apod is not None:
             d.rx_apod_kind = prob.rx_apod["kind"]
             d.rx_apod_p[0], d.rx_apod_p[1] = prob.rx_apod["p"]
```
